# ansonb/RECON

Measured on NVIDIA B200. Metric: SpKBGAT fwd+bwd edges/sec, higher is better.
Workload: dtype f32

## Files before the change

include/spkbgat.h:

```cpp
#ifndef SPKBGAT_H
#define SPKBGAT_H
#include <stdint.h>

#ifdef __cplusplus
extern "C" {
#endif

typedef void* spk_stream_t;

#define SPK_ABI_VERSION 6
int spk_abi_version(void);
const char* spk_last_error(void);
int64_t spk_launch_count(void);

typedef struct {
    int32_t n_heads;
    int32_t d_head;
    int32_t d_pad;
    int32_t width;
} spk_geom;

typedef struct {
    const int32_t* task_seg;
    const int32_t* task_beg;
    const int32_t* task_end;
    const int32_t* hub_seg;
    const int32_t* hub_task_ptr;
    float* partial;
    int64_t ldpart;
    int32_t n_tasks;
    int32_t n_hubs;
    int32_t hub_thresh;
    int32_t reserved;
    const int32_t* task_order;
} spk_hub_tasks;

int spk_edges_concat(const int64_t* edge , int64_t e1, const int64_t* edge_type ,
                     const int64_t* nhop , int64_t e2,
                     int32_t* row, int32_t* col, int32_t* t1, int32_t* t2 ,
                     int64_t n_nodes, int64_t n_rel, int32_t* err_flag, spk_stream_t stream);
int spk_pack_index_host(const int64_t* src, int64_t n, int64_t stride, int64_t lo, int64_t hi, int32_t* dst, int32_t n_threads);
int spk_iota_i32(int32_t* v, int64_t n, spk_stream_t stream);
int64_t spk_sort_workspace_bytes(int64_t n);
int spk_sort_pairs(int32_t* keys, int32_t* vals, int32_t* keys_tmp, int32_t* vals_tmp, int64_t n, int32_t key_bits,
                   void* workspace, int32_t* result_in_tmp, spk_stream_t stream);
int spk_segment_ptr(const int32_t* sorted_keys, int64_t n, int32_t n_seg, int32_t* ptr , spk_stream_t stream);
int spk_gather_i32(const int32_t* src, const int32_t* idx, int64_t n, int32_t* out, spk_stream_t stream);
int spk_rel_incidence(const int32_t* t1, const int32_t* t2, int64_t e, int32_t n_rel, int32_t* keys, int32_t* vals,
                      spk_stream_t stream);

int spk_gemm_nn(const float* A, int64_t lda, const float* B, int64_t ldb, float* C, int64_t ldc,
                int64_t M, int32_t N, int32_t K, int32_t accumulate, spk_stream_t stream);
int64_t spk_gemm_tn_workspace_floats(int64_t M, int32_t Ka, int32_t Nb);
int spk_gemm_tn(const float* A, int64_t lda, const float* B, int64_t ldb, float* C, int64_t ldc,
                int64_t M, int32_t Ka, int32_t Nb, int32_t accumulate, float* workspace, spk_stream_t stream);

int32_t spk_gemm_nn_tc_supported(const float* A, int64_t lda, int64_t M, int32_t N, int32_t K);
int64_t spk_gemm_tc_workspace_floats(int32_t N, int32_t K);
int spk_gemm_nn_tc(const float* A, int64_t lda, const float* B, int64_t ldb, float* C, int64_t ldc,
                   int64_t M, int32_t N, int32_t K, int32_t accumulate, float* workspace, spk_stream_t stream);

int spk_gemm_nn_tc_act(const float* A, int64_t lda, const float* B, int64_t ldb, float* C, int64_t ldc,
                       int64_t M, int32_t N, int32_t K, int32_t accumulate, int32_t act, float* workspace,
                       spk_stream_t stream);
int spk_elu_inplace(float* x, int64_t ldx, int64_t n_rows, int32_t width, spk_stream_t stream);

int32_t spk_gemm_tn_tc_supported(const float* A, int64_t lda, const float* B, int64_t ldb, int64_t M, int32_t Ka, int32_t Nb);
int64_t spk_gemm_tn_tc_workspace_floats(int64_t M, int32_t Ka, int32_t Nb);
int spk_gemm_tn_tc(const float* A, int64_t lda, const float* B, int64_t ldb, float* C, int64_t ldc,
                   int64_t M, int32_t Ka, int32_t Nb, int32_t accumulate, float* workspace, spk_stream_t stream);

typedef struct {
    const int32_t* segptr; const int32_t* col; const int32_t* t1; const int32_t* t2;
    const float* P1; int64_t ld1;
    const float* P2; int64_t ld2;
    const float* P3; int64_t ld3;
    const float* mask; int64_t mask_stride;
    float* out; int64_t ldo;
    float* den; float* sw;
    int32_t* nanflag;
    int32_t n_rows; int32_t apply_elu; float alpha;
    int32_t elu_rows;
    spk_geom geom;
    spk_hub_tasks hub;
} spk_edge_fwd_args;
int spk_edge_attn_fwd(const spk_edge_fwd_args* args, spk_stream_t stream);

typedef struct {
    const int32_t* segptr; const int32_t* col; const int32_t* t1; const int32_t* t2;
    const float* P1; int64_t ld1;
    const float* P2; int64_t ld2;
    const float* P3; int64_t ld3;
    const float* mask; int64_t mask_stride;
    const float* out; const float* dout; int64_t ldo;
    const float* den;
    float* G; int64_t ldg;
    float* dP1; int64_t ldd1;
    float* rec;
    int32_t n_rows; int32_t apply_elu; float alpha; int32_t reserved;
    spk_geom geom;
    spk_hub_tasks hub;
} spk_edge_bwd_rows_args;
int spk_edge_attn_bwd_rows(const spk_edge_bwd_rows_args* args, spk_stream_t stream);

typedef struct {
    const int32_t* segptr; const int32_t* src; const int32_t* pos;
    const float* G; int64_t ldg;
    const float* rec;
    float* out; int64_t ldout;
    int32_t n_seg;
    int32_t flags;
    spk_geom geom;
    spk_hub_tasks hub;
} spk_seg_gather_args;
int spk_edge_attn_bwd_segments(const spk_seg_gather_args* args, spk_stream_t stream);

typedef struct {
    const int32_t* rowptr;
    const int32_t* colptr; const int32_t* csc_row; const int32_t* csc_pos; const int32_t* csc_t1; const int32_t* csc_t2;
    const float* P1; int64_t ld1;
    const float* P2; int64_t ld2;
    const float* P3; int64_t ld3;
    const float* mask; int64_t mask_stride;
    const float* out; const float* dout; int64_t ldo;
    const float* den; const float* sw;
    float* G; int64_t ldg;
    float* rowsc;
    float* dP1; int64_t ldd1;
    float* dP2; int64_t ldd2;
    float* rec;
    int32_t n_rows; int32_t n_cols; int32_t apply_elu; float alpha;
    spk_geom geom;
    spk_hub_tasks row_hub;
    spk_hub_tasks col_hub;
} spk_edge_bwd_fused_args;
int spk_edge_attn_bwd_fused(const spk_edge_bwd_fused_args* args, spk_stream_t stream);

typedef struct {
    spk_edge_bwd_fused_args base;
    const int32_t* relptr; const int32_t* rel_row; const int32_t* rel_pos;
    float* rec4; float* dsv;
    float* dP3; int64_t ldd3;
    int32_t n_rel; int32_t phases;
    spk_hub_tasks rel_hub;
    float* colsum; int64_t ld_colsum;
    float* rowsum; int64_t ld_rowsum;
    const float* G_rel; int64_t ldg_rel;
    int32_t dup; int32_t reserved;
} spk_edge_bwd_split_args;
int spk_edge_attn_bwd_split(const spk_edge_bwd_split_args* args, spk_stream_t stream);

typedef struct {
    int32_t n_heads;
    int32_t f_chunks;
    int32_t r_chunks;
    int32_t lz;
} spk_agg_geom;
int spk_agg_table(const float* X, int64_t ldx, const float* V, float* T, int64_t ldt, int64_t n_rows,
                  int32_t F, int32_t f_chunks, spk_stream_t stream);
typedef struct {
    const int32_t* segptr; const int32_t* col; const int32_t* t1; const int32_t* t2;
    const float* xrow; int64_t ldxr;
    const float* xcol; int64_t ldxc;
    const float* rel; int64_t ldr;
    const float* mask; int64_t mask_stride;
    float* z; int64_t ldz;
    float* den; float* sw;
    int32_t* nanflag;
    int32_t n_rows; float alpha;
    spk_agg_geom geom;
    spk_hub_tasks hub;
} spk_agg_fwd_args;
int spk_agg_fwd(const spk_agg_fwd_args* args, spk_stream_t stream);
int spk_agg_bwd_pre(const float* out, const float* dout, int64_t ldo, const float* den, int32_t n_heads, int32_t d_head,
                    int32_t apply_elu, float* dhn, int64_t ldd, float* dden, int64_t n_rows, spk_stream_t stream);
typedef struct {
    const int32_t* segptr; const int32_t* col; const int32_t* t1; const int32_t* t2;
    const float* xrow; int64_t ldxr; const float* xcol; int64_t ldxc; const float* rel; int64_t ldr;
    const float* mask; int64_t mask_stride;
    const float* dz; int64_t ldz;
    const float* den; const float* sw; const float* dden;
    float* gx; int64_t ldgx;
    float* gr; int64_t ldgr;
    float* rowout; int64_t ldro;
    float* rowsc;
    float* rec;
    int32_t n_rows; float alpha;
    spk_agg_geom geom;
    spk_hub_tasks hub;
} spk_agg_bwd_args;
int spk_agg_bwd_rows(const spk_agg_bwd_args* args, spk_stream_t stream);
int spk_agg_bwd_ctx(const spk_agg_bwd_args* args, spk_stream_t stream);
int spk_agg_dx(const float* rowout, int64_t ldro, const float* dxc, int64_t ldc, const float* V, int64_t n_rows,
               int32_t F, int32_t f_chunks, int32_t n_heads, float* dX, int64_t lddx, float* dq, spk_stream_t stream);

int spk_spmm_rowsum_fwd(const int32_t* segptr, const int32_t* perm, const float* w, int64_t ldw, int32_t width,
                        float* out, int64_t ldo, int32_t n_rows, spk_stream_t stream);
int spk_spmm_rowsum_bwd(const int64_t* edge_row , const float* gout, int64_t ldg, int32_t width,
                        float* gw, int64_t ldw, int64_t n_edges, spk_stream_t stream);

int spk_rownorm(const float* x, int64_t ldx, float* y, int64_t ldy, int64_t n_rows, int32_t width, spk_stream_t stream);
int spk_residual_norm_fwd(const float* ew, int64_t lde, const float* x2, int64_t ldx, const float* mask,
                          float* out, int64_t ldo, float* inv_norm, int64_t n_rows, int32_t width, spk_stream_t stream);
int spk_residual_norm_bwd(const float* g, int64_t ldg, const float* out, int64_t ldo, const float* mask,
                          const float* inv_norm, float* dew, int64_t lde, float* dx2, int64_t ldx,
                          int64_t n_rows, int32_t width, spk_stream_t stream);
int spk_mask_from_index(const int64_t* idx, int64_t n_idx, float* mask, int64_t n_rows, int32_t* flag, spk_stream_t stream);
typedef struct {
    const float* a[4]; const float* a2[4];
    float* da[4]; float* da2[4];
    int32_t n_heads, F, Rd, D;
    int32_t mode; int32_t d_pad, width;
    int32_t f_pad, lz;
    int32_t reserved;
    float* W0; int64_t ld0;
    float* W1; int64_t ld1;
    float* W2;
} spk_attn_weights_args;
int spk_attn_weights_fwd(const spk_attn_weights_args* args, spk_stream_t stream);
int spk_attn_weights_bwd(const spk_attn_weights_args* args, spk_stream_t stream);

int64_t spk_inner_product_workspace_bytes(void);
int spk_inner_product(const float* a, const float* b, int64_t n, void* workspace, float* out, int32_t accumulate,
                      spk_stream_t stream);

int64_t spk_margin_loss_partials(int64_t n_pos);
int spk_margin_loss_fwd(const int64_t* triples, int64_t n_triples, int64_t n_pos,
                        const float* ent, int64_t lde, int64_t n_ent, const float* rel, int64_t ldr, int64_t n_rel,
                        int32_t width, float margin, int32_t mean,
                        float* norm, uint32_t* sgn, float* coef, double* partial, float* loss,
                        int32_t* err_flag, spk_stream_t stream);
int spk_triple_incidence(const int64_t* triples, int64_t n_triples, int64_t n_ent, int64_t n_rel,
                         int32_t* ent_keys , int32_t* ent_vals, int32_t* rel_keys , int32_t* rel_vals,
// ... 66 lines not shown
```

recon_b200/_lib.py:

```python
import ctypes as C
import os

import torch

_HERE = os.path.dirname(os.path.abspath(__file__))
LIB_PATH = os.environ.get("SPK_LIB") or os.path.join(_HERE, "libspkbgat.so")

c_i32p = C.POINTER(C.c_int32)
c_i64p = C.POINTER(C.c_int64)
c_f32p = C.POINTER(C.c_float)
ABI_VERSION = 6


class Geom(C.Structure):
    _fields_ = [("n_heads", C.c_int32), ("d_head", C.c_int32), ("d_pad", C.c_int32), ("width", C.c_int32)]


class HubTasks(C.Structure):
    _fields_ = [("task_seg", C.c_void_p), ("task_beg", C.c_void_p), ("task_end", C.c_void_p),
                ("hub_seg", C.c_void_p), ("hub_task_ptr", C.c_void_p),
                ("partial", C.c_void_p), ("ldpart", C.c_int64),
                ("n_tasks", C.c_int32), ("n_hubs", C.c_int32), ("hub_thresh", C.c_int32), ("reserved", C.c_int32),
                ("task_order", C.c_void_p)]


class EdgeFwdArgs(C.Structure):
    _fields_ = [("segptr", C.c_void_p), ("col", C.c_void_p), ("t1", C.c_void_p), ("t2", C.c_void_p),
                ("P1", C.c_void_p), ("ld1", C.c_int64), ("P2", C.c_void_p), ("ld2", C.c_int64),
                ("P3", C.c_void_p), ("ld3", C.c_int64),
                ("mask", C.c_void_p), ("mask_stride", C.c_int64),
                ("out", C.c_void_p), ("ldo", C.c_int64), ("den", C.c_void_p), ("sw", C.c_void_p),
                ("nanflag", C.c_void_p),
                ("n_rows", C.c_int32), ("apply_elu", C.c_int32), ("alpha", C.c_float), ("elu_rows", C.c_int32),
                ("geom", Geom), ("hub", HubTasks)]


class EdgeBwdRowsArgs(C.Structure):
    _fields_ = [("segptr", C.c_void_p), ("col", C.c_void_p), ("t1", C.c_void_p), ("t2", C.c_void_p),
                ("P1", C.c_void_p), ("ld1", C.c_int64), ("P2", C.c_void_p), ("ld2", C.c_int64),
                ("P3", C.c_void_p), ("ld3", C.c_int64),
                ("mask", C.c_void_p), ("mask_stride", C.c_int64),
                ("out", C.c_void_p), ("dout", C.c_void_p), ("ldo", C.c_int64),
                ("den", C.c_void_p),
                ("G", C.c_void_p), ("ldg", C.c_int64), ("dP1", C.c_void_p), ("ldd1", C.c_int64),
                ("rec", C.c_void_p),
                ("n_rows", C.c_int32), ("apply_elu", C.c_int32), ("alpha", C.c_float), ("reserved", C.c_int32),
                ("geom", Geom), ("hub", HubTasks)]


class SegGatherArgs(C.Structure):
    _fields_ = [("segptr", C.c_void_p), ("src", C.c_void_p), ("pos", C.c_void_p),
                ("G", C.c_void_p), ("ldg", C.c_int64), ("rec", C.c_void_p),
                ("out", C.c_void_p), ("ldout", C.c_int64),
                ("n_seg", C.c_int32), ("flags", C.c_int32),
                ("geom", Geom), ("hub", HubTasks)]


class EdgeBwdFusedArgs(C.Structure):
    _fields_ = [("rowptr", C.c_void_p),
                ("colptr", C.c_void_p), ("csc_row", C.c_void_p), ("csc_pos", C.c_void_p), ("csc_t1", C.c_void_p),
                ("csc_t2", C.c_void_p),
                ("P1", C.c_void_p), ("ld1", C.c_int64), ("P2", C.c_void_p), ("ld2", C.c_int64),
                ("P3", C.c_void_p), ("ld3", C.c_int64),
                ("mask", C.c_void_p), ("mask_stride", C.c_int64),
                ("out", C.c_void_p), ("dout", C.c_void_p), ("ldo", C.c_int64),
                ("den", C.c_void_p), ("sw", C.c_void_p),
                ("G", C.c_void_p), ("ldg", C.c_int64), ("rowsc", C.c_void_p),
                ("dP1", C.c_void_p), ("ldd1", C.c_int64), ("dP2", C.c_void_p), ("ldd2", C.c_int64),
                ("rec", C.c_void_p),
                ("n_rows", C.c_int32), ("n_cols", C.c_int32), ("apply_elu", C.c_int32), ("alpha", C.c_float),
                ("geom", Geom), ("row_hub", HubTasks), ("col_hub", HubTasks)]


class EdgeBwdSplitArgs(C.Structure):
    _fields_ = [("base", EdgeBwdFusedArgs),
                ("relptr", C.c_void_p), ("rel_row", C.c_void_p), ("rel_pos", C.c_void_p),
                ("rec4", C.c_void_p), ("dsv", C.c_void_p),
                ("dP3", C.c_void_p), ("ldd3", C.c_int64),
                ("n_rel", C.c_int32), ("phases", C.c_int32),
                ("rel_hub", HubTasks),
                ("colsum", C.c_void_p), ("ld_colsum", C.c_int64),
                ("rowsum", C.c_void_p), ("ld_rowsum", C.c_int64),
                ("G_rel", C.c_void_p), ("ldg_rel", C.c_int64),
                ("dup", C.c_int32), ("reserved", C.c_int32)]


class AggGeom(C.Structure):
    _fields_ = [("n_heads", C.c_int32), ("f_chunks", C.c_int32), ("r_chunks", C.c_int32), ("lz", C.c_int32)]


class AggFwdArgs(C.Structure):
    _fields_ = [("segptr", C.c_void_p), ("col", C.c_void_p), ("t1", C.c_void_p), ("t2", C.c_void_p),
                ("xrow", C.c_void_p), ("ldxr", C.c_int64), ("xcol", C.c_void_p), ("ldxc", C.c_int64),
                ("rel", C.c_void_p), ("ldr", C.c_int64),
                ("mask", C.c_void_p), ("mask_stride", C.c_int64),
                ("z", C.c_void_p), ("ldz", C.c_int64), ("den", C.c_void_p), ("sw", C.c_void_p),
                ("nanflag", C.c_void_p),
                ("n_rows", C.c_int32), ("alpha", C.c_float),
                ("geom", AggGeom), ("hub", HubTasks)]


class AggBwdArgs(C.Structure):
    _fields_ = [("segptr", C.c_void_p), ("col", C.c_void_p), ("t1", C.c_void_p), ("t2", C.c_void_p),
                ("xrow", C.c_void_p), ("ldxr", C.c_int64), ("xcol", C.c_void_p), ("ldxc", C.c_int64),
                ("rel", C.c_void_p), ("ldr", C.c_int64),
                ("mask", C.c_void_p), ("mask_stride", C.c_int64),
                ("dz", C.c_void_p), ("ldz", C.c_int64),
                ("den", C.c_void_p), ("sw", C.c_void_p), ("dden", C.c_void_p),
                ("gx", C.c_void_p), ("ldgx", C.c_int64), ("gr", C.c_void_p), ("ldgr", C.c_int64),
                ("rowout", C.c_void_p), ("ldro", C.c_int64), ("rowsc", C.c_void_p), ("rec", C.c_void_p),
                ("n_rows", C.c_int32), ("alpha", C.c_float),
                ("geom", AggGeom), ("hub", HubTasks)]


_VP, _I64, _I32 = C.c_void_p, C.c_int64, C.c_int32

ALLOC_FN = C.CFUNCTYPE(C.c_void_p, C.c_void_p, C.c_int64)


class TripleGraphArgs(C.Structure):
    _fields_ = [("uptr", C.c_void_p), ("ut", C.c_void_p), ("ur0", C.c_void_p), ("ugs", C.c_void_p), ("uge", C.c_void_p),
                ("rs", C.c_void_p), ("n_nodes", C.c_int32), ("n_pairs", C.c_int32), ("n_triples", C.c_int32),
                ("reserved", C.c_int32)]


class NhopResult(C.Structure):
    _fields_ = [("adj_idx", C.c_void_p), ("adj_val", C.c_void_p), ("nhop", C.c_void_p), ("e1", C.c_int64), ("e2", C.c_int64)]


class LossBwdArgs(C.Structure):
    _fields_ = [("segptr", C.c_void_p), ("inc", C.c_void_p), ("coef", C.c_void_p), ("sgn", C.c_void_p),
                ("gscale", C.c_void_p), ("out", C.c_void_p), ("ldo", C.c_int64),
                ("n_seg", C.c_int32), ("width", C.c_int32), ("mode", C.c_int32), ("reserved", C.c_int32),
                ("hub", HubTasks)]


class SgdArgs(C.Structure):
    _fields_ = [("param", C.c_void_p * 16), ("grad", C.c_void_p * 16), ("numel", C.c_int64 * 16),
                ("count", C.c_int32), ("lr", C.c_float)]


class AttnWeightsArgs(C.Structure):
    _fields_ = [("a", C.c_void_p * 4), ("a2", C.c_void_p * 4), ("da", C.c_void_p * 4), ("da2", C.c_void_p * 4),
                ("n_heads", C.c_int32), ("F", C.c_int32), ("Rd", C.c_int32), ("D", C.c_int32),
                ("mode", C.c_int32), ("d_pad", C.c_int32), ("width", C.c_int32),
                ("f_pad", C.c_int32), ("lz", C.c_int32), ("reserved", C.c_int32),
                ("W0", C.c_void_p), ("ld0", C.c_int64), ("W1", C.c_void_p), ("ld1", C.c_int64), ("W2", C.c_void_p)]


SIGNATURES = {
    "spk_abi_version": (_I32, []),
    "spk_last_error": (C.c_char_p, []),
    "spk_launch_count": (_I64, []),
    "spk_edges_concat": (_I32, [_VP, _I64, _VP, _VP, _I64, _VP, _VP, _VP, _VP, _I64, _I64, _VP, _VP]),
    "spk_pack_index_host": (_I32, [_VP, _I64, _I64, _I64, _I64, _VP, _I32]),
    "spk_iota_i32": (_I32, [_VP, _I64, _VP]),
    "spk_sort_workspace_bytes": (_I64, [_I64]),
    "spk_sort_pairs": (_I32, [_VP, _VP, _VP, _VP, _I64, _I32, _VP, C.POINTER(_I32), _VP]),
    "spk_segment_ptr": (_I32, [_VP, _I64, _I32, _VP, _VP]),
    "spk_gather_i32": (_I32, [_VP, _VP, _I64, _VP, _VP]),
    "spk_rel_incidence": (_I32, [_VP, _VP, _I64, _I32, _VP, _VP, _VP]),
    "spk_gemm_nn": (_I32, [_VP, _I64, _VP, _I64, _VP, _I64, _I64, _I32, _I32, _I32, _VP]),
    "spk_gemm_nn_tc_supported": (_I32, [_VP, _I64, _I64, _I32, _I32]),
    "spk_gemm_tc_workspace_floats": (_I64, [_I32, _I32]),
    "spk_gemm_nn_tc": (_I32, [_VP, _I64, _VP, _I64, _VP, _I64, _I64, _I32, _I32, _I32, _VP, _VP]),
    "spk_gemm_nn_tc_act": (_I32, [_VP, _I64, _VP, _I64, _VP, _I64, _I64, _I32, _I32, _I32, _I32, _VP, _VP]),
    "spk_elu_inplace": (_I32, [_VP, _I64, _I64, _I32, _VP]),
    "spk_agg_table": (_I32, [_VP, _I64, _VP, _VP, _I64, _I64, _I32, _I32, _VP]),
    "spk_agg_fwd": (_I32, [C.POINTER(AggFwdArgs), _VP]),
    "spk_agg_bwd_pre": (_I32, [_VP, _VP, _I64, _VP, _I32, _I32, _I32, _VP, _I64, _VP, _I64, _VP]),
    "spk_agg_bwd_rows": (_I32, [C.POINTER(AggBwdArgs), _VP]),
    "spk_agg_bwd_ctx": (_I32, [C.POINTER(AggBwdArgs), _VP]),
    "spk_agg_dx": (_I32, [_VP, _I64, _VP, _I64, _VP, _I64, _I32, _I32, _I32, _VP, _I64, _VP, _VP]),
    "spk_gemm_tn_tc_supported": (_I32, [_VP, _I64, _VP, _I64, _I64, _I32, _I32]),
    "spk_gemm_tn_tc_workspace_floats": (_I64, [_I64, _I32, _I32]),
    "spk_gemm_tn_tc": (_I32, [_VP, _I64, _VP, _I64, _VP, _I64, _I64, _I32, _I32, _I32, _VP, _VP]),
    "spk_gemm_tn_workspace_floats": (_I64, [_I64, _I32, _I32]),
    "spk_gemm_tn": (_I32, [_VP, _I64, _VP, _I64, _VP, _I64, _I64, _I32, _I32, _I32, _VP, _VP]),
    "spk_edge_attn_fwd": (_I32, [C.POINTER(EdgeFwdArgs), _VP]),
    "spk_edge_attn_bwd_rows": (_I32, [C.POINTER(EdgeBwdRowsArgs), _VP]),
    "spk_edge_attn_bwd_segments": (_I32, [C.POINTER(SegGatherArgs), _VP]),
    "spk_edge_attn_bwd_fused": (_I32, [C.POINTER(EdgeBwdFusedArgs), _VP]),
    "spk_edge_attn_bwd_split": (_I32, [C.POINTER(EdgeBwdSplitArgs), _VP]),
    "spk_spmm_rowsum_fwd": (_I32, [_VP, _VP, _VP, _I64, _I32, _VP, _I64, _I32, _VP]),
    "spk_spmm_rowsum_bwd": (_I32, [_VP, _VP, _I64, _I32, _VP, _I64, _I64, _VP]),
    "spk_rownorm": (_I32, [_VP, _I64, _VP, _I64, _I64, _I32, _VP]),
    "spk_residual_norm_fwd": (_I32, [_VP, _I64, _VP, _I64, _VP, _VP, _I64, _VP, _I64, _I32, _VP]),
    "spk_residual_norm_bwd": (_I32, [_VP, _I64, _VP, _I64, _VP, _VP, _VP, _I64, _VP, _I64, _I64, _I32, _VP]),
    "spk_mask_from_index": (_I32, [_VP, _I64, _VP, _I64, _VP, _VP]),
    "spk_attn_weights_fwd": (_I32, [_VP, _VP]),
    "spk_attn_weights_bwd": (_I32, [_VP, _VP]),
    "spk_inner_product_workspace_bytes": (_I64, []),
    "spk_inner_product": (_I32, [_VP, _VP, _I64, _VP, _VP, _I32, _VP]),
    "spk_margin_loss_partials": (_I64, [_I64]),
    "spk_margin_loss_fwd": (_I32, [_VP, _I64, _I64, _VP, _I64, _I64, _VP, _I64, _I64, _I32, C.c_float, _I32,
                                   _VP, _VP, _VP, _VP, _VP, _VP, _VP]),
    "spk_triple_incidence": (_I32, [_VP, _I64, _I64, _I64, _VP, _VP, _VP, _VP, _VP, _VP]),
    "spk_margin_loss_bwd": (_I32, [C.POINTER(LossBwdArgs), _VP]),
    "spk_sgd_step": (_I32, [C.POINTER(SgdArgs), _VP]),
    "spk_triple_keys": (_I32, [_VP, _I64, _I64, _I64, _VP, _VP, _VP]),
    "spk_corrupt_triples": (_I32, [_VP, _I64, _I32, _VP, _I64, _I64, _I64, _VP, _VP, C.c_uint64, _VP, _VP, _VP]),
    "spk_nhop_build": (_I32, [C.POINTER(TripleGraphArgs), _VP, _I64, _I32, ALLOC_FN, _VP, C.POINTER(NhopResult), _VP]),
    "spk_gather_concat": (_I32, [_VP, _VP, _VP, _VP, _VP, _I32, _I64, _I32, _VP, _I64, _VP, _VP]),
    "spk_mlp_head_fwd": (_I32, [_VP, _I64, _VP, _VP, _VP, C.c_float, _I64, _I32, _VP, _VP]),
    "spk_mlp_head_bwd": (_I32, [_VP, _I64, _VP, _VP, C.c_float, _VP, _I64, _I32, _VP, _I64, _VP, _I64, _VP]),
    "spk_tanh_fwd": (_I32, [_VP, _I64, _I64, _I32, _VP]),
    "spk_tanh_bwd": (_I32, [_VP, _I64, _VP, _I64, _I64, _I32, _VP, _I64, _VP]),
    "spk_rank_scores": (_I32, [_VP, _I64, _VP, _I64, _VP, _VP, C.c_float, _I64, _I32, _I32, _VP, _I64, _VP]),
    "spk_linkpred_count": (_I32, [_VP, _I64, _I64, _VP, _I64, _I64, _VP, _VP, C.c_float, _I32, _VP, _VP, _I64, _I32,
                                  _VP, _I64, _VP, _VP, _VP, _VP, _VP]),
    "spk_linkpred_filter": (_I32, [_VP, _I64, _I64, _I64, _VP, C.c_float, _I32, _VP, _I64, _I32, _VP, _I64, _VP, _VP,
                                   _VP, _I64, _VP, _VP, _VP, _VP]),
    "spk_export_json": (_I32, [_VP, _I64, _I64, _I64, C.c_char_p, _I32]),
    "spk_export_bin": (_I32, [_VP, _I64, _I64, _I64, C.c_char_p]),
    "spk_import_json_shape": (_I32, [C.c_char_p, C.POINTER(_I64), C.POINTER(_I64)]),
    "spk_import_json": (_I32, [C.c_char_p, _VP, _I64, _I64, _I64, _I32]),
}

_lib = None
current_tag = ""


class _Lib:

    def __init__(self, cdll):
        self._cdll = cdll
        self.timing = None

    def __getattr__(self, name):
        fn = getattr(self._cdll, name)
        if self.timing is None or SIGNATURES[name][1][-1:] != [_VP] or "workspace" in name or "supported" in name:
            return fn

        def timed(*args):
            e0 = torch.cuda.Event(enable_timing=True)
            e1 = torch.cuda.Event(enable_timing=True)
            e0.record()
            rc = fn(*args)
            e1.record()
            global current_tag
            self.timing.append((name[4:] + (":" + current_tag if current_tag else ""), e0, e1))
            if "gemm" in name:
                current_tag = ""
            return rc
        return timed


def load():
    global _lib
    if _lib is not None:
        return _lib
    if not os.path.exists(LIB_PATH):
        raise RuntimeError(
            f"{LIB_PATH} is missing: build it with `python -c 'import __graft_entry__ as g; g.build()'` "
            "(or make -C recon_b200/csrc). recon_b200 has no CPU / PyTorch fallback.")
    lib = C.CDLL(LIB_PATH)
    for name, (res, args) in SIGNATURES.items():
        fn = getattr(lib, name)
        fn.restype = res
        fn.argtypes = args
    if lib.spk_abi_version() != ABI_VERSION:
        raise RuntimeError(f"libspkbgat ABI {lib.spk_abi_version()} != binding {ABI_VERSION}")
    _lib = _Lib(lib)
    return _lib


def stream_ptr():
    return C.c_void_p(torch.cuda.current_stream().cuda_stream)


def ptr(t):
    if t is None:
        return None
    if not t.is_cuda:
        raise RuntimeError("recon_b200 ops need CUDA tensors (no CPU fallback)")
    return t.data_ptr()


def launch_count():
    return int(load().spk_launch_count())


def check(rc, what):
    if rc != 0:
        msg = load().spk_last_error().decode("utf-8", "replace")
        raise RuntimeError(f"libspkbgat {what} failed (code {rc}): {msg}")
```

recon_b200/csrc/spk_api.cu:

```cuda
#include "../../include/spkbgat.h"
#include "spk_common.cuh"
#include "spk_edge.cuh"
#include "spk_edge_bwd_fused.cuh"
#include "spk_agg.cuh"
#include "spk_gemm.cuh"
#include "spk_graph.cuh"
#include "spk_rowops.cuh"

namespace spk {

static thread_local char g_err[512] = "";
static unsigned long long g_launches = 0;

void set_error(const char* fmt, ...) {
    va_list ap;
    va_start(ap, fmt);
    vsnprintf(g_err, sizeof(g_err), fmt, ap);
    va_end(ap);
}

int check_launch(const char* what) {
    const cudaError_t e = cudaGetLastError();
    __atomic_fetch_add(&g_launches, 1ULL, __ATOMIC_RELAXED);
    if (e == cudaSuccess) return 0;
// ... 61 lines not shown
extern "C" {

int spk_abi_version(void) { return SPK_ABI_VERSION; }
const char* spk_last_error(void) { return g_err; }
int64_t spk_launch_count(void) { return (int64_t)__atomic_load_n(&g_launches, __ATOMIC_RELAXED); }

int spk_edges_concat(const int64_t* edge, int64_t e1, const int64_t* edge_type, const int64_t* nhop, int64_t e2,
                     int32_t* row, int32_t* col, int32_t* t1, int32_t* t2, int64_t n_nodes, int64_t n_rel,
                     int32_t* err_flag, spk_stream_t stream) {
    if (e1 + e2 >= (1LL << 31) || n_nodes >= (1LL << 31)) { set_error("edges_concat: sizes exceed int32"); return 1; }
    if (e2 > 0 && !t2) { set_error("edges_concat: t2 required when 2-hop rows are given"); return 1; }
    return edges_concat(reinterpret_cast<const long long*>(edge), e1, reinterpret_cast<const long long*>(edge_type),
                        reinterpret_cast<const long long*>(nhop), e2, row, col, t1, t2, n_nodes, n_rel, err_flag,
                        (cudaStream_t)stream);
}
int spk_iota_i32(int32_t* v, int64_t n, spk_stream_t stream) { return iota_i32(v, n, (cudaStream_t)stream); }
int64_t spk_sort_workspace_bytes(int64_t n) { return radix_sort_workspace_bytes(n); }
int spk_sort_pairs(int32_t* keys, int32_t* vals, int32_t* keys_tmp, int32_t* vals_tmp, int64_t n, int32_t key_bits,
                   void* workspace, int32_t* result_in_tmp, spk_stream_t stream) {
    if (key_bits < 1 || key_bits > 31) { set_error("sort_pairs: key_bits %d out of range", key_bits); return 1; }
    return radix_sort_pairs(keys, vals, keys_tmp, vals_tmp, n, key_bits, workspace, result_in_tmp, (cudaStream_t)stream);
}
int spk_segment_ptr(const int32_t* sorted_keys, int64_t n, int32_t n_seg, int32_t* ptr, spk_stream_t stream) {
    return segment_ptr(sorted_keys, n, n_seg, ptr, (cudaStream_t)stream);
}
int spk_gather_i32(const int32_t* src, const int32_t* idx, int64_t n, int32_t* out, spk_stream_t stream) {
    return gather_i32(src, idx, n, out, (cudaStream_t)stream);
}
int spk_rel_incidence(const int32_t* t1, const int32_t* t2, int64_t e, int32_t n_rel, int32_t* keys, int32_t* vals,
                      spk_stream_t stream) {
    return rel_incidence(t1, t2, e, n_rel, keys, vals, (cudaStream_t)stream);
}

int spk_gemm_nn(const float* A, int64_t lda, const float* B, int64_t ldb, float* C, int64_t ldc,
                int64_t M, int32_t N, int32_t K, int32_t accumulate, spk_stream_t stream) {
    if (lda < K || ldb < N || ldc < N) { set_error("gemm_nn: leading dimension too small"); return 1; }
    return gemm_nn_simt(A, lda, B, ldb, C, ldc, M, N, K, accumulate, (cudaStream_t)stream);
}
int64_t spk_gemm_tn_workspace_floats(int64_t M, int32_t Ka, int32_t Nb) { return gemm_tn_workspace_floats(M, Ka, Nb); }
int spk_gemm_tn(const float* A, int64_t lda, const float* B, int64_t ldb, float* C, int64_t ldc,
                int64_t M, int32_t Ka, int32_t Nb, int32_t accumulate, float* workspace, spk_stream_t stream) {
    if (lda < Ka || ldb < Nb || ldc < Nb) { set_error("gemm_tn: leading dimension too small"); return 1; }
    if (!workspace) { set_error("gemm_tn: workspace required"); return 1; }
    return gemm_tn_simt(A, lda, B, ldb, C, ldc, M, Ka, Nb, accumulate, workspace, (cudaStream_t)stream);
}

int32_t spk_gemm_nn_tc_supported(const float* A, int64_t lda, int64_t M, int32_t N, int32_t K) {
    return gemm_nn_tc_supported(A, lda, M, N, K);
}
int64_t spk_gemm_tc_workspace_floats(int32_t N, int32_t K) { return 2LL * N * gemm_tc_ldt(K); }
int spk_gemm_nn_tc(const float* A, int64_t lda, const float* B, int64_t ldb, float* C, int64_t ldc,
                   int64_t M, int32_t N, int32_t K, int32_t accumulate, float* workspace, spk_stream_t stream) {
    if (lda < K || ldb < N || ldc < N) { set_error("gemm_nn_tc: leading dimension too small"); return 1; }
    if (!gemm_nn_tc_supported(A, lda, M, N, K)) { set_error("gemm_nn_tc: A must be 16-byte aligned with lda %% 4 == 0"); return 1; }
    if (!workspace || (reinterpret_cast<uintptr_t>(workspace) & 15)) { set_error("gemm_nn_tc: aligned workspace required"); return 1; }
    return gemm_nn_tc(A, lda, B, ldb, C, ldc, M, N, K, accumulate, workspace, (cudaStream_t)stream);
}

int spk_gemm_nn_tc_act(const float* A, int64_t lda, const float* B, int64_t ldb, float* C, int64_t ldc,
                       int64_t M, int32_t N, int32_t K, int32_t accumulate, int32_t act, float* workspace, spk_stream_t stream) {
    if (lda < K || ldb < N || ldc < N) { set_error("gemm_nn_tc_act: leading dimension too small"); return 1; }
    if (!gemm_nn_tc_supported(A, lda, M, N, K)) { set_error("gemm_nn_tc_act: A must be 16-byte aligned with lda %% 4 == 0"); return 1; }
    if (!workspace || (reinterpret_cast<uintptr_t>(workspace) & 15)) { set_error("gemm_nn_tc_act: aligned workspace required"); return 1; }
    if (act < 0 || act > 2) { set_error("gemm_nn_tc_act: unknown activation %d", act); return 1; }
    return gemm_nn_tc(A, lda, B, ldb, C, ldc, M, N, K, accumulate, workspace, (cudaStream_t)stream, act);
}
int spk_elu_inplace(float* x, int64_t ldx, int64_t n_rows, int32_t width, spk_stream_t stream) {
    if (ldx < width) { set_error("elu_inplace: leading dimension too small"); return 1; }
    return launch_elu_inplace(x, ldx, n_rows, width, (cudaStream_t)stream);
}

int32_t spk_gemm_tn_tc_supported(const float* A, int64_t lda, const float* B, int64_t ldb, int64_t M, int32_t Ka, int32_t Nb) {
    return gemm_tn_tc_supported(A, lda, B, ldb, M, Ka, Nb);
}
int64_t spk_gemm_tn_tc_workspace_floats(int64_t M, int32_t Ka, int32_t Nb) { return gemm_tn_tc_workspace_floats(M, Ka, Nb); }
int spk_gemm_tn_tc(const float* A, int64_t lda, const float* B, int64_t ldb, float* C, int64_t ldc,
                   int64_t M, int32_t Ka, int32_t Nb, int32_t accumulate, float* workspace, spk_stream_t stream) {
    if (ldc < Nb) { set_error("gemm_tn_tc: leading dimension too small"); return 1; }
    if (!gemm_tn_tc_supported(A, lda, B, ldb, M, Ka, Nb)) { set_error("gemm_tn_tc: operands must be 16-byte aligned with ld %% 4 == 0"); return 1; }
    if (!workspace) { set_error("gemm_tn_tc: workspace required"); return 1; }
    return gemm_tn_tc(A, lda, B, ldb, C, ldc, M, Ka, Nb, accumulate, workspace, (cudaStream_t)stream);
}

int spk_edge_attn_fwd(const spk_edge_fwd_args* p, spk_stream_t stream) {
    EdgeFwdArgs a;
    if (!geom_ok(p->geom, &a.g, "edge_attn_fwd")) return 1;
    if ((p->ld1 & 3) || (p->ld2 & 3) || (p->ld3 & 3) || p->ld1 < p->geom.width || p->ld2 < p->geom.width ||
        p->ld3 < p->geom.width || !aligned16(p->P1) || !aligned16(p->P2) || !aligned16(p->P3)) {
        set_error("edge_attn_fwd: projected tables must be 16-byte aligned with ld >= width, ld %% 4 == 0");
        return 1;
    }
    a.segptr = p->segptr; a.col = p->col; a.t1 = p->t1; a.t2 = p->t2;
    a.P1 = p->P1; a.ld1 = p->ld1; a.P2 = p->P2; a.ld2 = p->ld2; a.P3 = p->P3; a.ld3 = p->ld3;
    a.mask = p->mask; a.mask_stride = p->mask_stride;
    a.out = p->out; a.ldo = p->ldo; a.den = p->den; a.sw = p->sw; a.nanflag = p->nanflag;
    a.n_rows = p->n_rows; a.alpha = p->alpha; a.apply_elu = p->apply_elu;
    a.elu_rows = p->elu_rows > 0 ? p->elu_rows : 0x7fffffff;
    a.out_vec = (p->geom.d_head % 4 == 0) && (p->ldo % 4 == 0) && aligned16(p->out);
    a.hub = hub_of(p->hub);
    if (a.hub.n_tasks > 0 && (a.hub.ldpart < p->geom.width + 2 * SPK_MAX_HEADS || (a.hub.ldpart & 3) || !aligned16(a.hub.partial))) {
        set_error("edge_attn_fwd: hub partial buffer needs ldpart >= width+8, ldpart %% 4 == 0");
        return 1;
    }
    return launch_edge_fwd(a, (cudaStream_t)stream);
}

int spk_edge_attn_bwd_rows(const spk_edge_bwd_rows_args* p, spk_stream_t stream) {
    EdgeBwdRowsArgs a;
    if (!geom_ok(p->geom, &a.g, "edge_attn_bwd_rows")) return 1;
    if ((p->ld1 & 3) || (p->ld2 & 3) || (p->ld3 & 3) || (p->ldg & 3) || (p->ldd1 & 3) || p->ldg < p->geom.n_heads * p->geom.d_pad ||
        p->ldd1 < p->geom.width || !aligned16(p->P1) || !aligned16(p->P2) || !aligned16(p->P3) || !aligned16(p->G) ||
        !aligned16(p->dP1) || (reinterpret_cast<uintptr_t>(p->rec) & 7)) {
        set_error("edge_attn_bwd_rows: bad leading dimension or alignment");
        return 1;
    }
    a.segptr = p->segptr; a.col = p->col; a.t1 = p->t1; a.t2 = p->t2;
    a.P1 = p->P1; a.ld1 = p->ld1; a.P2 = p->P2; a.ld2 = p->ld2; a.P3 = p->P3; a.ld3 = p->ld3;
    a.mask = p->mask; a.mask_stride = p->mask_stride;
    a.out = p->out; a.dout = p->dout; a.ldo = p->ldo; a.den = p->den;
    a.G = p->G; a.ldg = p->ldg; a.dP1 = p->dP1; a.ldd1 = p->ldd1; a.rec = p->rec;
    a.n_rows = p->n_rows; a.alpha = p->alpha; a.apply_elu = p->apply_elu;
    a.out_vec = (p->geom.d_head % 4 == 0) && (p->ldo % 4 == 0) && aligned16(p->out) && aligned16(p->dout);
    a.hub = hub_of(p->hub);
    if (a.hub.n_tasks > 0 && a.hub.ldpart < 2 * SPK_MAX_HEADS) { set_error("edge_attn_bwd_rows: hub ldpart must be >= 8"); return 1; }
    return launch_edge_bwd_rows(a, (cudaStream_t)stream);
}

int spk_edge_attn_bwd_segments(const spk_seg_gather_args* p, spk_stream_t stream) {
    SegGatherArgs a;
    if (!geom_ok(p->geom, &a.g, "edge_attn_bwd_segments")) return 1;
    if ((p->ldg & 3) || (p->ldout & 3) || p->ldout < p->geom.width || p->ldg < p->geom.n_heads * p->geom.d_pad ||
        !aligned16(p->G) || !aligned16(p->out) || (reinterpret_cast<uintptr_t>(p->rec) & 7)) {
        set_error("edge_attn_bwd_segments: bad leading dimension or alignment");
        return 1;
    }
    a.segptr = p->segptr; a.src = p->src; a.pos = p->pos; a.G = p->G; a.ldg = p->ldg; a.rec = p->rec;
    a.outp = p->out; a.ldout = p->ldout; a.n_seg = p->n_seg; a.prefer_stream = p->flags & 1;
    a.hub = hub_of(p->hub);
    if (a.hub.n_tasks > 0 && (a.hub.ldpart < p->geom.width || (a.hub.ldpart & 3) || !aligned16(a.hub.partial))) {
        set_error("edge_attn_bwd_segments: hub partial buffer needs ldpart >= width");
        return 1;
    }
    return launch_seg_gather(a, (cudaStream_t)stream);
}

static int fused_args_of(const spk_edge_bwd_fused_args* p, BwdFusedArgs& a, const char* who, int dup = 0);

int spk_edge_attn_bwd_fused(const spk_edge_bwd_fused_args* p, spk_stream_t stream) {
    BwdFusedArgs a;
    if (int rc = fused_args_of(p, a, "edge_attn_bwd_fused")) return rc;
    if (reinterpret_cast<uintptr_t>(p->rec) & 7) { set_error("edge_attn_bwd_fused: rec must be 8-byte aligned"); return 1; }
    return launch_edge_bwd_fused(a, (cudaStream_t)stream);
}

int spk_edge_attn_bwd_split(const spk_edge_bwd_split_args* q, spk_stream_t stream) {
    BwdSplitArgs a;
    if (int rc = fused_args_of(&q->base, a.f, "edge_attn_bwd_split", q->dup)) return rc;
    if (q->base.csc_t2 != nullptr) { set_error("edge_attn_bwd_split: graphs with 2-hop edges are not supported"); return 1; }
    if ((q->ldd3 & 3) || q->ldd3 < q->base.geom.width || !aligned16(q->dP3) || !aligned16(q->rec4) ||
        (reinterpret_cast<uintptr_t>(q->dsv) & 3)) {
        set_error("edge_attn_bwd_split: bad leading dimension or alignment");
        return 1;
    }
    a.colptr = a.f.colptr; a.csc_row = a.f.csc_row; a.csc_pos = a.f.csc_pos; a.csc_t1 = a.f.csc_t1;
    a.relptr = q->relptr; a.rel_row = q->rel_row; a.rel_pos = q->rel_pos;
    a.P2 = a.f.P2; a.ld2 = a.f.ld2; a.P3 = a.f.P3; a.ld3 = a.f.ld3; a.mask = a.f.mask; a.mask_stride = a.f.mask_stride;
    a.G = a.f.G; a.ldg = a.f.ldg; a.rowsc = a.f.rowsc; a.rec4 = q->rec4; a.dsv = q->dsv;
    a.dP2 = a.f.dP2; a.ldd2 = a.f.ldd2; a.dP3 = q->dP3; a.ldd3 = q->ldd3;
    a.n_cols = a.f.n_cols; a.n_rel = q->n_rel; a.g = a.f.g; a.alpha = a.f.alpha;
    a.col_hub = a.f.col_hub;
    if (a.f.row_hub.n_tasks > 0 && (a.f.row_hub.partial == nullptr || a.f.row_hub.ldpart < 4)) {
        set_error("edge_attn_bwd_split: row hub partial buffer [n_tasks, >= 4] required");
        return 1;
    }
    a.phases = q->phases == 0 ? 15 : q->phases;
    a.colsum = q->colsum; a.ld_colsum = q->ld_colsum;
    a.rowsum = q->rowsum; a.ld_rowsum = q->ld_rowsum;
    a.G_rel = q->G_rel ? q->G_rel : a.f.G; a.ldg_rel = q->G_rel ? q->ldg_rel : a.f.ldg;
    a.dup = q->dup;
    if ((a.rowsum && a.ld_rowsum < q->base.geom.n_heads) || (q->G_rel && ((q->ldg_rel & 3) || !aligned16(q->G_rel) ||
        q->ldg_rel < q->base.geom.n_heads * q->base.geom.d_pad)) || (a.dup && (a.phases & 1))) {
        set_error("edge_attn_bwd_split: bad rowsum / G_rel / dup arguments");
        return 1;
    }
    if (a.phases < 0 || a.phases > 15 || (a.colsum && a.ld_colsum < q->base.geom.n_heads)) {
        set_error("edge_attn_bwd_split: bad phases / colsum");
        return 1;
    }
    a.rel_hub = hub_of(q->rel_hub);
    if (a.rel_hub.n_tasks > 0 && (a.rel_hub.ldpart < q->base.geom.width || (a.rel_hub.ldpart & 3) || !aligned16(a.rel_hub.partial))) {
        set_error("edge_attn_bwd_split: relation hub partial buffer needs ldpart >= width");
        return 1;
    }
    return launch_edge_bwd_split(a, (cudaStream_t)stream);
}

static int fused_args_of(const spk_edge_bwd_fused_args* p, BwdFusedArgs& a, const char* who, int dup) {
    if (!geom_ok(p->geom, &a.g, who)) return 1;
    const int64_t tab_w = dup ? p->geom.d_pad + 4 : p->geom.width;
    if ((p->ld1 & 3) || (p->ld2 & 3) || (p->ld3 & 3) || (p->ldg & 3) || (p->ldd1 & 3) || (p->ldd2 & 3) ||
        p->ldg < p->geom.n_heads * p->geom.d_pad || p->ldd1 < p->geom.width || p->ldd2 < p->geom.width ||
        (!dup && p->ld1 < p->geom.width) || p->ld2 < tab_w || p->ld3 < tab_w ||
        !aligned16(p->P1) || !aligned16(p->P2) || !aligned16(p->P3) || !aligned16(p->G) || !aligned16(p->dP1) ||
        !aligned16(p->dP2) || !aligned16(p->rowsc)) {
        set_error("%s: bad leading dimension or alignment", who);
        return 1;
    }
    a.rowptr = p->rowptr; a.colptr = p->colptr; a.csc_row = p->csc_row; a.csc_pos = p->csc_pos;
    a.csc_t1 = p->csc_t1; a.csc_t2 = p->csc_t2;
    a.P1 = p->P1; a.ld1 = p->ld1; a.P2 = p->P2; a.ld2 = p->ld2; a.P3 = p->P3; a.ld3 = p->ld3;
    a.mask = p->mask; a.mask_stride = p->mask_stride;
    a.out = p->out; a.dout = p->dout; a.ldo = p->ldo; a.den = p->den; a.sw = p->sw;
    a.G = p->G; a.ldg = p->ldg; a.rowsc = p->rowsc; a.dP1 = p->dP1; a.ldd1 = p->ldd1; a.dP2 = p->dP2; a.ldd2 = p->ldd2;
    a.rec = p->rec; a.n_rows = p->n_rows; a.n_cols = p->n_cols; a.alpha = p->alpha; a.apply_elu = p->apply_elu;
    a.out_vec = (p->geom.d_head % 4 == 0) && (p->ldo % 4 == 0) && aligned16(p->out) && aligned16(p->dout);
    a.row_hub = hub_of(p->row_hub);
    a.col_hub = hub_of(p->col_hub);
    if (a.col_hub.n_tasks > 0 && (a.col_hub.ldpart < p->geom.width || (a.col_hub.ldpart & 3) || !aligned16(a.col_hub.partial))) {
        set_error("%s: hub partial buffer needs ldpart >= width", who);
        return 1;
    }
    return 0;
}

static bool agg_geom_ok(const spk_agg_geom& g, AggGeom* out, const char* who) {
    if (g.n_heads < 1 || g.n_heads > 2 || g.f_chunks < 1 || g.f_chunks > 15 || g.r_chunks < 1 || g.r_chunks > 15 ||
        g.lz != 4 * (2 * g.f_chunks + g.r_chunks)) {
        set_error("%s: bad geometry H=%d f_chunks=%d r_chunks=%d lz=%d", who, g.n_heads, g.f_chunks, g.r_chunks, g.lz);
        return false;
    }
    out->H = g.n_heads; out->Fx4 = g.f_chunks; out->Fr4 = g.r_chunks; out->LZ = g.lz;
    return true;
}

int spk_agg_table(const float* X, int64_t ldx, const float* V, float* T, int64_t ldt, int64_t n_rows, int32_t F,
                  int32_t f_chunks, spk_stream_t stream) {
    if (F < 1 || F > 60 || f_chunks != (F + 3) / 4 || ldt < 4 * f_chunks + 4 || ldx < F || !aligned16(V)) {
        set_error("agg_table: needs 1 <= F <= 60, f_chunks = ceil(F/4), ldt >= 4*f_chunks+4, 16-byte aligned V");
        return 1;
    }
    return launch_agg_table(X, ldx, V, T, ldt, n_rows, F, f_chunks, (cudaStream_t)stream);
}

int spk_agg_fwd(const spk_agg_fwd_args* p, spk_stream_t stream) {
    AggFwdArgs a;
    if (!agg_geom_ok(p->geom, &a.g, "agg_fwd")) return 1;
    const int wx = 4 * a.g.Fx4 + 4, wr = 4 * a.g.Fr4 + 4;
    if ((p->ldxr & 3) || (p->ldxc & 3) || (p->ldr & 3) || (p->ldz & 3) || p->ldxr < wx || p->ldxc < wx || p->ldr < wr ||
        p->ldz < (int64_t)a.g.H * a.g.LZ || !aligned16(p->xrow) || !aligned16(p->xcol) || !aligned16(p->rel) || !aligned16(p->z)) {
        set_error("agg_fwd: tables must be 16-byte aligned with ld %% 4 == 0 and wide enough");
        return 1;
    }
    a.segptr = p->segptr; a.col = p->col; a.t1 = p->t1; a.t2 = p->t2;
    a.Xrow = p->xrow; a.ldxr = p->ldxr; a.Xcol = p->xcol; a.ldxc = p->ldxc; a.Rt = p->rel; a.ldr = p->ldr;
    a.mask = p->mask; a.mask_stride = p->mask_stride;
    a.Z = p->z; a.ldz = p->ldz; a.den = p->den; a.sw = p->sw; a.nanflag = p->nanflag;
    a.n_rows = p->n_rows; a.alpha = p->alpha;
    a.hub = hub_of(p->hub);
    if (a.hub.n_tasks > 0 && (a.hub.ldpart < AGG_LDPART || (a.hub.ldpart & 3) || !aligned16(a.hub.partial))) {
        set_error("agg_fwd: hub partial buffer needs ldpart >= %d, ldpart %% 4 == 0", AGG_LDPART);
        return 1;
    }
    return launch_agg_fwd(a, (cudaStream_t)stream);
}

int spk_agg_bwd_pre(const float* out, const float* dout, int64_t ldo, const float* den, int32_t n_heads, int32_t d_head,
                    int32_t apply_elu, float* dhn, int64_t ldd, float* dden, int64_t n_rows, spk_stream_t stream) {
    if (n_heads < 1 || d_head < 1 || ldo < (int64_t)n_heads * d_head || ldd < (int64_t)n_heads * d_head) {
        set_error("agg_bwd_pre: bad shape");
        return 1;
    }
    return launch_agg_bwd_pre(out, dout, ldo, den, n_heads, d_head, apply_elu, dhn, ldd, dden, n_rows, (cudaStream_t)stream);
}

int spk_agg_bwd_rows(const spk_agg_bwd_args* p, spk_stream_t stream) {
    AggBwdArgs a;
    if (!agg_geom_ok(p->geom, &a.g, "agg_bwd_rows")) return 1;
// ... 118 lines not shown
```

recon_b200/csrc/spk_edge.cuh:

```cuda
#pragma once
#include "spk_common.cuh"

namespace spk {

struct HubTasks {
    const int* task_seg;
    const int* task_beg;
    const int* task_end;
    const int* hub_seg;
    const int* hub_task_ptr;
    float* partial;
    long ldpart;
    int n_tasks;
    int n_hubs;
    int hub_thresh;
    const int* task_order;
};

__device__ __forceinline__ int hub_task_of_slot(const HubTasks& h, int slot) {
    return h.task_order ? __ldg(h.task_order + slot) : slot;
}

struct EdgeFwdArgs {
    const int* segptr;
    const int* col;
    const int* t1;
    const int* t2;
    const float* P1; long ld1;
    const float* P2; long ld2;
    const float* P3; long ld3;
    const float* mask; long mask_stride;
    float* out; long ldo;
    float* den;
    float* sw;
    int* nanflag;
    int n_rows;
    LayerGeom g;
    float alpha;
    int apply_elu;
    int elu_rows;
    int out_vec;
    HubTasks hub;
};

struct EdgeBwdRowsArgs {
    const int* segptr; const int* col; const int* t1; const int* t2;
    const float* P1; long ld1;
    const float* P2; long ld2;
    const float* P3; long ld3;
    const float* mask; long mask_stride;
    const float* out; const float* dout; long ldo;
    const float* den;
    float* G; long ldg;
    float* dP1; long ldd1;
    float* rec;
    int n_rows;
    LayerGeom g;
    float alpha;
    int apply_elu;
    int out_vec;
    HubTasks hub;
};

struct SegGatherArgs {
    const int* segptr;
    const int* src;
    const int* pos;
    const float* G; long ldg;
    const float* rec;
    float* outp; long ldout;
    int n_seg;
    int prefer_stream;
    LayerGeom g;
    HubTasks hub;
};

int launch_edge_fwd(const EdgeFwdArgs& a, cudaStream_t s);
int launch_edge_bwd_rows(const EdgeBwdRowsArgs& a, cudaStream_t s);
int launch_seg_gather(const SegGatherArgs& a, cudaStream_t s);

}
```

recon_b200/csrc/spk_edge_bwd.cuh:

```cuda
#pragma once
#include "spk_edge.cuh"

namespace spk {

__device__ __forceinline__ float4 load_act_chunk(const float* base, int h, int off, int D, int vec) {
    const float* p = base + (long)h * D + off;
    if (vec) return ldg4(p);
    float4 r;
    r.x = off + 0 < D ? __ldg(p + 0) : 0.f;
    r.y = off + 1 < D ? __ldg(p + 1) : 0.f;
    r.z = off + 2 < D ? __ldg(p + 2) : 0.f;
    r.w = off + 3 < D ? __ldg(p + 3) : 0.f;
    return r;
}

template <int NCH, int HT>
struct RowCtx {
    float4 dnum[NCH];
    int hc[NCH];
    float q1[HT];
    float dden[HT];
    float c1[HT];
};

template <int NCH, int HT>
__device__ __forceinline__ void bwd_row_prologue(const EdgeBwdRowsArgs& a, int row, int lane, RowCtx<NCH, HT>& rc) {
    const LayerGeom g = a.g;
    float pdh[HT], pc1[HT], den[HT];
#pragma unroll
    for (int h = 0; h < HT; ++h) {
        pdh[h] = 0.f; pc1[h] = 0.f;
        den[h] = h < g.H ? __ldg(a.den + (long)row * g.H + h) : 1.f;
    }
    const float4 q1v = ldg4(a.P1 + (long)row * a.ld1 + (long)g.Dt4 * 4);
#pragma unroll
    for (int h = 0; h < HT; ++h) rc.q1[h] = f4get(q1v, h);
#pragma unroll
    for (int ci = 0; ci < NCH; ++ci) {
        const int c4 = lane + 32 * ci;
        rc.hc[ci] = 0;
        rc.dnum[ci] = make_float4(0.f, 0.f, 0.f, 0.f);
        if (c4 >= g.Dt4) continue;
        const int h = HT > 1 ? c4 / g.Dp4 : 0;
        rc.hc[ci] = h;
        const int off = (c4 - h * g.Dp4) * 4;
        const float4 o4 = load_act_chunk(a.out + (long)row * a.ldo, h, off, g.D, a.out_vec);
        const float4 g4 = load_act_chunk(a.dout + (long)row * a.ldo, h, off, g.D, a.out_vec);
        const float o[4] = {o4.x, o4.y, o4.z, o4.w};
        const float gg[4] = {g4.x, g4.y, g4.z, g4.w};
        float dh[4], hv[4];
#pragma unroll
        for (int k = 0; k < 4; ++k) {
            if (a.apply_elu) {
                const bool pos = o[k] > 0.f;
                dh[k] = pos ? gg[k] : gg[k] * (o[k] + 1.f);
                hv[k] = pos ? o[k] : (o[k] > -1.f ? fast_log1p(o[k]) : 0.f);
            } else {
                dh[k] = gg[k];
                hv[k] = o[k];
            }
        }
        const float d = selh<HT>(h, den);
        const float dot_h = fmaf(dh[0], hv[0], fmaf(dh[1], hv[1], fmaf(dh[2], hv[2], dh[3] * hv[3])));
        rc.dnum[ci] = make_float4(dh[0] / d, dh[1] / d, dh[2] / d, dh[3] / d);
        const float4 p1 = ldg4(a.P1 + (long)row * a.ld1 + c4 * 4);
        const float dot_c = f4dot(rc.dnum[ci], p1);
#pragma unroll
        for (int hh = 0; hh < HT; ++hh) {
            pdh[hh] += (h == hh) ? dot_h : 0.f;
            pc1[hh] += (h == hh) ? dot_c : 0.f;
        }
    }
#pragma unroll
    for (int h = 0; h < HT; ++h) {
        rc.dden[h] = 0.f; rc.c1[h] = 0.f;
        if (h < g.H) {
            rc.dden[h] = -warp_sum(pdh[h]) / den[h];
            rc.c1[h] = warp_sum(pc1[h]);
        }
    }
}

template <int NCH, int HT>
__device__ __forceinline__ void bwd_row_store(const EdgeBwdRowsArgs& a, int row, int lane, const RowCtx<NCH, HT>& rc,
                                              const float (&usum)[HT], const float (&swsum)[HT],
                                              bool store_g, bool store_dp1) {
    const LayerGeom g = a.g;
#pragma unroll
    for (int ci = 0; ci < NCH; ++ci) {
        const int c4 = lane + 32 * ci;
        if (store_g && c4 * 4 < a.ldg)
            *reinterpret_cast<float4*>(a.G + (long)row * a.ldg + c4 * 4) = rc.dnum[ci];
        if (store_dp1 && c4 < g.Wd4) {
            float4 o;
            if (c4 < g.Dt4) {
                const float s = selh<HT>(rc.hc[ci], swsum);
                o = make_float4(s * rc.dnum[ci].x, s * rc.dnum[ci].y, s * rc.dnum[ci].z, s * rc.dnum[ci].w);
            } else if (c4 == g.Dt4) {
                o = make_float4(usum[0], HT > 1 ? usum[HT > 1 ? 1 : 0] : 0.f, HT > 2 ? usum[HT > 2 ? 2 : 0] : 0.f,
                                HT > 3 ? usum[HT > 3 ? 3 : 0] : 0.f);
            } else {
                o = make_float4(0.f, 0.f, 0.f, 0.f);
            }
            *reinterpret_cast<float4*>(a.dP1 + (long)row * a.ldd1 + c4 * 4) = o;
        }
    }
}


int launch_edge_bwd_rows_stream(const EdgeBwdRowsArgs& a, cudaStream_t s);

}
```

recon_b200/csrc/spk_edge_bwd_fused.cu:

```cuda
#include <stdlib.h>
#include "spk_edge.cuh"
#include "spk_edge_bwd.cuh"
#include "spk_edge_bwd_fused.cuh"

namespace spk {
namespace {

constexpr unsigned FULLM = 0xffffffffu;
__device__ __forceinline__ float fexp(float x) { return exp2f(x * 1.4426950408889634f); }

template <int NCH, int HT>
__global__ void __launch_bounds__(SPK_CTA_THREADS)
bwd_node_kernel(const EdgeBwdRowsArgs a, const float* __restrict__ sw, float* __restrict__ rowsc) {
    const int lane = threadIdx.x & 31;
    const int row = blockIdx.x * SPK_WARPS_PER_CTA + (threadIdx.x >> 5);
    if (row >= a.n_rows) return;
    if (__ldg(a.segptr + row) == __ldg(a.segptr + row + 1)) {
        for (int c4 = lane; c4 < a.g.Wd4; c4 += 32)
            *reinterpret_cast<float4*>(a.dP1 + (long)row * a.ldd1 + c4 * 4) = make_float4(0.f, 0.f, 0.f, 0.f);
        return;
    }
    RowCtx<NCH, HT> rc;
    bwd_row_prologue<NCH, HT>(a, row, lane, rc);
    float usum[HT], swsum[HT];
#pragma unroll
    for (int h = 0; h < HT; ++h) {
        usum[h] = 0.f;
        swsum[h] = h < a.g.H ? __ldg(sw + (long)row * a.g.H + h) : 0.f;
    }
    bwd_row_store<NCH, HT>(a, row, lane, rc, usum, swsum, true, true);
    if (lane < a.g.H) {
        const float4 o = make_float4(selh<HT>(lane, rc.q1), selh<HT>(lane, rc.c1), selh<HT>(lane, rc.dden), 0.f);
        *reinterpret_cast<float4*>(rowsc + ((long)row * a.g.H + lane) * 4) = o;
    }
}

template <int NCH, int HT>
struct ColCtx {
    float4 p2[NCH];
    int hc[NCH];
    float q2[HT];
};

template <int NCH, int HT>
__device__ __forceinline__ void col_ctx_load(const BwdFusedArgs& a, int colj, int lane, ColCtx<NCH, HT>& cc) {
    const LayerGeom g = a.g;
    const float* p = a.P2 + (long)colj * a.ld2;
#pragma unroll
    for (int ci = 0; ci < NCH; ++ci) {
        const int c4 = lane + 32 * ci;
        cc.hc[ci] = (HT > 1 && c4 < g.Dt4) ? c4 / g.Dp4 : 0;
        cc.p2[ci] = c4 < g.Dt4 ? ldg4(p + c4 * 4) : make_float4(0.f, 0.f, 0.f, 0.f);
    }
    const float4 qv = ldg4(p + (long)g.Dt4 * 4);
#pragma unroll
    for (int h = 0; h < HT; ++h) cc.q2[h] = f4get(qv, h);
}

template <int NCH, int HT>
struct ColAcc {
    float4 acc[NCH];
    float vs[HT];
};

template <int NCH, int HT, bool HAS2, int U>
__device__ __forceinline__ void col_accumulate(const BwdFusedArgs& a, int beg, int end, int lane,
                                               const ColCtx<NCH, HT>& cc, ColAcc<NCH, HT>& st) {
    const LayerGeom g = a.g;
    const int H = g.H;
    const bool has_mask = a.mask != nullptr;
    for (int base = beg; base < end; base += 32) {
        const int n = min(32, end - base);
        int my_row = 0, my_pos = 0, my_k1 = 0, my_k2 = -1;
        float my_w[HT], my_ca[HT], my_cb[HT], my_t[HT];
#pragma unroll
        for (int h = 0; h < HT; ++h) { my_w[h] = 0.f; my_ca[h] = 0.f; my_cb[h] = 0.f; my_t[h] = 0.f; }
        if (lane < n) {
            my_row = __ldg(a.csc_row + base + lane);
            my_pos = __ldg(a.csc_pos + base + lane);
            my_k1 = __ldg(a.csc_t1 + base + lane);
            if (HAS2) my_k2 = __ldg(a.csc_t2 + base + lane);
            float4 q3 = ldg4(a.P3 + (long)my_k1 * a.ld3 + (long)g.Dt4 * 4);
            if (HAS2 && my_k2 >= 0) q3 = f4add(q3, ldg4(a.P3 + (long)my_k2 * a.ld3 + (long)g.Dt4 * 4));
#pragma unroll
            for (int h = 0; h < HT; ++h) {
                if (h < H) {
                    const float4 rs = ldg4(a.rowsc + ((long)my_row * H + h) * 4);
                    const float m = has_mask ? __ldg(a.mask + (long)h * a.mask_stride + my_pos) : 1.f;
                    const float s = rs.x + cc.q2[h] + f4get(q3, h);
                    const float slope = s > 0.f ? 1.f : a.alpha;
                    const float ee = fexp(-(s * slope));
                    my_w[h] = ee * m;
                    my_ca[h] = my_w[h] * slope;
                    my_cb[h] = fmaf(m, rs.y, rs.z) * ee * slope;
                }
            }
        }
        for (int u0 = 0; u0 < n; u0 += U) {
            float4 v[U][NCH], r[U][NCH];
#pragma unroll
            for (int u = 0; u < U; ++u) {
                const int idx = u0 + u;
                const int i = __shfl_sync(FULLM, my_row, idx & 31);
                const int k1 = __shfl_sync(FULLM, my_k1, idx & 31);
                int k2 = -1;
                if (HAS2) k2 = __shfl_sync(FULLM, my_k2, idx & 31);
// ... 134 lines not shown
    __shared__ float red[HT][512];
    const int row = __ldg(hub_seg + blockIdx.x);
    const int beg = __ldg(rowptr + row), end = __ldg(rowptr + row + 1);
    float u[HT];
#pragma unroll
    for (int h = 0; h < HT; ++h) u[h] = 0.f;
    for (int e = beg + threadIdx.x; e < end; e += 512) {
#pragma unroll
        for (int h = 0; h < HT; ++h)
            if (h < H) u[h] += __ldg(rec + (long)e * (2 * H) + 2 * h + 1);
    }
#pragma unroll
    for (int h = 0; h < HT; ++h) red[h][threadIdx.x] = u[h];
    __syncthreads();
    for (int s = 256; s > 0; s >>= 1) {
        if ((int)threadIdx.x < s) {
#pragma unroll
            for (int h = 0; h < HT; ++h) red[h][threadIdx.x] += red[h][threadIdx.x + s];
        }
        __syncthreads();
    }
    if ((int)threadIdx.x < H) dP1[(long)row * ldd1 + qoff + threadIdx.x] = red[threadIdx.x < HT ? threadIdx.x : 0][0];
}

static int fused_variant() {
    static int v = -1;
    if (v < 0) { const char* e = getenv("SPK_FUSED_VARIANT"); v = e ? atoi(e) : 0; if (v < 0 || v > 1) v = 0; }
    return v;
}

template <int NCH, int HT, bool HAS2, int U, int MINB>
int launch_cols_v(const BwdFusedArgs& a, cudaStream_t s) {
    if (a.n_cols > 0) {
        const unsigned grid = (a.n_cols + SPK_WARPS_PER_CTA - 1) / SPK_WARPS_PER_CTA;
        bwd_cols_fused_kernel<NCH, HT, HAS2, U, MINB><<<grid, SPK_CTA_THREADS, 0, s>>>(a);
        if (int rc = check_launch("bwd_cols_fused")) return rc;
    }
    if (a.col_hub.n_tasks > 0) {
        const unsigned grid = (a.col_hub.n_tasks + SPK_WARPS_PER_CTA - 1) / SPK_WARPS_PER_CTA;
        bwd_cols_fused_tasks_kernel<NCH, HT, HAS2, U, MINB><<<grid, SPK_CTA_THREADS, 0, s>>>(a);
        if (int rc = check_launch("bwd_cols_fused_tasks")) return rc;
    }
    return 0;
}

template <int NCH, int HT, bool HAS2>
int launch_fused_t(const BwdFusedArgs& a, cudaStream_t s) {
    constexpr int U = (NCH <= 2) ? 4 : 2;
    constexpr int MINB = (NCH <= 2) ? 2 : 1;
    bool done = false;
    if constexpr (NCH <= 2) {
        if (fused_variant() == 1) { if (int rc = launch_cols_v<NCH, HT, HAS2, 2, 3>(a, s)) return rc; done = true; }
    }
    if (!done) { if (int rc = launch_cols_v<NCH, HT, HAS2, U, MINB>(a, s)) return rc; }
    if (a.col_hub.n_tasks > 0) {
        SegGatherArgs fa;
        fa.segptr = a.colptr; fa.src = nullptr; fa.pos = nullptr; fa.G = a.G; fa.ldg = a.ldg; fa.rec = a.rec;
        fa.outp = a.dP2; fa.ldout = a.ldd2; fa.n_seg = a.n_cols; fa.prefer_stream = 0; fa.g = a.g; fa.hub = a.col_hub;
        if (int rc = launch_seg_gather_hub_finalize(fa, s)) return rc;
    }
    if (a.n_rows > 0) {
        const unsigned grid = (a.n_rows + SPK_WARPS_PER_CTA - 1) / SPK_WARPS_PER_CTA;
        bwd_rowsum_kernel<HT><<<grid, SPK_CTA_THREADS, 0, s>>>(a.rowptr, a.rec, a.g.H, a.n_rows, a.row_hub.hub_thresh,
                                                               a.dP1, a.ldd1, a.g.Dt4 * 4);
        if (int rc = check_launch("bwd_rowsum")) return rc;
        if (a.row_hub.n_hubs > 0) {
            bwd_rowsum_hub_kernel<HT><<<a.row_hub.n_hubs, 512, 0, s>>>(a.rowptr, a.row_hub.hub_seg, a.rec, a.g.H, a.dP1,
                                                                       a.ldd1, a.g.Dt4 * 4);
            if (int rc = check_launch("bwd_rowsum_hub")) return rc;
        }
    }
    return 0;
}

template <int NCH>
int launch_fused_n(const BwdFusedArgs& a, cudaStream_t s) {
    const bool has2 = a.csc_t2 != nullptr;
    if (a.g.H == 1) return has2 ? launch_fused_t<NCH, 1, true>(a, s) : launch_fused_t<NCH, 1, false>(a, s);
    if (a.g.H == 2) return has2 ? launch_fused_t<NCH, 2, true>(a, s) : launch_fused_t<NCH, 2, false>(a, s);
    return has2 ? launch_fused_t<NCH, 4, true>(a, s) : launch_fused_t<NCH, 4, false>(a, s);
}


template <int NCH>
int launch_node_n(const EdgeBwdRowsArgs& ra, const BwdFusedArgs& a, cudaStream_t s) {
    const unsigned grid = (a.n_rows + SPK_WARPS_PER_CTA - 1) / SPK_WARPS_PER_CTA;
    if (a.g.H == 1) bwd_node_kernel<NCH, 1><<<grid, SPK_CTA_THREADS, 0, s>>>(ra, a.sw, a.rowsc);
    else if (a.g.H == 2) bwd_node_kernel<NCH, 2><<<grid, SPK_CTA_THREADS, 0, s>>>(ra, a.sw, a.rowsc);
    else bwd_node_kernel<NCH, 4><<<grid, SPK_CTA_THREADS, 0, s>>>(ra, a.sw, a.rowsc);
    return check_launch("bwd_node");
}

}

int launch_edge_bwd_node(const BwdFusedArgs& a, cudaStream_t s) {
    if (a.n_rows <= 0) return 0;
    EdgeBwdRowsArgs ra;
    ra.segptr = a.rowptr; ra.col = nullptr; ra.t1 = nullptr; ra.t2 = nullptr;
    ra.P1 = a.P1; ra.ld1 = a.ld1; ra.P2 = a.P2; ra.ld2 = a.ld2; ra.P3 = a.P3; ra.ld3 = a.ld3;
    ra.mask = nullptr; ra.mask_stride = 0;
    ra.out = a.out; ra.dout = a.dout; ra.ldo = a.ldo; ra.den = a.den;
    ra.G = a.G; ra.ldg = a.ldg; ra.dP1 = a.dP1; ra.ldd1 = a.ldd1; ra.rec = a.rec;
    ra.n_rows = a.n_rows; ra.g = a.g; ra.alpha = a.alpha; ra.apply_elu = a.apply_elu; ra.out_vec = a.out_vec;
    ra.hub = a.row_hub;
    switch ((a.g.Wd4 + 31) / 32) {
        case 1: return launch_node_n<1>(ra, a, s);
        case 2: return launch_node_n<2>(ra, a, s);
        case 3: return launch_node_n<3>(ra, a, s);
        case 4: return launch_node_n<4>(ra, a, s);
        default: set_error("edge_bwd_node: row width %d floats exceeds the supported 512", a.g.Wd4 * 4); return 2;
    }
}

int launch_edge_bwd_fused(const BwdFusedArgs& a, cudaStream_t s) {
    if (int rc = launch_edge_bwd_node(a, s)) return rc;
    switch ((a.g.Wd4 + 31) / 32) {
        case 1: return launch_fused_n<1>(a, s);
        case 2: return launch_fused_n<2>(a, s);
        case 3: return launch_fused_n<3>(a, s);
        case 4: return launch_fused_n<4>(a, s);
        default: set_error("edge_bwd_fused: row width %d floats exceeds the supported 512", a.g.Wd4 * 4); return 2;
    }
}

}
```

recon_b200/csrc/spk_edge_bwd_fused.cuh:

```cuda
#pragma once
#include "spk_edge.cuh"

namespace spk {

struct BwdFusedArgs {
    const int* rowptr;
    const int* colptr;
    const int* csc_row;
    const int* csc_pos;
    const int* csc_t1;
    const int* csc_t2;
    const float* P1; long ld1;
    const float* P2; long ld2;
    const float* P3; long ld3;
    const float* mask; long mask_stride;
    const float* out; const float* dout; long ldo;
    const float* den; const float* sw;
    float* G; long ldg;
    float* rowsc;
    float* dP1; long ldd1;
    float* dP2; long ldd2;
    float* rec;
    int n_rows, n_cols;
    LayerGeom g;
    float alpha;
    int apply_elu;
    int out_vec;
    HubTasks row_hub;
    HubTasks col_hub;
};

struct BwdSplitArgs {
    BwdFusedArgs f;
    const int* colptr; const int* csc_row; const int* csc_pos; const int* csc_t1;
    const int* relptr; const int* rel_row; const int* rel_pos;
    const float* P2; long ld2;
    const float* P3; long ld3;
    const float* mask; long mask_stride;
    const float* G; long ldg;
    const float* rowsc;
    float* rec4;
    float* dsv;
    float* dP2; long ldd2;
    float* dP3; long ldd3;
    int n_cols, n_rel;
    LayerGeom g;
    float alpha;
    HubTasks col_hub;
    HubTasks rel_hub;
    int phases;
    float* colsum; long ld_colsum;
    float* rowsum; long ld_rowsum;
    const float* G_rel; long ldg_rel;
    int dup;
};

int launch_edge_bwd_fused(const BwdFusedArgs& a, cudaStream_t s);
int launch_edge_bwd_node(const BwdFusedArgs& a, cudaStream_t s);
int launch_edge_bwd_split(const BwdSplitArgs& a, cudaStream_t s);
int launch_seg_gather_hub_finalize(const SegGatherArgs& a, cudaStream_t s);

}
```

recon_b200/csrc/spk_edge_bwd_split.cu:

```cuda
#include <stdlib.h>
#include "spk_edge.cuh"
#include "spk_edge_bwd.cuh"
#include "spk_edge_bwd_fused.cuh"

namespace spk {
namespace {

constexpr unsigned FULLM = 0xffffffffu;
__device__ __forceinline__ float sexp(float x) { return exp2f(x * 1.4426950408889634f); }

template <int NCH, int HT>
struct SegCtx {
    float4 p[NCH];
    int hc[NCH];
    float q[HT];
};

template <int NCH, int HT>
__device__ __forceinline__ void seg_ctx_load(const float* __restrict__ row, const LayerGeom& g, int lane, SegCtx<NCH, HT>& cc,
                                             int dup = 0) {
#pragma unroll
    for (int ci = 0; ci < NCH; ++ci) {
        const int c4 = lane + 32 * ci;
        cc.hc[ci] = (HT > 1 && c4 < g.Dt4) ? c4 / g.Dp4 : 0;
// ... 345 lines not shown
        if (int rc = check_launch("split_sum_hub")) return rc;
    }
    return 0;
}

static int split_variant() {
    static int v = -1;
    if (v < 0) { const char* e = getenv("SPK_SPLIT_VARIANT"); v = e ? atoi(e) : 0; if (v < 0 || v > 3) v = 0; }
    return v;
}

static int sm_count() {
    static int n[64] = {};
    int dev = 0;
    if (cudaGetDevice(&dev) != cudaSuccess || dev < 0 || dev >= 64) return 148;
    if (n[dev] == 0) { int v = 148; cudaDeviceGetAttribute(&v, cudaDevAttrMultiProcessorCount, dev); n[dev] = v > 0 ? v : 148; }
    return n[dev];
}
static int split_persist() {
    static int v = -1;
    if (v < 0) { const char* e = getenv("SPK_SPLIT_PERSIST"); v = e ? atoi(e) : 8; if (v < 0 || v > 64) v = 8; }
    return v;
}

template <int NCH, int HT, int U, int MINB>
int launch_split_passes(const BwdSplitArgs& a, cudaStream_t s, int which) {
    if (which == 0) {
        if (a.n_cols > 0) {
            const unsigned full = (a.n_cols + SPK_WARPS_PER_CTA - 1) / SPK_WARPS_PER_CTA;
            const unsigned resident = (unsigned)(sm_count() * MINB) * (unsigned)split_persist();
            const unsigned grid = (split_persist() > 0 && full > resident) ? resident : full;
            split_cols_kernel<NCH, HT, U, MINB><<<grid, SPK_CTA_THREADS, 0, s>>>(a);
            if (int rc = check_launch("split_cols")) return rc;
        }
        if (a.col_hub.n_tasks > 0) {
            const unsigned grid = (a.col_hub.n_tasks + SPK_WARPS_PER_CTA - 1) / SPK_WARPS_PER_CTA;
            split_cols_tasks_kernel<NCH, HT, U, MINB><<<grid, SPK_CTA_THREADS, 0, s>>>(a);
            if (int rc = check_launch("split_cols_tasks")) return rc;
        }
    } else {
        if (a.n_rel > 0) {
            const unsigned grid = (a.n_rel + SPK_WARPS_PER_CTA - 1) / SPK_WARPS_PER_CTA;
            split_rels_kernel<NCH, HT, U, MINB><<<grid, SPK_CTA_THREADS, 0, s>>>(a);
            if (int rc = check_launch("split_rels")) return rc;
        }
        if (a.rel_hub.n_tasks > 0) {
            const unsigned grid = (a.rel_hub.n_tasks + SPK_WARPS_PER_CTA - 1) / SPK_WARPS_PER_CTA;
            split_rels_tasks_kernel<NCH, HT, U, MINB><<<grid, SPK_CTA_THREADS, 0, s>>>(a);
            if (int rc = check_launch("split_rels_tasks")) return rc;
        }
    }
    return 0;
}

static int split_variant_narrow() {
    static int v = -1;
    if (v < 0) { const char* e = getenv("SPK_SPLIT_VARIANT1"); v = e ? atoi(e) : 0; if (v < 0 || v > 4) v = 0; }
    return v;
}

template <int NCH, int HT>
int launch_split_pass(const BwdSplitArgs& a, cudaStream_t s, int which) {
    if constexpr (NCH == 1) {
        switch (split_variant_narrow()) {
            case 1: return launch_split_passes<NCH, HT, 2, 6>(a, s, which);
            case 2: return launch_split_passes<NCH, HT, 2, 8>(a, s, which);
            case 3: return launch_split_passes<NCH, HT, 4, 5>(a, s, which);
            case 4: return launch_split_passes<NCH, HT, 4, 6>(a, s, which);
            default: return launch_split_passes<NCH, HT, 4, 4>(a, s, which);
        }
    } else if constexpr (NCH <= 2) {
        switch (split_variant()) {
            case 1: return launch_split_passes<NCH, HT, 4, 3>(a, s, which);
            case 2: return launch_split_passes<NCH, HT, 2, 4>(a, s, which);
            case 3: return launch_split_passes<NCH, HT, 8, 2>(a, s, which);
            default: return launch_split_passes<NCH, HT, 4, 4>(a, s, which);
        }
    } else {
        return launch_split_passes<NCH, HT, 2, 2>(a, s, which);
    }
}

template <int NCH, int HT>
int launch_split_t(const BwdSplitArgs& a, cudaStream_t s) {
    if (a.phases & 1) {
        if (int rc = launch_edge_bwd_node(a.f, s)) return rc;
    }
    if (a.phases & 2) {
        if (int rc = launch_split_pass<NCH, HT>(a, s, 0)) return rc;
        if (a.col_hub.n_tasks > 0) {
            SegGatherArgs fa;
            fa.segptr = a.colptr; fa.src = nullptr; fa.pos = nullptr; fa.G = a.G; fa.ldg = a.ldg; fa.rec = nullptr;
            fa.outp = a.dP2; fa.ldout = a.ldd2; fa.n_seg = a.n_cols; fa.prefer_stream = 0; fa.g = a.g; fa.hub = a.col_hub;
            if (int rc = launch_seg_gather_hub_finalize(fa, s)) return rc;
        }
    }
    if (a.phases & 4) {
        if (int rc = launch_split_pass<NCH, HT>(a, s, 1)) return rc;
        if (a.rel_hub.n_tasks > 0) {
            SegGatherArgs fa;
            fa.segptr = a.relptr; fa.src = nullptr; fa.pos = nullptr; fa.G = a.G; fa.ldg = a.ldg; fa.rec = nullptr;
            fa.outp = a.dP3; fa.ldout = a.ldd3; fa.n_seg = a.n_rel; fa.prefer_stream = 0; fa.g = a.g; fa.hub = a.rel_hub;
            if (int rc = launch_seg_gather_hub_finalize(fa, s)) return rc;
        }
        if (a.rowsum) {
            if (int rc = launch_sums<HT>(a.f.rowptr, nullptr, a.dsv, a.g.H, a.f.n_rows, a.f.row_hub, a.rowsum, a.ld_rowsum, 0, s)) return rc;
        } else {
            if (int rc = launch_sums<HT>(a.f.rowptr, nullptr, a.dsv, a.g.H, a.f.n_rows, a.f.row_hub, a.f.dP1, a.f.ldd1, a.g.Dt4 * 4, s)) return rc;
        }
    }
    if (a.phases & 8) {
        if (a.colsum) return launch_sums<HT>(a.colptr, a.csc_pos, a.dsv, a.g.H, a.n_cols, a.col_hub, a.colsum, a.ld_colsum, 0, s);
        return launch_sums<HT>(a.colptr, a.csc_pos, a.dsv, a.g.H, a.n_cols, a.col_hub, a.dP2, a.ldd2, a.g.Dt4 * 4, s);
    }
    return 0;
}

template <int NCH>
int launch_split_n(const BwdSplitArgs& a, cudaStream_t s) {
    if (a.g.H == 1) return launch_split_t<NCH, 1>(a, s);
    if (a.g.H == 2) return launch_split_t<NCH, 2>(a, s);
    return launch_split_t<NCH, 4>(a, s);
}

}

int launch_edge_bwd_split(const BwdSplitArgs& a, cudaStream_t s) {
    switch ((a.g.Wd4 + 31) / 32) {
        case 1: return launch_split_n<1>(a, s);
        case 2: return launch_split_n<2>(a, s);
        case 3: return launch_split_n<3>(a, s);
        case 4: return launch_split_n<4>(a, s);
        default: set_error("edge_bwd_split: row width %d floats exceeds the supported 512", a.g.Wd4 * 4); return 2;
    }
}

}
```

recon_b200/csrc/spk_edge_fwd.cu:

```cuda
#include "spk_edge.cuh"
#include "spk_stream.cuh"
#include <stdlib.h>

namespace spk {

__device__ __forceinline__ float elu1(float x) {
    const float big = exp2f(x * 1.4426950408889634f) - 1.0f;
    const float small = x * (1.0f + x * (0.5f + x * (0.16666667f + x * (0.041666668f + x * 0.0083333338f))));
    const float neg = x > -0.125f ? small : big;
    return x > 0.f ? x : neg;
}

template <int NCH, int HT>
struct FwdAcc {
    float4 acc[NCH];
    float den[HT];
    float sw[HT];
};

template <int NCH, int HT, bool HAS2>
__device__ __forceinline__ void fwd_accumulate(const EdgeFwdArgs& a, int row, int beg, int end, int lane,
                                               const int (&hc)[NCH], FwdAcc<NCH, HT>& st, bool& bad) {
    constexpr int U = (NCH <= 2) ? 4 : 2;
    const int H = a.g.H, Wd4 = a.g.Wd4;
// ... 6 lines not shown

    for (int base = beg; base < end; base += 32) {
        const int n = min(32, end - base);
        int my_col = 0, my_t1 = 0, my_t2 = -1;
        float my_m[HT];
#pragma unroll
        for (int h = 0; h < HT; ++h) my_m[h] = 1.f;
        if (lane < n) {
            my_col = __ldg(a.col + base + lane);
            my_t1 = __ldg(a.t1 + base + lane);
            if (HAS2) my_t2 = __ldg(a.t2 + base + lane);
            if (has_mask) {
#pragma unroll
                for (int h = 0; h < HT; ++h)
                    if (h < H) my_m[h] = __ldg(a.mask + (long)h * a.mask_stride + base + lane);
            }
        }
        for (int u0 = 0; u0 < n; u0 += U) {
            float4 v[U][NCH];
#pragma unroll
            for (int u = 0; u < U; ++u) {
                const int idx = u0 + u;
                const int j = __shfl_sync(0xffffffffu, my_col, idx & 31);
                const int k1 = __shfl_sync(0xffffffffu, my_t1, idx & 31);
                int k2 = -1;
                if (HAS2) k2 = __shfl_sync(0xffffffffu, my_t2, idx & 31);
                const float* p2 = a.P2 + (long)j * a.ld2;
                const float* p3 = a.P3 + (long)k1 * a.ld3;
                const float* p3b = a.P3 + (long)(k2 < 0 ? 0 : k2) * a.ld3;
#pragma unroll
                for (int ci = 0; ci < NCH; ++ci) {
                    const int c4 = lane + 32 * ci;
                    float4 x = make_float4(0.f, 0.f, 0.f, 0.f);
                    if (idx < n && c4 < Wd4) {
                        x = f4add(ldg4(p2 + c4 * 4), ldg4(p3 + c4 * 4));
                        if (HAS2 && k2 >= 0) x = f4add(x, ldg4(p3b + c4 * 4));
                    }
                    v[u][ci] = x;
                }
            }
#pragma unroll
            for (int u = 0; u < U; ++u) {
                const int idx = u0 + u;
                if (idx >= n) break;
                float4 qv = v[u][0];
#pragma unroll
                for (int ci = 1; ci < NCH; ++ci)
                    if (qci == ci) qv = v[u][ci];
                float w[HT];
#pragma unroll
                for (int h = 0; h < HT; ++h) {
                    w[h] = 0.f;
                    if (h < H) {
                        const float s = q1[h] + __shfl_sync(0xffffffffu, f4get(qv, h), qlane);
                        const float ee = expf(-(s > 0.f ? s : a.alpha * s));
                        bad |= (ee != ee);
                        st.den[h] += ee;
                        float m = 1.f;
                        if (has_mask) m = __shfl_sync(0xffffffffu, my_m[h], idx & 31);
                        w[h] = ee * m;
                        st.sw[h] += w[h];
                    }
                }
#pragma unroll
                for (int ci = 0; ci < NCH; ++ci) f4fma(st.acc[ci], selh<HT>(hc[ci], w), v[u][ci]);
            }
        }
    }
}

template <int NCH, int HT>
__device__ __forceinline__ void fwd_init(const LayerGeom& g, int lane, int (&hc)[NCH], FwdAcc<NCH, HT>& st) {
#pragma unroll
    for (int ci = 0; ci < NCH; ++ci) {
        const int c4 = lane + 32 * ci;
        hc[ci] = (HT > 1 && c4 < g.Dt4) ? c4 / g.Dp4 : 0;
        st.acc[ci] = make_float4(0.f, 0.f, 0.f, 0.f);
    }
#pragma unroll
    for (int h = 0; h < HT; ++h) st.den[h] = st.sw[h] = 0.f;
}

template <int NCH, int HT>
__device__ __forceinline__ void fwd_finalize(const EdgeFwdArgs& a, int row, int lane, const int (&hc)[NCH],
                                             FwdAcc<NCH, HT>& st, bool& bad, uint32_t p1_smem = 0) {
    const LayerGeom g = a.g;
    float rden[HT];
#pragma unroll
    for (int h = 0; h < HT; ++h) {
        if (st.den[h] == 0.f) st.den[h] = 1e-12f;
        rden[h] = 1.0f / st.den[h];
    }
#pragma unroll
    for (int ci = 0; ci < NCH; ++ci) {
        const int c4 = lane + 32 * ci;
        if (c4 >= g.Dt4) continue;
        const int h = hc[ci];
        const float d = selh<HT>(h, rden);
        const float s = selh<HT>(h, st.sw);
        const float4 p1 = p1_smem ? lds4(p1_smem + c4 * 16) : ldg4(a.P1 + (long)row * a.ld1 + c4 * 4);
        float o[4] = {fmaf(s, p1.x, st.acc[ci].x), fmaf(s, p1.y, st.acc[ci].y),
                      fmaf(s, p1.z, st.acc[ci].z), fmaf(s, p1.w, st.acc[ci].w)};
#pragma unroll
        for (int k = 0; k < 4; ++k) {
            o[k] = o[k] * d;
            bad |= (o[k] != o[k]);
            if (a.apply_elu && row < a.elu_rows) o[k] = elu1(o[k]);
        }
        const int off = (c4 - h * g.Dp4) * 4;
        float* dst = a.out + (long)row * a.ldo + (long)h * g.D + off;
        if (a.out_vec) {
            *reinterpret_cast<float4*>(dst) = make_float4(o[0], o[1], o[2], o[3]);
        } else {
#pragma unroll
            for (int k = 0; k < 4; ++k)
                if (off + k < g.D) dst[k] = o[k];
        }
    }
    if (lane < g.H) {
        a.den[(long)row * g.H + lane] = selh<HT>(lane, st.den);
        a.sw[(long)row * g.H + lane] = selh<HT>(lane, st.sw);
    }
}


template <int NCH, int HT>
__device__ __forceinline__ void fwd_zero_row(const EdgeFwdArgs& a, int row, int lane) {
    const LayerGeom g = a.g;
    const int hd = g.H * g.D;
    float* dst = a.out + (long)row * a.ldo;
    for (int c = lane; c < hd; c += 32) dst[c] = 0.f;
    if (lane < g.H) { a.den[(long)row * g.H + lane] = 1e-12f; a.sw[(long)row * g.H + lane] = 0.f; }
}

template <int NCH, int HT, bool HAS2>
__global__ void __launch_bounds__(SPK_CTA_THREADS, (NCH <= 2) ? 3 : 2)
edge_fwd_rows_kernel(const EdgeFwdArgs a) {
    const int lane = threadIdx.x & 31;
    const int row = blockIdx.x * SPK_WARPS_PER_CTA + (threadIdx.x >> 5);
    if (row >= a.n_rows) return;
    const int beg = __ldg(a.segptr + row), end = __ldg(a.segptr + row + 1);
    if (end - beg > a.hub.hub_thresh) return;
    int hc[NCH];
    FwdAcc<NCH, HT> st;
    bool bad = false;
    fwd_init<NCH, HT>(a.g, lane, hc, st);
    fwd_accumulate<NCH, HT, HAS2>(a, row, beg, end, lane, hc, st, bad);
    fwd_finalize<NCH, HT>(a, row, lane, hc, st, bad);
    if (__any_sync(0xffffffffu, bad) && lane == 0) atomicOr(a.nanflag, 1);
}

template <int NCH, int HT, bool HAS2>
__global__ void __launch_bounds__(SPK_CTA_THREADS, (NCH <= 2) ? 3 : 2)
edge_fwd_tasks_kernel(const EdgeFwdArgs a) {
    const int lane = threadIdx.x & 31;
    const int task = blockIdx.x * SPK_WARPS_PER_CTA + (threadIdx.x >> 5);
    if (task >= a.hub.n_tasks) return;
    const int row = __ldg(a.hub.task_seg + task);
    int hc[NCH];
    FwdAcc<NCH, HT> st;
    bool bad = false;
    fwd_init<NCH, HT>(a.g, lane, hc, st);
    fwd_accumulate<NCH, HT, HAS2>(a, row, __ldg(a.hub.task_beg + task), __ldg(a.hub.task_end + task), lane, hc, st, bad);
    float* part = a.hub.partial + (long)task * a.hub.ldpart;
#pragma unroll
    for (int ci = 0; ci < NCH; ++ci) {
        const int c4 = lane + 32 * ci;
        if (c4 < a.g.Wd4) *reinterpret_cast<float4*>(part + c4 * 4) = st.acc[ci];
    }
    if (lane < SPK_MAX_HEADS) {
        part[a.g.Wd4 * 4 + lane] = lane < HT ? selh<HT>(lane, st.den) : 0.f;
        part[a.g.Wd4 * 4 + SPK_MAX_HEADS + lane] = lane < HT ? selh<HT>(lane, st.sw) : 0.f;
    }
    if (__any_sync(0xffffffffu, bad) && lane == 0) atomicOr(a.nanflag, 1);
}

template <int NCH> struct FinCfg { static constexpr int NW = (NCH <= 2) ? 32 : 16; };

template <int NCH, int HT>
__global__ void __launch_bounds__(FinCfg<NCH>::NW * 32)
edge_fwd_hub_finalize_kernel(const EdgeFwdArgs a) {
    __shared__ __align__(16) float red[FinCfg<NCH>::NW][NCH * 128 + 2 * SPK_MAX_HEADS];
    const int lane = threadIdx.x & 31, wid = threadIdx.x >> 5;
    const int hub = blockIdx.x;
    const int row = __ldg(a.hub.hub_seg + hub);
    const int t0 = __ldg(a.hub.hub_task_ptr + hub), t1 = __ldg(a.hub.hub_task_ptr + hub + 1);
    const int len = a.g.Wd4 * 4 + 2 * SPK_MAX_HEADS;
    cta_sum_partials<NCH * 4 + 1, FinCfg<NCH>::NW>(a.hub.partial, a.hub.ldpart, t0, t1, len, &red[0][0], NCH * 128 + 2 * SPK_MAX_HEADS);
    if (wid != 0) return;
    int hc[NCH];
    FwdAcc<NCH, HT> st;
    bool bad = false;
    fwd_init<NCH, HT>(a.g, lane, hc, st);
#pragma unroll
    for (int ci = 0; ci < NCH; ++ci) {
        const int c4 = lane + 32 * ci;
        if (c4 < a.g.Wd4) st.acc[ci] = *reinterpret_cast<const float4*>(&red[0][c4 * 4]);
    }
#pragma unroll
    for (int h = 0; h < HT; ++h) {
        st.den[h] = red[0][a.g.Wd4 * 4 + h];
        st.sw[h] = red[0][a.g.Wd4 * 4 + SPK_MAX_HEADS + h];
    }
    fwd_finalize<NCH, HT>(a, row, lane, hc, st, bad);
    if (__any_sync(0xffffffffu, bad) && lane == 0) atomicOr(a.nanflag, 1);
}


constexpr int STREAM_WARPS = 8;
constexpr int STREAM_G = 2;
template <int NCH, bool HAS2> struct StreamCfg { static constexpr int NG = (NCH <= 2) ? (HAS2 ? 2 : 3) : 2; };

template <int HT>
struct IdxBatch { int col, t1, t2; float m[HT]; };

// ... 25 lines not shown
    long row0 = 0;
    int task_row = 0;
    if (!TASKS) {
        row0 = ((long)blockIdx.x * STREAM_WARPS + wid) * 32;
        const long r = row0 + lane;
        if (r < a.n_rows) {
            const int b = __ldg(a.segptr + r), e = __ldg(a.segptr + r + 1);
            st.beg = b;
            if (e - b > a.hub.hub_thresh) is_hub = true; else st.deg = e - b;
        }
    } else {
        const int task = blockIdx.x * STREAM_WARPS + wid;
        if (task >= a.hub.n_tasks) return;
        task_row = __ldg(a.hub.task_seg + task);
        if (lane == 0) { st.beg = __ldg(a.hub.task_beg + task); st.deg = __ldg(a.hub.task_end + task) - st.beg; }
    }
    st.pre = warp_excl_scan(st.deg, lane, st.total);
    const int T = st.total;
    const bool has_mask = a.mask != nullptr;
    const long qoff = (long)g.Dt4 * 4;

    bool bad = false;
    float4 q1v = make_float4(0.f, 0.f, 0.f, 0.f);
    if (!TASKS) { if (st.deg > 0) q1v = ldg4(a.P1 + (row0 + lane) * a.ld1 + qoff); }
    else q1v = ldg4(a.P1 + (long)task_row * a.ld1 + qoff);
    IdxBatch<HT> cur, nxt;
    auto load_batch = [&](int nb0, IdxBatch<HT>& b) {
        b.col = 0; b.t1 = 0; b.t2 = -1;
#pragma unroll
        for (int h = 0; h < HT; ++h) b.m[h] = 1.f;
        if (nb0 >= T) return;
        const int m = nb0 + lane;
        int seg;
        const int e = st.entry_of(m < T ? m : T - 1, seg);
        if (m < T) {
            b.col = __ldg(a.col + e);
            b.t1 = __ldg(a.t1 + e);
            if (HAS2) b.t2 = __ldg(a.t2 + e);
            if (has_mask) {
#pragma unroll
                for (int h = 0; h < HT; ++h)
                    if (h < H) b.m[h] = __ldg(a.mask + (long)h * a.mask_stride + e);
            }
        }
    };
    load_batch(0, cur);
    load_batch(32, nxt);
    int nb = 0;
    auto issue_group = [&](int n0) {
        const int n = n0 + lane;
        const int d = n - nb, src = d & 31;
        const int jc = __shfl_sync(0xffffffffu, cur.col, src), jn = __shfl_sync(0xffffffffu, nxt.col, src);
        const int kc = __shfl_sync(0xffffffffu, cur.t1, src), kn = __shfl_sync(0xffffffffu, nxt.t1, src);
        int k2 = -1;
        if (HAS2) {
            const int k2c = __shfl_sync(0xffffffffu, cur.t2, src), k2n = __shfl_sync(0xffffffffu, nxt.t2, src);
            k2 = d < 32 ? k2c : k2n;
        }
        const bool mine = lane < G && n < T;
        const uint32_t bar = bars + 8u * ((n0 / G) % NG);
        unsigned n3 = 0;
        if (HAS2) n3 = __popc(__ballot_sync(0xffffffffu, mine && k2 >= 0));
        if (lane == 0) {
            const int cnt = T - n0 < G ? T - n0 : G;
            sbar_expect(bar, (uint32_t)cnt * 2u * row_bytes + n3 * row_bytes);
        }
        if (mine) {
            const int j = d < 32 ? jc : jn, k1 = d < 32 ? kc : kn;
            const uint32_t slot = wbase + (uint32_t)(n % S) * slot_bytes;
            bulk_g2s(slot, a.P2 + (long)j * a.ld2, row_bytes, bar);
            bulk_g2s(slot + row_bytes, a.P3 + (long)k1 * a.ld3, row_bytes, bar);
            if (HAS2 && k2 >= 0) bulk_g2s(slot + 2u * row_bytes, a.P3 + (long)k2 * a.ld3, row_bytes, bar);
        }
    };
    for (int gi = 0; gi < NG && gi * G < T; ++gi) issue_group(gi * G);

    unsigned act = TASKS ? 1u : __ballot_sync(0xffffffffu, st.deg > 0);
    if (!TASKS) {
        unsigned empt = __ballot_sync(0xffffffffu, st.deg == 0 && !is_hub && row0 + lane < a.n_rows);
        while (empt) { const int r = __ffs(empt) - 1; empt &= empt - 1; fwd_zero_row<NCH, HT>(a, (int)(row0 + r), lane); }
    }
    unsigned rem = TASKS ? 0u : act;
    int pk = 0;
    auto issue_p1 = [&]() {
        if (!rem) return;
        const int r = __ffs(rem) - 1;
        rem &= rem - 1;
        if (lane == 0) {
            const uint32_t bar = bars + 8u * (NG + (pk & 1));
            sbar_expect(bar, row_bytes);
            bulk_g2s(p1buf + (uint32_t)(pk & 1) * row_bytes, a.P1 + (row0 + r) * a.ld1, row_bytes, bar);
        }
        ++pk;
    };
    issue_p1();
    issue_p1();

    int hc[NCH];
    bool cvalid[NCH];
    uint32_t coff[NCH];
#pragma unroll
    for (int ci = 0; ci < NCH; ++ci) { cvalid[ci] = lane + 32 * ci < g.Wd4; coff[ci] = (uint32_t)(lane + 32 * ci) * 16u; }
    FwdAcc<NCH, HT> acc;
    fwd_init<NCH, HT>(g, lane, hc, acc);
    int ak = 0;
    int r = TASKS ? 0 : __ffs(act) - 1;
    act &= act - 1;
    int row_end = T ? __shfl_sync(0xffffffffu, st.pre + st.deg, r < 0 ? 0 : r) : 0;
    float q1[HT];
#pragma unroll
    for (int h = 0; h < HT; ++h) q1[h] = TASKS ? f4get(q1v, h) : __shfl_sync(0xffffffffu, f4get(q1v, h), r < 0 ? 0 : r);
    const uint32_t qo = (uint32_t)g.Dt4 * 16u;

    for (int n0 = 0; n0 < T; n0 += G) {
        if (n0 - nb == 32) { cur = nxt; nb += 32; load_batch(nb + 32, nxt); }
        const int grp = (n0 / G) % NG;
        sbar_wait(bars + 8u * grp, (uint32_t)(n0 / S) & 1u);
#pragma unroll
        for (int u = 0; u < G; ++u) {
            const int n = n0 + u;
            if (n >= T) break;
            const uint32_t slot = wbase + (uint32_t)(grp * G + u) * slot_bytes;
            const int src = n - nb;
            int k2 = -1;
            if (HAS2) k2 = __shfl_sync(0xffffffffu, cur.t2, src);
            float4 v[NCH];
#pragma unroll
            for (int ci = 0; ci < NCH; ++ci) {
                float4 x = make_float4(0.f, 0.f, 0.f, 0.f);
                if (cvalid[ci]) {
                    x = f4add(lds4(slot + coff[ci]), lds4(slot + row_bytes + coff[ci]));
                    if (HAS2 && k2 >= 0) x = f4add(x, lds4(slot + 2u * row_bytes + coff[ci]));
                }
                v[ci] = x;
            }
            float4 qq = f4add(lds4(slot + qo), lds4(slot + row_bytes + qo));
            if (HAS2 && k2 >= 0) qq = f4add(qq, lds4(slot + 2u * row_bytes + qo));
            float w[HT];
#pragma unroll
            for (int h = 0; h < HT; ++h) {
                w[h] = 0.f;
                if (h < H) {
                    const float sc = q1[h] + f4get(qq, h);
                    const float ee = fast_exp(-(sc > 0.f ? sc : a.alpha * sc));
                    bad |= (ee != ee);
                    acc.den[h] += ee;
                    w[h] = has_mask ? ee * __shfl_sync(0xffffffffu, cur.m[h], src) : ee;
                    acc.sw[h] += w[h];
                }
            }
#pragma unroll
            for (int ci = 0; ci < NCH; ++ci) f4fma(acc.acc[ci], selh<HT>(hc[ci], w), v[ci]);
            if (!TASKS && n + 1 == row_end) {
                const uint32_t pb = p1buf + (uint32_t)(ak & 1) * row_bytes;
                sbar_wait(bars + 8u * (NG + (ak & 1)), (uint32_t)(ak >> 1) & 1u);
                fwd_finalize<NCH, HT>(a, (int)(row0 + r), lane, hc, acc, bad, pb);
                __syncwarp();
                issue_p1();
                ++ak;
                fwd_init<NCH, HT>(g, lane, hc, acc);
                if (act) {
                    r = __ffs(act) - 1;
                    act &= act - 1;
                    row_end = __shfl_sync(0xffffffffu, st.pre + st.deg, r);
#pragma unroll
                    for (int h = 0; h < HT; ++h) q1[h] = __shfl_sync(0xffffffffu, f4get(q1v, h), r);
                }
            }
        }
        __syncwarp();
        if (n0 + S < T) issue_group(n0 + S);
    }
    if (TASKS) {
        const int task = blockIdx.x * STREAM_WARPS + wid;
// ... 112 lines not shown
```

recon_b200/csrc/spk_stream.cuh:

```cuda
#pragma once
#include "spk_common.cuh"

namespace spk {

__device__ __forceinline__ uint32_t smem_addr(const void* p) { return (uint32_t)__cvta_generic_to_shared(p); }

__device__ __forceinline__ void sbar_init(uint32_t bar, uint32_t count) {
    asm volatile("mbarrier.init.shared::cta.b64 [%0], %1;" ::"r"(bar), "r"(count) : "memory");
}
__device__ __forceinline__ void sbar_expect(uint32_t bar, uint32_t bytes) {
    asm volatile("mbarrier.arrive.expect_tx.shared::cta.b64 _, [%0], %1;" ::"r"(bar), "r"(bytes) : "memory");
}
__device__ __forceinline__ void sbar_wait(uint32_t bar, uint32_t parity) {
    asm volatile(
        "{\n\t"
        ".reg .pred P1;\n\t"
        "SW_WAIT:\n\t"
        "mbarrier.try_wait.parity.shared::cta.b64 P1, [%0], %1;\n\t"
        "@P1 bra SW_DONE;\n\t"
        "bra SW_WAIT;\n\t"
        "SW_DONE:\n\t"
        "}" ::"r"(bar), "r"(parity) : "memory");
}
__device__ __forceinline__ void bulk_g2s(uint32_t dst, const void* src, uint32_t bytes, uint32_t bar) {
    asm volatile("cp.async.bulk.shared::cluster.global.mbarrier::complete_tx::bytes [%0], [%1], %2, [%3];"
                 ::"r"(dst), "l"(src), "r"(bytes), "r"(bar) : "memory");
}
__device__ __forceinline__ float4 lds4(uint32_t addr) {
    float4 v;
    asm volatile("ld.shared.v4.f32 {%0,%1,%2,%3}, [%4];" : "=f"(v.x), "=f"(v.y), "=f"(v.z), "=f"(v.w) : "r"(addr));
    return v;
}

__device__ __forceinline__ int warp_excl_scan(int v, int lane, int& total) {
    int inc = v;
#pragma unroll
    for (int o = 1; o < 32; o <<= 1) {
        const int t = __shfl_up_sync(0xffffffffu, inc, o);
        if (lane >= o) inc += t;
    }
    total = __shfl_sync(0xffffffffu, inc, 31);
    return inc - v;
}

struct SegTable {
    int beg, deg, pre, total;
    __device__ __forceinline__ int entry_of(int m, int& seg) const {
        int lo = 0, hi = 31;
#pragma unroll
        for (int it = 0; it < 5; ++it) {
            const int mid = (lo + hi + 1) >> 1;
            const int pm = __shfl_sync(0xffffffffu, pre, mid);
            if (pm <= m) lo = mid; else hi = mid - 1;
        }
        seg = lo;
        return __shfl_sync(0xffffffffu, beg, lo) + (m - __shfl_sync(0xffffffffu, pre, lo));
    }
};

}
```

recon_b200/functional.py:

```python
import ctypes as C
import os
import weakref

import torch

from . import _lib
from .graph import KGraph

MAX_HEADS = 4
USE_TC = True
TC_MIN_ROWS = 1


WD_ALIGN = int(os.environ.get("SPK_WD_ALIGN", "8"))


class Geometry:

    def __init__(self, n_heads, d_head):
        assert 1 <= n_heads <= MAX_HEADS
        self.H, self.D = n_heads, d_head
        self.Dp = (d_head + 3) // 4 * 4
        self.Dt = self.H * self.Dp
        self.Wd = (self.Dt + self.H + WD_ALIGN - 1) // WD_ALIGN * WD_ALIGN
# ... 126 lines not shown


def gemm_tn(A, B, out=None, accumulate=False):
    assert A.dim() == 2 and B.dim() == 2 and A.shape[0] == B.shape[0]
    assert A.stride(1) == 1 and B.stride(1) == 1
    M, Ka = A.shape
    Nb = B.shape[1]
    lib = _lib.load()
    if out is None:
        assert not accumulate
        out = torch.empty(Ka, Nb, dtype=torch.float32, device=A.device)
    if Ka and Nb:
        if lib.timing is not None:
            _lib.current_tag = f"{M}x{Ka}x{Nb}"
        if USE_TC and M >= TC_MIN_ROWS and lib.spk_gemm_tn_tc_supported(_lib.ptr(A), A.stride(0), _lib.ptr(B), B.stride(0),
                                                                        M, Ka, Nb):
            ws = torch.empty(max(1, lib.spk_gemm_tn_tc_workspace_floats(M, Ka, Nb)), dtype=torch.float32, device=A.device)
            _lib.check(lib.spk_gemm_tn_tc(_lib.ptr(A), A.stride(0), _lib.ptr(B), B.stride(0), _lib.ptr(out),
                                          out.stride(0), M, Ka, Nb, int(accumulate), _lib.ptr(ws), _lib.stream_ptr()),
                       "gemm_tn_tc")
        else:
            ws = torch.empty(max(1, lib.spk_gemm_tn_workspace_floats(M, Ka, Nb)), dtype=torch.float32, device=A.device)
            _lib.check(lib.spk_gemm_tn(_lib.ptr(A), A.stride(0), _lib.ptr(B), B.stride(0), _lib.ptr(out), out.stride(0),
                                       M, Ka, Nb, int(accumulate), _lib.ptr(ws), _lib.stream_ptr()), "gemm_tn")
    return out


def tc_friendly(X):
    if X.dim() != 2 or X.stride(1) != 1 or X.stride(0) % 4 == 0 or not USE_TC:
        return X
    f = X.shape[1]
    Xp = X.new_zeros(X.shape[0], (f + 3) // 4 * 4)
    Xp[:, :f] = X
    return Xp[:, :f]


_X_TABLE = {"key": None, "table": None}


def _x_key(X):
    return (X.data_ptr(), X._version, tuple(X.shape), tuple(X.stride()), str(X.device))


def _tma_operand(X):
    if _X_TABLE["key"] is not None and _X_TABLE["key"] == _x_key(X) and USE_TC:
        t = _X_TABLE["table"]()
        _X_TABLE["key"] = _X_TABLE["table"] = None
        if t is not None:
            return t[:, :X.shape[1]]
    return tc_friendly(X.contiguous())


class MatMulFn(torch.autograd.Function):

    @staticmethod
    def forward(ctx, X, W, dist=None):
        X = _tma_operand(X); W = W.contiguous()
        ctx.save_for_backward(X, W)
        ctx.dist = dist
        return gemm_nn(X, W)

    @staticmethod
    def backward(ctx, g):
        X, W = ctx.saved_tensors
        g = g.contiguous()
        dX = gemm_nn(g, W.t().contiguous()) if ctx.needs_input_grad[0] else None
        dW = gemm_tn(X, g) if ctx.needs_input_grad[1] else None
        if dW is not None and ctx.dist is not None:
            ctx.dist.all_reduce(dW)
        return dX, dW, None


def matmul(X, W, dist=None):
    return MatMulFn.apply(X, W, dist)



def _hub_partial(hubs, ldpart, device):
    if hubs is None or hubs.n_tasks == 0:
        return None
    return torch.empty(hubs.n_tasks, ldpart, dtype=torch.float32, device=device)


def edge_attn_forward(graph, P1, P2, P3, geom, alpha, apply_elu, mask_csr, nanflag, elu_rows=0):
    lib = _lib.load()
    n = graph.n_nodes
    dev = P1.device
    out = torch.empty(n, geom.H * geom.D, dtype=torch.float32, device=dev)
    den = torch.empty(n, geom.H, dtype=torch.float32, device=dev)
    sw = torch.empty(n, geom.H, dtype=torch.float32, device=dev)
    a = _lib.EdgeFwdArgs()
    a.segptr = graph.rowptr.data_ptr(); a.col = graph.col.data_ptr(); a.t1 = graph.t1.data_ptr()
    a.t2 = graph.t2.data_ptr() if graph.t2 is not None else None
    a.P1 = P1.data_ptr(); a.ld1 = P1.stride(0)
    a.P2 = P2.data_ptr(); a.ld2 = P2.stride(0)
    a.P3 = P3.data_ptr(); a.ld3 = P3.stride(0)
    if mask_csr is not None:
        a.mask = mask_csr.data_ptr(); a.mask_stride = mask_csr.stride(0)
    a.out = out.data_ptr(); a.ldo = out.stride(0); a.den = den.data_ptr(); a.sw = sw.data_ptr()
    a.nanflag = nanflag.data_ptr()
    a.n_rows = n; a.apply_elu = int(apply_elu); a.alpha = float(alpha); a.elu_rows = int(elu_rows)
    a.geom = geom.struct()
    ldpart = geom.Wd + 2 * MAX_HEADS
    partial = _hub_partial(graph.row_hubs, ldpart, dev)
    graph.row_hubs.fill(a.hub, partial, ldpart)
    _lib.check(lib.spk_edge_attn_fwd(C.byref(a), _lib.stream_ptr()), "edge_attn_fwd")
    return out, den, sw


BWD_MODE = os.environ.get("SPK_BWD_MODE", "split")


def _fill_fused_args(f, graph, P1, P2, P3, geom, alpha, apply_elu, mask_csr, out, dout, den, sw, G, ldg, rowsc, dP1, dP2, rec):
    f.rowptr = graph.rowptr.data_ptr()
    f.colptr = graph.colptr.data_ptr(); f.csc_row = graph.csc_row.data_ptr(); f.csc_pos = graph.csc_pos.data_ptr()
    f.csc_t1 = graph.csc_t1.data_ptr(); f.csc_t2 = graph.csc_t2.data_ptr() if graph.csc_t2 is not None else None
    f.P1 = P1.data_ptr(); f.ld1 = P1.stride(0); f.P2 = P2.data_ptr(); f.ld2 = P2.stride(0)
    f.P3 = P3.data_ptr(); f.ld3 = P3.stride(0)
    if mask_csr is not None:
        f.mask = mask_csr.data_ptr(); f.mask_stride = mask_csr.stride(0)
    f.out = out.data_ptr(); f.dout = dout.data_ptr(); f.ldo = out.stride(0)
    assert dout.stride(0) == out.stride(0)
    f.den = den.data_ptr(); f.sw = sw.data_ptr()
    f.G = G.data_ptr(); f.ldg = ldg; f.rowsc = rowsc.data_ptr()
    f.dP1 = dP1.data_ptr(); f.ldd1 = dP1.stride(0); f.dP2 = dP2.data_ptr(); f.ldd2 = dP2.stride(0)
    f.rec = rec.data_ptr() if rec is not None else None
    f.n_rows = graph.n_nodes; f.n_cols = graph.n_cols; f.apply_elu = int(apply_elu); f.alpha = float(alpha)
    f.geom = geom.struct()
    graph.row_hubs.fill(f.row_hub, None, 0)
    part = _hub_partial(graph.col_hubs, geom.Wd, P1.device)
    graph.col_hubs.fill(f.col_hub, part, geom.Wd)
    return part


def edge_attn_backward(graph, P1, P2, P3, geom, alpha, apply_elu, mask_csr, out, dout, den, sw, dP1, dP2, dP3,
                       after_columns=None, colsum=None):
    lib = _lib.load()
    graph.build_backward()
    n, dev = graph.n_nodes, P1.device
    ldg = _row_stride(geom.Dt, G_ALIGN)
    G = torch.empty(n, ldg, dtype=torch.float32, device=dev)
    mode = BWD_MODE if sw is not None else "rows"
    if mode == "split" and graph.t2 is not None:
        mode = "rows"
    ne = max(1, graph.n_edges)
    if mode == "split":
        q = _lib.EdgeBwdSplitArgs()
        rowsc = torch.empty(max(1, n), geom.H, 4, dtype=torch.float32, device=dev)
        rec4 = torch.empty(ne, geom.H, 4, dtype=torch.float32, device=dev)
        dsv = torch.empty(ne, geom.H, dtype=torch.float32, device=dev)
        keep = _fill_fused_args(q.base, graph, P1, P2, P3, geom, alpha, apply_elu, mask_csr, out, dout, den, sw, G, ldg,
                                rowsc, dP1, dP2, None)
        q.relptr = graph.relptr.data_ptr(); q.rel_row = graph.rel_row.data_ptr(); q.rel_pos = graph.rel_pos.data_ptr()
        q.rec4 = rec4.data_ptr(); q.dsv = dsv.data_ptr()
        q.dP3 = dP3.data_ptr(); q.ldd3 = dP3.stride(0); q.n_rel = graph.n_rel
        part3 = _hub_partial(graph.rel_hubs, geom.Wd, dev)
        graph.rel_hubs.fill(q.rel_hub, part3, geom.Wd)
        part1 = _hub_partial(graph.row_hubs, 4, dev)
        graph.row_hubs.fill(q.base.row_hub, part1, 4)
        if after_columns is None:
            if lib.timing is None:
                _lib.check(lib.spk_edge_attn_bwd_split(C.byref(q), _lib.stream_ptr()), "edge_attn_bwd_split")
            else:
                for ph, tag in ((1, "node"), (2, "cols"), (4, "rels"), (8, "colsums")):
                    q.phases = ph
                    _lib.current_tag = tag
                    _lib.check(lib.spk_edge_attn_bwd_split(C.byref(q), _lib.stream_ptr()), "edge_attn_bwd_split")
                _lib.current_tag = ""
            del keep, part3, part1
            return False
        q.phases = 3
        _lib.current_tag = "node+cols"
        _lib.check(lib.spk_edge_attn_bwd_split(C.byref(q), _lib.stream_ptr()), "edge_attn_bwd_split")
        after_columns()
        q.phases = 12
        q.colsum = colsum.data_ptr(); q.ld_colsum = colsum.stride(0)
        _lib.current_tag = "rels+sums"
        _lib.check(lib.spk_edge_attn_bwd_split(C.byref(q), _lib.stream_ptr()), "edge_attn_bwd_split")
        _lib.current_tag = ""
        del keep, part3, part1
        return True
    rec = torch.empty(ne, 2 * geom.H, dtype=torch.float32, device=dev)
    if mode == "fused":
        f = _lib.EdgeBwdFusedArgs()
        rowsc = torch.empty(max(1, n), geom.H, 4, dtype=torch.float32, device=dev)
        keep = _fill_fused_args(f, graph, P1, P2, P3, geom, alpha, apply_elu, mask_csr, out, dout, den, sw, G, ldg, rowsc,
                                dP1, dP2, rec)
        _lib.check(lib.spk_edge_attn_bwd_fused(C.byref(f), _lib.stream_ptr()), "edge_attn_bwd_fused")
        del keep
        seg_gather(graph.relptr, graph.rel_row, graph.rel_pos, graph.rel_hubs, G, ldg, rec, geom, dP3, graph.n_rel, "rels")
        return False
    a = _lib.EdgeBwdRowsArgs()
    a.segptr = graph.rowptr.data_ptr(); a.col = graph.col.data_ptr(); a.t1 = graph.t1.data_ptr()
    a.t2 = graph.t2.data_ptr() if graph.t2 is not None else None
    a.P1 = P1.data_ptr(); a.ld1 = P1.stride(0)
    a.P2 = P2.data_ptr(); a.ld2 = P2.stride(0)
    a.P3 = P3.data_ptr(); a.ld3 = P3.stride(0)
    if mask_csr is not None:
        a.mask = mask_csr.data_ptr(); a.mask_stride = mask_csr.stride(0)
    a.out = out.data_ptr(); a.dout = dout.data_ptr(); a.ldo = out.stride(0)
    assert dout.stride(0) == out.stride(0)
    a.den = den.data_ptr()
    a.G = G.data_ptr(); a.ldg = ldg; a.dP1 = dP1.data_ptr(); a.ldd1 = dP1.stride(0); a.rec = rec.data_ptr()
    a.n_rows = n; a.apply_elu = int(apply_elu); a.alpha = float(alpha)
    a.geom = geom.struct()
    part_a = _hub_partial(graph.row_hubs, 2 * MAX_HEADS, dev)
    graph.row_hubs.fill(a.hub, part_a, 2 * MAX_HEADS)
    _lib.check(lib.spk_edge_attn_bwd_rows(C.byref(a), _lib.stream_ptr()), "edge_attn_bwd_rows")

    seg_gather(graph.colptr, graph.csc_row, graph.csc_pos, graph.col_hubs, G, ldg, rec, geom, dP2, graph.n_cols, "cols")
    seg_gather(graph.relptr, graph.rel_row, graph.rel_pos, graph.rel_hubs, G, ldg, rec, geom, dP3, graph.n_rel, "rels")
    return False


def seg_gather(ptr, src, pos, hubs, G, ldg, rec, geom, dst, n_seg, tag):
    s = _lib.SegGatherArgs()
    s.segptr = ptr.data_ptr(); s.src = src.data_ptr(); s.pos = pos.data_ptr()
    s.G = G.data_ptr(); s.ldg = ldg; s.rec = rec.data_ptr()
    s.out = dst.data_ptr(); s.ldout = dst.stride(0); s.n_seg = n_seg
    s.flags = 1 if (n_seg > 0 and src.numel() < 5 * n_seg) else 0
    s.geom = geom.struct()
    part = _hub_partial(hubs, geom.Wd, G.device)
    hubs.fill(s.hub, part, geom.Wd)
    _lib.current_tag = f"{tag}:w{geom.Wd}"
    try:
        _lib.check(_lib.load().spk_edge_attn_bwd_segments(C.byref(s), _lib.stream_ptr()), "edge_attn_bwd_segments")
    finally:
        _lib.current_tag = ""


def _ghost_combine(ghost, vals, den, sw, n, H):
    ng = ghost.n
    W = vals.shape[1] // H
    v = vals[n:].view(ng, H, W)
    d = den[n:]
    d0 = torch.where(sw[n:] == 0, torch.zeros_like(d), d)
    buf = torch.cat(((v * d0.unsqueeze(-1)).reshape(ng, H * W), d0), dim=1)
    ghost.sum_partials(buf)
    dg = buf[:, H * W:]
    dg = torch.where(dg == 0, torch.full_like(dg, 1e-12), dg)
    vals[n:] = (buf[:, :H * W].view(ng, H, W) / dg.unsqueeze(-1)).reshape(ng, H * W)
    den[n:] = dg


def _ghost_dout(ghost, dout, n, n_ext):
    ext = torch.empty(n_ext, dout.shape[1], dtype=dout.dtype, device=dout.device)
    ext[:n] = dout
    ext[n:] = ghost.gather_rows(dout)
    ext[ghost.mine_local] = 0
    return ext


class AttentionGroupFn(torch.autograd.Function):

    @staticmethod
    def forward(ctx, X, Wn, Rel, Wr, graph, geom, alpha, apply_elu, mask_csr, nanflag):
        X = tc_friendly(X.contiguous()); Wn = Wn.contiguous(); Rel = Rel.contiguous(); Wr = Wr.contiguous()
        dist = getattr(graph, "dist", None)
        ghost = dist.ghost if dist is not None else None
        Wd = geom.Wd
        mode = "local"
        X_all = None
        if dist is None:
            P3 = gemm_nn(Rel, Wr)
            P = gemm_nn(X, Wn)
            P1, P2 = P[:, :Wd], P[:, Wd:]
        elif 2 * X.shape[1] <= Wd:
            mode = "input"
            Fp = (X.shape[1] + 3) // 4 * 4
            X_all, mine = dist.gather_buffer(Fp, X.device)
            mine[:, :X.shape[1]].copy_(X)
            if Fp != X.shape[1]:
                mine[:, X.shape[1]:].zero_()
            h = dist.all_gather_start(X_all)
            P3 = gemm_nn(Rel, Wr)
            P1 = gemm_nn(X, Wn[:, :Wd])
            h.wait()
            X_all = X_all[:, :X.shape[1]]
            P2 = gemm_nn(X_all, Wn[:, Wd:])
        else:
            mode = "proj"
            P2, mine = dist.gather_buffer(Wd, X.device)
            gemm_nn(X, Wn[:, Wd:], out=mine)
            h = dist.all_gather_start(P2)
            n = X.shape[0]
            if ghost is None:
                P1 = gemm_nn(X, Wn[:, :Wd])
            else:
                P1 = torch.empty(n + ghost.n, Wd, dtype=torch.float32, device=X.device)
                gemm_nn(X, Wn[:, :Wd], out=P1[:n])
                gemm_nn(tc_friendly(ghost.gather_rows(X)), Wn[:, :Wd], out=P1[n:])
            P3 = gemm_nn(Rel, Wr)
            h.wait()
        if ghost is not None and mode != "proj":
            raise NotImplementedError("hub rows split across ranks need the projected exchange (or the aggregate-then-project path)")
        if ghost is None:
            out, den, sw = edge_attn_forward(graph, P1, P2, P3, geom, alpha, apply_elu, mask_csr, nanflag)
            out_ret = out
        else:
            n = X.shape[0]
            k_elu = bool(apply_elu) and n > 0
            out, den, sw = edge_attn_forward(graph, P1, P2, P3, geom, alpha, k_elu, mask_csr, nanflag, elu_rows=n if k_elu else 0)
            _ghost_combine(ghost, out, den, sw, n, geom.H)
            nanflag.bitwise_or_(torch.isnan(out[n:]).any().to(torch.int32))
            if apply_elu and out.shape[0] > n:
                tail = out[n:]
                _lib.check(_lib.load().spk_elu_inplace(_lib.ptr(tail), tail.stride(0), tail.shape[0], tail.shape[1],
                                                       _lib.stream_ptr()), "elu_inplace")
            out[ghost.mine_local] = out[n:][ghost.mine]
            out_ret = out[:n]
        ctx.save_for_backward(X, Wn, Rel, Wr, P1, P2, P3, out, den, sw, X_all if X_all is not None else X.new_empty(0))
        ctx.graph, ctx.geom, ctx.alpha, ctx.apply_elu, ctx.mask_csr, ctx.mode = graph, geom, alpha, apply_elu, mask_csr, mode
        ctx.mark_non_differentiable(den, sw)
        return out_ret, den, sw

    @staticmethod
    def backward(ctx, dout, _dden, _dsw):
        geom, graph, mode = ctx.geom, ctx.graph, ctx.mode
        dist = getattr(graph, "dist", None)
        X, Wn, Rel, Wr, P1, P2, P3, out, den, sw, X_all = ctx.saved_tensors
        Wd = geom.Wd
        dout = dout.contiguous()
        n = X.shape[0]
        dev = X.device
        dP3 = torch.empty_like(P3)
        WnT = Wn.t().contiguous()
        need_x, need_w = ctx.needs_input_grad[0], ctx.needs_input_grad[1]
        dX = dWn = None
        if mode == "local":
            dP = torch.empty(n, 2 * Wd, dtype=torch.float32, device=dev)
            edge_attn_backward(graph, P1, P2, P3, geom, ctx.alpha, ctx.apply_elu, ctx.mask_csr, out, dout, den, sw,
                               dP[:, :Wd], dP[:, Wd:], dP3)
            if need_x:
                dX = gemm_nn(dP, WnT)
            if need_w:
                dWn = gemm_tn(X, dP)
        else:
            mr = dist.part.max_rows
            ghost = dist.ghost
            n_ext = n + (ghost.n if ghost is not None else 0)
            if ghost is not None:
                dout = _ghost_dout(ghost, dout, n, n_ext)
            dP1 = torch.empty(n_ext, Wd, dtype=torch.float32, device=dev)
            dP2_all = torch.empty_like(P2)
            colsum = torch.empty(P2.shape[0], geom.H, dtype=torch.float32, device=dev)
            pend = {}

            def start_main():
                if mode == "proj":
                    pend["pad"] = torch.empty(mr, Wd, dtype=torch.float32, device=dev)
                    pend["h"] = dist.reduce_scatter_start(dP2_all, pend["pad"])

            split = edge_attn_backward(graph, P1, P2, P3, geom, ctx.alpha, ctx.apply_elu, ctx.mask_csr, out, dout, den, sw,
                                       dP1, dP2_all, dP3, after_columns=start_main if mode == "proj" else None, colsum=colsum)
            if mode == "proj":
                if split:
                    qs_pad = torch.empty(mr, geom.H, dtype=torch.float32, device=dev)
                    hq = dist.reduce_scatter_start(colsum, qs_pad)
                else:
                    start_main()
                h3 = dist.all_reduce_start(dP3)
                if ghost is not None:
                    gsum = ghost.sum_partials(dP1[n:].contiguous())
                    dP1[ghost.mine_local] = gsum[ghost.mine]
                    dP1 = dP1[:n]
                if need_x:
                    dX = gemm_nn(dP1, WnT[:Wd])
                if need_w:
                    dWn = torch.empty_like(Wn)
                    gemm_tn(X, dP1, out=dWn[:, :Wd])
                pend["h"].wait()
                dP2 = pend["pad"][:n]
                if split:
                    hq.wait()
                    dP2[:, geom.Dt:geom.Dt + geom.H].copy_(qs_pad[:n])
                del dP2_all
                if need_x:
                    gemm_nn(dP2, WnT[Wd:], out=dX, accumulate=True)
                if need_w:
                    gemm_tn(X, dP2, out=dWn[:, Wd:])
                    dist.all_reduce(dWn)
                h3.wait()
            else:
                h3 = dist.all_reduce_start(dP3)
                F = X.shape[1]
                Fp = (F + 3) // 4 * 4
                if need_x:
                    dX2_all = torch.empty(P2.shape[0], Fp, dtype=torch.float32, device=dev)
                    gemm_nn(dP2_all, WnT[Wd:], out=dX2_all[:, :F])
                    if Fp != F:
                        dX2_all[:, F:].zero_()
                    pad = torch.empty(mr, Fp, dtype=torch.float32, device=dev)
                    h = dist.reduce_scatter_start(dX2_all, pad)
                    dX1 = gemm_nn(dP1, WnT[:Wd])
                    h.wait()
                    dX = dX1.add_(pad[:n, :F])
                    del dX2_all
                if need_w:
                    dWn = torch.empty_like(Wn)
                    gemm_tn(X, dP1, out=dWn[:, :Wd])
                    gemm_tn(X_all, dP2_all, out=dWn[:, Wd:])
                    dist.all_reduce(dWn)
                h3.wait()
        dRel = gemm_nn(dP3, Wr.t().contiguous()) if ctx.needs_input_grad[2] else None
        dWr = gemm_tn(Rel, dP3) if ctx.needs_input_grad[3] else None
        return dX, dWn, dRel, dWr, None, None, None, None, None, None



AGG_MODE = "auto"
AGG_BWD_MODE = os.environ.get("SPK_AGG_BWD_MODE", "split")
AGG_MAX_HEADS = 2


G_ALIGN = int(os.environ.get("SPK_G_ALIGN", "8"))
GX_ALIGN = int(os.environ.get("SPK_GX_ALIGN", "8"))
LX_ALIGN = int(os.environ.get("SPK_LX_ALIGN", "8"))


def _row_stride(width, align):
    return (width + align - 1) // align * align


class AggGeometry:

    def __init__(self, n_heads, in_features, nrela_dim, d_head):
        self.H, self.F, self.Rd, self.D = n_heads, in_features, nrela_dim, d_head
        self.Fx4, self.Fr4 = (in_features + 3) // 4, (nrela_dim + 3) // 4
        self.Fp, self.Rp = 4 * self.Fx4, 4 * self.Fr4
        self.LX = _row_stride(self.Fp + 4, LX_ALIGN)
        self.LR = _row_stride(self.Rp + 4, LX_ALIGN)
        self.LZ = 2 * self.Fp + self.Rp

    @staticmethod
    def supported(n_heads, in_features, nrela_dim):
        return 1 <= n_heads <= AGG_MAX_HEADS and 1 <= in_features <= 60 and 1 <= nrela_dim <= 60

    def struct(self):
        return _lib.AggGeom(self.H, self.Fx4, self.Fr4, self.LZ)


def use_agg_path(n_heads, in_features, nrela_dim, d_head, graph):
    if AGG_MODE == "off" or (getattr(graph, "dist", None) is None and graph.n_cols != graph.n_nodes):
        return False
    if not AggGeometry.supported(n_heads, in_features, nrela_dim):
        return False
    if AGG_MODE == "force":
        return True
    g = AggGeometry(n_heads, in_features, nrela_dim, d_head)
    return g.LX + g.LR < n_heads * d_head


def agg_weights(a_list, a2_list, geom):
    if _on_library(list(a_list) + list(a2_list)):
        dims = dict(F=geom.F, Rd=geom.Rd, D=geom.D, Fp=geom.Fp, LZ=geom.LZ)
        return AttnWeightsFn.apply(1, dims, *a_list, *a2_list)
    return _agg_weights_torch(a_list, a2_list, geom)


def _agg_weights_torch(a_list, a2_list, geom):
    F, Rd, Fp = geom.F, geom.Rd, geom.Fp
    a0 = a_list[0]
    Wa = a0.new_zeros(geom.H, geom.LZ, geom.D)
    V = a0.new_zeros(F, 4)
    V3 = a0.new_zeros(Rd, 4)
    for h, (a, a2) in enumerate(zip(a_list, a2_list)):
        at = a.t()
        qa = (at * a2).sum(dim=1)
        Wa[h, :F] = at[:F]
        Wa[h, Fp:Fp + F] = at[F:2 * F]
        Wa[h, 2 * Fp:2 * Fp + Rd] = at[2 * F:]
        V[:, 2 + h] = qa[:F]
        V[:, h] = qa[F:2 * F]
        V3[:, h] = qa[2 * F:]
    return Wa, V, V3


def _agg_table(X, V, ld, chunks, out=None):
    T = torch.empty(X.shape[0], ld, dtype=torch.float32, device=X.device) if out is None else out
    assert T.shape[0] == X.shape[0] and T.stride(1) == 1 and T.stride(0) >= ld
    ld = T.stride(0)
    if X.shape[0]:
        _lib.check(_lib.load().spk_agg_table(_lib.ptr(X), X.stride(0), _lib.ptr(V), _lib.ptr(T), ld, X.shape[0],
                                             X.shape[1], chunks, _lib.stream_ptr()), "agg_table")
    return T


class AggGroupFn(torch.autograd.Function):

# ... 127 lines not shown
            rowsum = torch.empty(max(1, n), H, **f32)
            q.rowsum = rowsum.data_ptr(); q.ld_rowsum = H
            q.G_rel = Gr.data_ptr(); q.ldg_rel = Gr.stride(0)
            q.dup = 1

            def run(phases, tag):
                q.phases = phases
                _lib.current_tag = tag + f":w{gx_geom.Wd}"
                try:
                    _lib.check(lib.spk_edge_attn_bwd_split(C.byref(q), _lib.stream_ptr()), "edge_attn_bwd_split")
                finally:
                    _lib.current_tag = ""
        else:
            rec = torch.empty(max(1, graph.n_edges), 2 * H, **f32)
            a.segptr = graph.rowptr.data_ptr(); a.col = graph.col.data_ptr(); a.t1 = graph.t1.data_ptr()
            a.t2 = graph.t2.data_ptr() if graph.t2 is not None else None
            a.xcol = Xc.data_ptr(); a.ldxc = Xc.stride(0)
            a.rel = Rt.data_ptr(); a.ldr = Rt.stride(0)
            if ctx.mask_csr is not None:
                a.mask = ctx.mask_csr.data_ptr(); a.mask_stride = ctx.mask_csr.stride(0)
            rowsc = torch.empty(max(1, n), 8, **f32)
            a.rowsc = rowsc.data_ptr(); a.rec = rec.data_ptr()
            part = _hub_partial(graph.row_hubs, 8, dev)
            graph.row_hubs.fill(a.hub, part, 8)
            _lib.check(lib.spk_agg_bwd_rows(C.byref(a), _lib.stream_ptr()), "agg_bwd_rows")
            del dZ
        if split:
            run(2, "cols")
        else:
            seg_gather(graph.colptr, graph.csc_row, graph.csc_pos, graph.col_hubs, Gx, Gx.stride(0), rec, gx_geom, dXc,
                       graph.n_cols, "cols")
        if dist is not None:
            dXc_all = dXc
            dXc_pad = torch.empty(dist.part.max_rows, gx_geom.Wd, **f32)
            hx = dist.reduce_scatter_start(dXc_all, dXc_pad)
        if split:
            run(4, "rels")
            rowout[:, Fp:Fp + H] = rowsum[:n]
            if dist is not None:
                colsum = torch.empty(graph.n_cols, H, **f32)
                q.colsum = colsum.data_ptr(); q.ld_colsum = H
            run(8, "colsums")
            if dist is not None:
                qs_pad = torch.empty(dist.part.max_rows, H, **f32)
                hq = dist.reduce_scatter_start(colsum, qs_pad)
        else:
            seg_gather(graph.relptr, graph.rel_row, graph.rel_pos, graph.rel_hubs, Gr, Gr.stride(0), rec, gr_geom, dRc,
                       graph.n_rel, "rels")
        if dist is not None:
            dist.all_reduce(dRc)
            dist.all_reduce(dWa)
            if ghost is not None:
                gsum = ghost.sum_partials(rowout[n_loc:].contiguous())
                rowout[ghost.mine_local] = gsum[ghost.mine]
            hx.wait()
            dXc = dXc_pad[:n_loc]
            del dXc_all
            if split:
                hq.wait()
                dXc[:, H * Fp:H * Fp + H].copy_(qs_pad[:n_loc])
        n = n_loc
        dX = torch.empty(n, geom.F, **f32)
        dq = torch.empty(n, 4, **f32)
        _lib.check(lib.spk_agg_dx(_lib.ptr(rowout), rowout.stride(0), _lib.ptr(dXc), dXc.stride(0), _lib.ptr(V), n,
                                  geom.F, geom.Fx4, H, _lib.ptr(dX), dX.stride(0), _lib.ptr(dq), _lib.stream_ptr()),
                   "agg_dx")
        dV = gemm_tn(Xt[:n, :geom.F], dq) if ctx.needs_input_grad[3] else None
        if dV is not None and dist is not None:
            dist.all_reduce(dV)
        dq3 = dRc[:, H * Rp:H * Rp + H].contiguous()
        dRel = None
        if ctx.needs_input_grad[1]:
            dRel = dRc[:, :geom.Rd].clone()
            for h in range(1, H):
                dRel += dRc[:, h * Rp:h * Rp + geom.Rd]
            dRel = gemm_nn(dq3, V3[:, :H].t().contiguous(), out=dRel, accumulate=True)
        dV3 = None
        if ctx.needs_input_grad[4]:
            dV3 = torch.zeros_like(V3)
            dV3[:, :H] = gemm_tn(Rel, dq3)
        return dX, dRel, dWa, dV, dV3, None, None, None, None, None, None


def attention_group(X, Rel, a_list, a2_list, graph, alpha, apply_elu, mask_csr, nanflag):
    outs = []
    if X.shape[0] != graph.n_nodes - getattr(graph, "n_ghost", 0):
        raise IndexError(f"entity table has {X.shape[0]} rows but the graph was built for "
                         f"{graph.n_nodes - getattr(graph, 'n_ghost', 0)} nodes")
    if getattr(graph, "dist", None) is None and graph.n_cols > X.shape[0]:
        raise IndexError(f"graph gathers from {graph.n_cols} nodes but the entity table has {X.shape[0]} rows")
    if Rel.shape[0] < graph.n_rel:
        raise IndexError(f"relation table has {Rel.shape[0]} rows but the graph uses {graph.n_rel} relations")
    if X.device != graph.device or Rel.device != graph.device:
        raise RuntimeError(f"tables on {X.device} / {Rel.device} but the graph layouts live on {graph.device}")
    F = X.shape[1]
    D = a_list[0].shape[0]
    Rd = a_list[0].shape[1] - 2 * F
    if use_agg_path(min(len(a_list), AGG_MAX_HEADS), F, Rd, D, graph):
        for g0 in range(0, len(a_list), AGG_MAX_HEADS):
            al, a2l = a_list[g0:g0 + AGG_MAX_HEADS], a2_list[g0:g0 + AGG_MAX_HEADS]
            geom = AggGeometry(len(al), F, Rd, D)
            Wa, V, V3 = agg_weights(al, a2l, geom)
            m = None if mask_csr is None else mask_csr[g0:g0 + AGG_MAX_HEADS].contiguous()
            outs.append(AggGroupFn.apply(X, Rel, Wa, V, V3, graph, geom, alpha, apply_elu, m, nanflag))
        return outs[0] if len(outs) == 1 else torch.cat(outs, dim=1)
    for g0 in range(0, len(a_list), MAX_HEADS):
        al, a2l = a_list[g0:g0 + MAX_HEADS], a2_list[g0:g0 + MAX_HEADS]
        geom = Geometry(len(al), D)
        Wn, Wr = extended_weights(al, a2l, F, geom)
        m = None if mask_csr is None else mask_csr[g0:g0 + MAX_HEADS].contiguous()
        out, _, _ = AttentionGroupFn.apply(X, Wn, Rel, Wr, graph, geom, alpha, apply_elu, m, nanflag)
        outs.append(out)
    return outs[0] if len(outs) == 1 else torch.cat(outs, dim=1)



def rownorm_(x):
    assert x.dim() == 2 and x.stride(1) == 1
    _lib.check(_lib.load().spk_rownorm(_lib.ptr(x), x.stride(0), _lib.ptr(x), x.stride(0), x.shape[0], x.shape[1],
                                       _lib.stream_ptr()), "rownorm")
    return x


def rownorm(x):
    x = x.contiguous()
    y = torch.empty_like(x)
    _lib.check(_lib.load().spk_rownorm(_lib.ptr(x), x.stride(0), _lib.ptr(y), y.stride(0), x.shape[0], x.shape[1],
                                       _lib.stream_ptr()), "rownorm")
    return y


def mask_from_index(idx, n_rows, device, flag=None):
    mask = torch.zeros(n_rows, dtype=torch.float32, device=device)
    if idx.numel() and not idx.is_cuda:
        if int(idx.min()) < -n_rows or int(idx.max()) >= n_rows:
            raise IndexError("batch_entities index out of range")
    idx = idx.to(device=device, dtype=torch.int64).contiguous()
    if idx.numel():
        own = flag is None
        if own:
            flag = torch.zeros(1, dtype=torch.int32, device=device)
        _lib.check(_lib.load().spk_mask_from_index(_lib.ptr(idx), idx.numel(), _lib.ptr(mask), n_rows, _lib.ptr(flag),
                                                   _lib.stream_ptr()), "mask_from_index")
        if own and int(flag.item()) & 2:
            raise IndexError("batch_entities index out of range")
    return mask


class ResidualNormFn(torch.autograd.Function):

    @staticmethod
    def forward(ctx, EW, x2, mask):
        EW = EW.contiguous(); x2 = x2.contiguous()
        n, w = EW.shape
        out = torch.empty_like(EW)
        inv = torch.empty(n, dtype=torch.float32, device=EW.device)
        _lib.check(_lib.load().spk_residual_norm_fwd(_lib.ptr(EW), EW.stride(0), _lib.ptr(x2), x2.stride(0),
                                                     _lib.ptr(mask), _lib.ptr(out), out.stride(0), _lib.ptr(inv),
                                                     n, w, _lib.stream_ptr()), "residual_norm_fwd")
        ctx.save_for_backward(out, mask, inv)
        return out

    @staticmethod
    def backward(ctx, g):
        out, mask, inv = ctx.saved_tensors
        g = g.contiguous()
        n, w = out.shape
        dew = torch.empty_like(out)
        dx2 = torch.empty_like(out)
        _lib.check(_lib.load().spk_residual_norm_bwd(_lib.ptr(g), g.stride(0), _lib.ptr(out), out.stride(0),
                                                     _lib.ptr(mask), _lib.ptr(inv), _lib.ptr(dew), dew.stride(0),
                                                     _lib.ptr(dx2), dx2.stride(0), n, w, _lib.stream_ptr()),
                   "residual_norm_bwd")
        return dew, dx2, None



class InnerProductFn(torch.autograd.Function):

    @staticmethod
    def forward(ctx, *tensors):
# ... 33 lines not shown
```

recon_b200/models.py:

```python
import torch
import torch.nn as nn

from . import functional as SF
from .graph import KGraph
from .layers import SpGraphAttentionLayer, ConvKB, check_nanflag, edge_dropout_mask


def _fingerprint(t):
    if t.is_cuda or t.numel() == 0:
        return None
    flat = t.reshape(-1)
    n = flat.numel()
    return tuple(int(flat[i]) for i in sorted({0, n // 3, n // 2, (2 * n) // 3, n - 1}))


def _nhop_rows(edge_list_nhop, edge_type_nhop):
    if edge_type_nhop is None or edge_type_nhop.numel() == 0:
        return None
    el = edge_list_nhop.long()
    et = edge_type_nhop.long().to(el.device)
    return torch.stack((el[1], et[:, 0], et[:, 1], el[0]), dim=1)


class SpGAT(nn.Module):
    def __init__(self, num_nodes, nfeat, nhid, relation_dim, dropout, alpha, nheads):
        super().__init__()
        self.dropout = dropout
        self.alpha = alpha
        self.dropout_layer = nn.Dropout(self.dropout)
        self.attentions = [SpGraphAttentionLayer(num_nodes, nfeat, nhid, relation_dim, dropout=dropout,
                                                 alpha=alpha, concat=True) for _ in range(nheads)]
        for i, attention in enumerate(self.attentions):
            self.add_module('attention_{}'.format(i), attention)
        self.W = nn.Parameter(torch.zeros(size=(relation_dim, nheads * nhid)))
        nn.init.xavier_uniform_(self.W.data, gain=1.414)
        self.out_att = SpGraphAttentionLayer(num_nodes, nhid * nheads, nheads * nhid, nheads * nhid,
                                             dropout=dropout, alpha=alpha, concat=False)

    def forward(self, Corpus_, entity_embeddings, relation_embed, edge_list, edge_type, edge_embed,
                edge_list_nhop, edge_type_nhop, graph=None, dropout_masks=None, nanflag=None):
        x = entity_embeddings
        if not x.is_cuda:
            raise RuntimeError("recon_b200.SpGAT needs CUDA tensors (no CPU fallback)")
        dev = x.device
        with torch.cuda.device(dev):
            return self._forward(x, relation_embed, edge_list, edge_type, edge_list_nhop, edge_type_nhop, graph,
                                 dropout_masks, nanflag)

    def _forward(self, x, relation_embed, edge_list, edge_type, edge_list_nhop, edge_type_nhop, graph, dropout_masks, nanflag):
        dev = x.device
        if graph is None:
            graph = KGraph(edge_list, edge_type, _nhop_rows(edge_list_nhop, edge_type_nhop), x.shape[0],
                           relation_embed.shape[0], device=dev)
        own_flag = nanflag is None
        if own_flag:
            nanflag = torch.zeros(1, dtype=torch.int32, device=dev)
        nheads = len(self.attentions)
        e = graph.n_edges
        p = self.dropout
        m_att = m_out = m_x = None
        if dropout_masks is not None:
            if dropout_masks.get("att") is not None:
                m_att = graph.to_csr_order(dropout_masks["att"].to(dev, torch.float32).reshape(nheads, e))
            if dropout_masks.get("out") is not None:
                m_out = graph.to_csr_order(dropout_masks["out"].to(dev, torch.float32).reshape(1, e))
            if dropout_masks.get("x") is not None:
                m_x = dropout_masks["x"].to(dev, torch.float32)
        elif self.training and p > 0:
            m_att = edge_dropout_mask(p, nheads, e, dev)
            m_out = edge_dropout_mask(p, 1, e, dev)
            m_x = (torch.rand(x.shape[0], nheads * self.attentions[0].out_features, device=dev) >= p).float().mul_(1.0 / (1.0 - p))

        x = SF.attention_group(x, relation_embed, [att.a for att in self.attentions],
                               [att.a_2 for att in self.attentions], graph, self.alpha, True, m_att, nanflag)
        if m_x is not None:
            x = x * m_x
        out_relation_1 = SF.matmul(relation_embed, self.W)
        x = SF.attention_group(x, out_relation_1, [self.out_att.a], [self.out_att.a_2], graph, self.alpha,
                               True, m_out, nanflag)
        if own_flag:
            check_nanflag(nanflag)
        return x, out_relation_1


class SpKBGATModified(nn.Module):
    def __init__(self, initial_entity_emb, initial_relation_emb, entity_out_dim, relation_out_dim,
                 drop_GAT, alpha, nheads_GAT, initial_entity_emb_params=None, *, sep_space=False):
        super().__init__()
        self.num_nodes = initial_entity_emb.shape[0]
        self.entity_in_dim = initial_entity_emb.shape[1]
        self.entity_out_dim_1 = entity_out_dim[0]
        self.nheads_GAT_1 = nheads_GAT[0]
        self.entity_out_dim_2 = entity_out_dim[1]
        self.nheads_GAT_2 = nheads_GAT[1]
        self.num_relation = initial_relation_emb.shape[0]
        self.relation_dim = initial_relation_emb.shape[1]
        self.relation_out_dim_1 = relation_out_dim[0]
        self.drop_GAT = drop_GAT
        self.alpha = alpha
        hd = self.entity_out_dim_1 * self.nheads_GAT_1
        self.final_entity_embeddings = nn.Parameter(torch.randn(self.num_nodes, hd))
        self.final_relation_embeddings = nn.Parameter(torch.randn(self.num_relation, hd))
        self.entity_embeddings = nn.Parameter(initial_entity_emb)
        self.relation_embeddings = nn.Parameter(initial_relation_emb)
        self.sparse_gat_1 = SpGAT(self.num_nodes, self.entity_in_dim, self.entity_out_dim_1, self.relation_dim,
                                  self.drop_GAT, self.alpha, self.nheads_GAT_1)
        self.W_entities = nn.Parameter(torch.zeros(size=(self.entity_in_dim, hd)))
        nn.init.xavier_uniform_(self.W_entities.data, gain=1.414)
        self.nonlinearity_ent2rel = torch.tanh
        if sep_space:
            self.W_ent2rel = nn.Parameter(torch.zeros(size=(self.num_relation, hd, hd)))
            nn.init.xavier_uniform_(self.W_ent2rel.data, gain=1.414)
        self._graph_cache = {}
        self.graph_cache = True

    def load_state_dict(self, state_dict, strict=True, **kw):
        has = "W_ent2rel" in self._parameters
        if "W_ent2rel" in state_dict and not has:
            w = state_dict["W_ent2rel"]
            self.W_ent2rel = nn.Parameter(torch.empty_like(w, device=self.W_entities.device))
        elif has and "W_ent2rel" not in state_dict:
            state_dict = dict(state_dict)
            state_dict["W_ent2rel"] = self.W_ent2rel.detach()
        return super().load_state_dict(state_dict, strict=strict, **kw)

    def _graph_key(self, adj, train_indices_nhop):
        edge_list, edge_type = adj[0], adj[1]
        has2 = train_indices_nhop is not None and train_indices_nhop.numel() > 0
        tensors = (edge_list, edge_type, train_indices_nhop) if has2 else (edge_list, edge_type)
        dev = self.entity_embeddings.device
        return (str(dev),) + tuple((t.data_ptr(), tuple(t.shape), t._version, str(t.device), _fingerprint(t)) for t in tensors)

    def _graph_is_cached(self, adj, train_indices_nhop):
        if isinstance(adj, KGraph):
            return True
        return bool(self.graph_cache) and self._graph_key(adj, train_indices_nhop) in self._graph_cache

    def prepare_graph(self, adj, train_indices_nhop=None):
        if isinstance(adj, KGraph):
            return adj
        edge_list, edge_type = adj[0], adj[1]
        has2 = train_indices_nhop is not None and train_indices_nhop.numel() > 0
        dev = self.entity_embeddings.device
        if dev.type != "cuda":
            raise RuntimeError("recon_b200.SpKBGATModified must live on a CUDA device (no CPU fallback)")
        key = self._graph_key(adj, train_indices_nhop)
        g = self._graph_cache.get(key) if self.graph_cache else None
        if g is None:
            nhop = train_indices_nhop if has2 else None
            with torch.cuda.device(dev):
                g = KGraph(edge_list, edge_type, nhop, self.num_nodes, self.num_relation, device=dev)
            self._graph_cache.clear()
            if self.graph_cache:
                self._graph_cache[key] = g
                g._keepalive = (edge_list, edge_type, train_indices_nhop)
        return g

    def _run(self, entity_embeddings, relation_embeddings, batch_entities, graph, dropout_masks, entities_upgraded=None):
        with torch.cuda.device(entity_embeddings.device):
            return self._run_on(entity_embeddings, relation_embeddings, batch_entities, graph, dropout_masks, entities_upgraded)

    def _run_on(self, entity_embeddings, relation_embeddings, batch_entities, graph, dropout_masks, entities_upgraded=None):
        dev = entity_embeddings.device
        nanflag = torch.zeros(1, dtype=torch.int32, device=dev)
        out_entity_1, out_relation_1 = self.sparse_gat_1(
            None, entity_embeddings, relation_embeddings, None, None, None, None, None,
            graph=graph, dropout_masks=dropout_masks, nanflag=nanflag)
        mask = SF.mask_from_index(torch.as_tensor(batch_entities), entity_embeddings.shape[0], dev, flag=nanflag)
        if entities_upgraded is None:
            entities_upgraded = SF.matmul(entity_embeddings, self.W_entities, getattr(graph, "dist", None))
        out_entity_1 = SF.ResidualNormFn.apply(entities_upgraded, out_entity_1, mask)
        check_nanflag(nanflag)
        return out_entity_1, out_relation_1, mask

    def forward(self, Corpus_, batch_entities, adj, train_indices_nhop, dropout_masks=None):
        if self.entity_embeddings.device.type != "cuda":
            raise RuntimeError("recon_b200.SpKBGATModified must live on a CUDA device (no CPU fallback)")
        pre = None
        with torch.cuda.device(self.entity_embeddings.device):
            self.entity_embeddings.data = SF.rownorm(self.entity_embeddings.data)
            if not self._graph_is_cached(adj, train_indices_nhop):
                pre = SF.matmul(self.entity_embeddings, self.W_entities, None)
        graph = self.prepare_graph(adj, train_indices_nhop)
        out_entity_1, out_relation_1, mask = self._run(self.entity_embeddings, self.relation_embeddings,
                                                       batch_entities, graph, dropout_masks, pre)
        self.final_entity_embeddings.data = out_entity_1.data
        self.final_relation_embeddings.data = out_relation_1.data
        return out_entity_1, out_relation_1, mask

    def batch_test(self, Corpus_, batch_entities, adj, train_indices_nhop, entity_embeddings, dropout_masks=None):
        graph = self.prepare_graph(adj, train_indices_nhop)
        relation_embeddings = self.relation_embeddings.detach()
        entity_embeddings = SF.rownorm(entity_embeddings.data.to(self.W_entities.device))
        return self._run(entity_embeddings, relation_embeddings, batch_entities, graph, dropout_masks)
```

Before: 509.9 million.

## Fuse residual add and row normalization into edge attention forward and backward kernels

Adds residual variants of the edge-attention forward kernel and the split backward kernel. They compute the masked residual-plus-normalize step (and its gradient) inside the node kernels instead of running a separate ResidualNormFn pass. The model now routes the residual through attention_group when the conditions hold: not the agg path, split backward mode, no 2-hop edges, not distributed. This removes extra kernel launches and global memory round trips of the output, in exchange for more code paths and extra register pressure in the node kernels.

```diff
diff --git a/include/spkbgat.h b/include/spkbgat.h
--- a/include/spkbgat.h
+++ b/include/spkbgat.h
@@ -8,7 +8,7 @@
 
 typedef void* spk_stream_t;
 
-#define SPK_ABI_VERSION 6
+#define SPK_ABI_VERSION 7
 int spk_abi_version(void);
 const char* spk_last_error(void);
 int64_t spk_launch_count(void);
@@ -87,6 +87,16 @@
 int spk_edge_attn_fwd(const spk_edge_fwd_args* args, spk_stream_t stream);
 
 typedef struct {
+    const float* ew; int64_t lde;
+    const float* mask;
+    float* out; int64_t ldo;
+    float* inv;
+    const float* g; int64_t ldg;
+    float* dew; int64_t ldd;
+} spk_residual_args;
+int spk_edge_attn_fwd_residual(const spk_edge_fwd_args* args, const spk_residual_args* res, spk_stream_t stream);
+
+typedef struct {
     const int32_t* segptr; const int32_t* col; const int32_t* t1; const int32_t* t2;
     const float* P1; int64_t ld1;
     const float* P2; int64_t ld2;
@@ -149,6 +159,7 @@
     int32_t dup; int32_t reserved;
 } spk_edge_bwd_split_args;
 int spk_edge_attn_bwd_split(const spk_edge_bwd_split_args* args, spk_stream_t stream);
+int spk_edge_attn_bwd_split_residual(const spk_edge_bwd_split_args* args, const spk_residual_args* res, spk_stream_t stream);
 
 typedef struct {
     int32_t n_heads;
diff --git a/recon_b200/_lib.py b/recon_b200/_lib.py
--- a/recon_b200/_lib.py
+++ b/recon_b200/_lib.py
@@ -9,7 +9,7 @@
 c_i32p = C.POINTER(C.c_int32)
 c_i64p = C.POINTER(C.c_int64)
 c_f32p = C.POINTER(C.c_float)
-ABI_VERSION = 6
+ABI_VERSION = 7
 
 
 class Geom(C.Structure):
@@ -83,6 +83,11 @@
                 ("rowsum", C.c_void_p), ("ld_rowsum", C.c_int64),
                 ("G_rel", C.c_void_p), ("ldg_rel", C.c_int64),
                 ("dup", C.c_int32), ("reserved", C.c_int32)]
+
+
+class ResidualArgs(C.Structure):
+    _fields_ = [("ew", C.c_void_p), ("lde", C.c_int64), ("mask", C.c_void_p), ("out", C.c_void_p), ("ldo", C.c_int64),
+                ("inv", C.c_void_p), ("g", C.c_void_p), ("ldg", C.c_int64), ("dew", C.c_void_p), ("ldd", C.c_int64)]
 
 
 class AggGeom(C.Structure):
@@ -178,10 +183,12 @@
     "spk_gemm_tn_workspace_floats": (_I64, [_I64, _I32, _I32]),
     "spk_gemm_tn": (_I32, [_VP, _I64, _VP, _I64, _VP, _I64, _I64, _I32, _I32, _I32, _VP, _VP]),
     "spk_edge_attn_fwd": (_I32, [C.POINTER(EdgeFwdArgs), _VP]),
+    "spk_edge_attn_fwd_residual": (_I32, [C.POINTER(EdgeFwdArgs), C.POINTER(ResidualArgs), _VP]),
     "spk_edge_attn_bwd_rows": (_I32, [C.POINTER(EdgeBwdRowsArgs), _VP]),
     "spk_edge_attn_bwd_segments": (_I32, [C.POINTER(SegGatherArgs), _VP]),
     "spk_edge_attn_bwd_fused": (_I32, [C.POINTER(EdgeBwdFusedArgs), _VP]),
     "spk_edge_attn_bwd_split": (_I32, [C.POINTER(EdgeBwdSplitArgs), _VP]),
+    "spk_edge_attn_bwd_split_residual": (_I32, [C.POINTER(EdgeBwdSplitArgs), C.POINTER(ResidualArgs), _VP]),
     "spk_spmm_rowsum_fwd": (_I32, [_VP, _VP, _VP, _I64, _I32, _VP, _I64, _I32, _VP]),
     "spk_spmm_rowsum_bwd": (_I32, [_VP, _VP, _I64, _I32, _VP, _I64, _I64, _VP]),
     "spk_rownorm": (_I32, [_VP, _I64, _VP, _I64, _I64, _I32, _VP]),
@@ -219,6 +226,7 @@
 
 _lib = None
 current_tag = ""
+TIMING_NAMES = {"spk_edge_attn_fwd_residual": "edge_attn_fwd", "spk_edge_attn_bwd_split_residual": "edge_attn_bwd_split"}
 
 
 class _Lib:
@@ -239,7 +247,7 @@
             rc = fn(*args)
             e1.record()
             global current_tag
-            self.timing.append((name[4:] + (":" + current_tag if current_tag else ""), e0, e1))
+            self.timing.append((TIMING_NAMES.get(name, name[4:]) + (":" + current_tag if current_tag else ""), e0, e1))
             if "gemm" in name:
                 current_tag = ""
             return rc
diff --git a/recon_b200/csrc/spk_api.cu b/recon_b200/csrc/spk_api.cu
--- a/recon_b200/csrc/spk_api.cu
+++ b/recon_b200/csrc/spk_api.cu
@@ -167,8 +167,8 @@
     return gemm_tn_tc(A, lda, B, ldb, C, ldc, M, Ka, Nb, accumulate, workspace, (cudaStream_t)stream);
 }
 
-int spk_edge_attn_fwd(const spk_edge_fwd_args* p, spk_stream_t stream) {
-    EdgeFwdArgs a;
+static int edge_fwd_args_of(const spk_edge_fwd_args* p, EdgeFwdArgs& a) {
+    a.res = ResidualArgs{};
     if (!geom_ok(p->geom, &a.g, "edge_attn_fwd")) return 1;
     if ((p->ld1 & 3) || (p->ld2 & 3) || (p->ld3 & 3) || p->ld1 < p->geom.width || p->ld2 < p->geom.width ||
         p->ld3 < p->geom.width || !aligned16(p->P1) || !aligned16(p->P2) || !aligned16(p->P3)) {
@@ -187,6 +187,40 @@
         set_error("edge_attn_fwd: hub partial buffer needs ldpart >= width+8, ldpart %% 4 == 0");
         return 1;
     }
+    return 0;
+}
+
+static bool residual_of(const spk_residual_args* r, const spk_geom& g, bool bwd, ResidualArgs& o, const char* who) {
+    const int64_t w = (int64_t)g.n_heads * g.d_head;
+    if (!r || !r->mask || !r->out || !r->inv || r->ldo < w || (!bwd && (!r->ew || r->lde < w)) ||
+        (bwd && (!r->g || !r->dew || r->ldg < w || r->ldd < w))) {
+        set_error("%s: residual arrays missing or leading dimension below %lld", who, (long long)w);
+        return false;
+    }
+    o = ResidualArgs{};
+    o.mask = r->mask; o.out = r->out; o.ldo = r->ldo; o.inv = r->inv;
+    bool vec = g.d_head % 4 == 0 && r->ldo % 4 == 0 && aligned16(r->out);
+    if (bwd) {
+        o.g = r->g; o.ldg = r->ldg; o.dew = r->dew; o.ldd = r->ldd;
+        vec = vec && r->ldg % 4 == 0 && r->ldd % 4 == 0 && aligned16(r->g) && aligned16(r->dew);
+    } else {
+        o.ew = r->ew; o.lde = r->lde;
+        vec = vec && r->lde % 4 == 0 && aligned16(r->ew);
+    }
+    o.vec = vec;
+    return true;
+}
+
+int spk_edge_attn_fwd(const spk_edge_fwd_args* p, spk_stream_t stream) {
+    EdgeFwdArgs a;
+    if (int rc = edge_fwd_args_of(p, a)) return rc;
+    return launch_edge_fwd(a, (cudaStream_t)stream);
+}
+
+int spk_edge_attn_fwd_residual(const spk_edge_fwd_args* p, const spk_residual_args* r, spk_stream_t stream) {
+    EdgeFwdArgs a;
+    if (int rc = edge_fwd_args_of(p, a)) return rc;
+    if (!residual_of(r, p->geom, false, a.res, "edge_attn_fwd_residual")) return 1;
     return launch_edge_fwd(a, (cudaStream_t)stream);
 }
 
@@ -238,8 +272,7 @@
     return launch_edge_bwd_fused(a, (cudaStream_t)stream);
 }
 
-int spk_edge_attn_bwd_split(const spk_edge_bwd_split_args* q, spk_stream_t stream) {
-    BwdSplitArgs a;
+static int split_args_of(const spk_edge_bwd_split_args* q, BwdSplitArgs& a) {
     if (int rc = fused_args_of(&q->base, a.f, "edge_attn_bwd_split", q->dup)) return rc;
     if (q->base.csc_t2 != nullptr) { set_error("edge_attn_bwd_split: graphs with 2-hop edges are not supported"); return 1; }
     if ((q->ldd3 & 3) || q->ldd3 < q->base.geom.width || !aligned16(q->dP3) || !aligned16(q->rec4) ||
@@ -277,7 +310,22 @@
         set_error("edge_attn_bwd_split: relation hub partial buffer needs ldpart >= width");
         return 1;
     }
-    return launch_edge_bwd_split(a, (cudaStream_t)stream);
+    return 0;
+}
+
+int spk_edge_attn_bwd_split(const spk_edge_bwd_split_args* q, spk_stream_t stream) {
+    BwdSplitArgs a;
+    if (int rc = split_args_of(q, a)) return rc;
+    return launch_edge_bwd_split(a, nullptr, (cudaStream_t)stream);
+}
+
+int spk_edge_attn_bwd_split_residual(const spk_edge_bwd_split_args* q, const spk_residual_args* r, spk_stream_t stream) {
+    BwdSplitArgs a;
+    if (int rc = split_args_of(q, a)) return rc;
+    if (a.dup) { set_error("edge_attn_bwd_split_residual: not with dup tables"); return 1; }
+    ResidualArgs res;
+    if (!residual_of(r, q->base.geom, true, res, "edge_attn_bwd_split_residual")) return 1;
+    return launch_edge_bwd_split(a, &res, (cudaStream_t)stream);
 }
 
 static int fused_args_of(const spk_edge_bwd_fused_args* p, BwdFusedArgs& a, const char* who, int dup) {
diff --git a/recon_b200/csrc/spk_edge.cuh b/recon_b200/csrc/spk_edge.cuh
--- a/recon_b200/csrc/spk_edge.cuh
+++ b/recon_b200/csrc/spk_edge.cuh
@@ -21,6 +21,36 @@
     return h.task_order ? __ldg(h.task_order + slot) : slot;
 }
 
+struct ResidualArgs {
+    const float* ew; long lde;
+    const float* mask;
+    float* out; long ldo;
+    float* inv;
+    const float* g; long ldg;
+    float* dew; long ldd;
+    int vec;
+};
+
+__device__ __forceinline__ float4 load_act_chunk(const float* base, int h, int off, int D, int vec) {
+    const float* p = base + (long)h * D + off;
+    if (vec) return ldg4(p);
+    float4 r;
+    r.x = off + 0 < D ? __ldg(p + 0) : 0.f;
+    r.y = off + 1 < D ? __ldg(p + 1) : 0.f;
+    r.z = off + 2 < D ? __ldg(p + 2) : 0.f;
+    r.w = off + 3 < D ? __ldg(p + 3) : 0.f;
+    return r;
+}
+
+__device__ __forceinline__ void store_act_chunk(float* base, int h, int off, int D, int vec, float4 v) {
+    float* p = base + (long)h * D + off;
+    if (vec) { *reinterpret_cast<float4*>(p) = v; return; }
+    if (off + 0 < D) p[0] = v.x;
+    if (off + 1 < D) p[1] = v.y;
+    if (off + 2 < D) p[2] = v.z;
+    if (off + 3 < D) p[3] = v.w;
+}
+
 struct EdgeFwdArgs {
     const int* segptr;
     const int* col;
@@ -41,6 +71,7 @@
     int elu_rows;
     int out_vec;
     HubTasks hub;
+    ResidualArgs res;
 };
 
 struct EdgeBwdRowsArgs {
diff --git a/recon_b200/csrc/spk_edge_bwd.cuh b/recon_b200/csrc/spk_edge_bwd.cuh
--- a/recon_b200/csrc/spk_edge_bwd.cuh
+++ b/recon_b200/csrc/spk_edge_bwd.cuh
@@ -2,17 +2,6 @@
 #include "spk_edge.cuh"
 
 namespace spk {
-
-__device__ __forceinline__ float4 load_act_chunk(const float* base, int h, int off, int D, int vec) {
-    const float* p = base + (long)h * D + off;
-    if (vec) return ldg4(p);
-    float4 r;
-    r.x = off + 0 < D ? __ldg(p + 0) : 0.f;
-    r.y = off + 1 < D ? __ldg(p + 1) : 0.f;
-    r.z = off + 2 < D ? __ldg(p + 2) : 0.f;
-    r.w = off + 3 < D ? __ldg(p + 3) : 0.f;
-    return r;
-}
 
 template <int NCH, int HT>
 struct RowCtx {
@@ -24,15 +13,41 @@
 };
 
 template <int NCH, int HT>
-__device__ __forceinline__ void bwd_row_prologue(const EdgeBwdRowsArgs& a, int row, int lane, RowCtx<NCH, HT>& rc) {
+struct RowLoads {
+    float4 o[NCH];
+    float4 p1[NCH];
+    float4 q1v;
+    float den[HT];
+};
+
+template <int NCH, int HT>
+__device__ __forceinline__ void bwd_row_load(const EdgeBwdRowsArgs& a, int row, int lane, RowLoads<NCH, HT>& ld) {
+    const LayerGeom g = a.g;
+#pragma unroll
+    for (int h = 0; h < HT; ++h) ld.den[h] = h < g.H ? __ldg(a.den + (long)row * g.H + h) : 1.f;
+    ld.q1v = ldg4(a.P1 + (long)row * a.ld1 + (long)g.Dt4 * 4);
+#pragma unroll
+    for (int ci = 0; ci < NCH; ++ci) {
+        const int c4 = lane + 32 * ci;
+        ld.o[ci] = ld.p1[ci] = make_float4(0.f, 0.f, 0.f, 0.f);
+        if (c4 >= g.Dt4) continue;
+        const int h = HT > 1 ? c4 / g.Dp4 : 0;
+        ld.o[ci] = load_act_chunk(a.out + (long)row * a.ldo, h, (c4 - h * g.Dp4) * 4, g.D, a.out_vec);
+        ld.p1[ci] = ldg4(a.P1 + (long)row * a.ld1 + c4 * 4);
+    }
+}
+
+template <int NCH, int HT, bool REG = false>
+__device__ __forceinline__ void bwd_row_prologue(const EdgeBwdRowsArgs& a, int row, int lane, RowCtx<NCH, HT>& rc,
+                                                 const RowLoads<NCH, HT>& ld, const float4 (&dout_reg)[NCH]) {
     const LayerGeom g = a.g;
     float pdh[HT], pc1[HT], den[HT];
 #pragma unroll
     for (int h = 0; h < HT; ++h) {
         pdh[h] = 0.f; pc1[h] = 0.f;
-        den[h] = h < g.H ? __ldg(a.den + (long)row * g.H + h) : 1.f;
+        den[h] = REG ? ld.den[h] : (h < g.H ? __ldg(a.den + (long)row * g.H + h) : 1.f);
     }
-    const float4 q1v = ldg4(a.P1 + (long)row * a.ld1 + (long)g.Dt4 * 4);
+    const float4 q1v = REG ? ld.q1v : ldg4(a.P1 + (long)row * a.ld1 + (long)g.Dt4 * 4);
 #pragma unroll
     for (int h = 0; h < HT; ++h) rc.q1[h] = f4get(q1v, h);
 #pragma unroll
@@ -44,8 +59,8 @@
         const int h = HT > 1 ? c4 / g.Dp4 : 0;
         rc.hc[ci] = h;
         const int off = (c4 - h * g.Dp4) * 4;
-        const float4 o4 = load_act_chunk(a.out + (long)row * a.ldo, h, off, g.D, a.out_vec);
-        const float4 g4 = load_act_chunk(a.dout + (long)row * a.ldo, h, off, g.D, a.out_vec);
+        const float4 o4 = REG ? ld.o[ci] : load_act_chunk(a.out + (long)row * a.ldo, h, off, g.D, a.out_vec);
+        const float4 g4 = REG ? dout_reg[ci] : load_act_chunk(a.dout + (long)row * a.ldo, h, off, g.D, a.out_vec);
         const float o[4] = {o4.x, o4.y, o4.z, o4.w};
         const float gg[4] = {g4.x, g4.y, g4.z, g4.w};
         float dh[4], hv[4];
@@ -63,7 +78,7 @@
         const float d = selh<HT>(h, den);
         const float dot_h = fmaf(dh[0], hv[0], fmaf(dh[1], hv[1], fmaf(dh[2], hv[2], dh[3] * hv[3])));
         rc.dnum[ci] = make_float4(dh[0] / d, dh[1] / d, dh[2] / d, dh[3] / d);
-        const float4 p1 = ldg4(a.P1 + (long)row * a.ld1 + c4 * 4);
+        const float4 p1 = REG ? ld.p1[ci] : ldg4(a.P1 + (long)row * a.ld1 + c4 * 4);
         const float dot_c = f4dot(rc.dnum[ci], p1);
 #pragma unroll
         for (int hh = 0; hh < HT; ++hh) {
@@ -79,6 +94,13 @@
             rc.c1[h] = warp_sum(pc1[h]);
         }
     }
+}
+
+template <int NCH, int HT>
+__device__ __forceinline__ void bwd_row_prologue(const EdgeBwdRowsArgs& a, int row, int lane, RowCtx<NCH, HT>& rc) {
+    const float4 unused[NCH] = {};
+    const RowLoads<NCH, HT> none = {};
+    bwd_row_prologue<NCH, HT, false>(a, row, lane, rc, none, unused);
 }
 
 template <int NCH, int HT>
diff --git a/recon_b200/csrc/spk_edge_bwd_fused.cu b/recon_b200/csrc/spk_edge_bwd_fused.cu
--- a/recon_b200/csrc/spk_edge_bwd_fused.cu
+++ b/recon_b200/csrc/spk_edge_bwd_fused.cu
@@ -10,18 +10,60 @@
 __device__ __forceinline__ float fexp(float x) { return exp2f(x * 1.4426950408889634f); }
 
 template <int NCH, int HT>
+__device__ __forceinline__ void node_residual_bwd(const ResidualArgs& r, const LayerGeom& g, int row, int lane,
+                                                  float4 (&dout)[NCH]) {
+    float4 gv[NCH], ov[NCH];
+    float dot = 0.f;
+#pragma unroll
+    for (int ci = 0; ci < NCH; ++ci) {
+        const int c4 = lane + 32 * ci;
+        gv[ci] = ov[ci] = make_float4(0.f, 0.f, 0.f, 0.f);
+        if (c4 >= g.Dt4) continue;
+        const int h = HT > 1 ? c4 / g.Dp4 : 0;
+        const int off = (c4 - h * g.Dp4) * 4;
+        gv[ci] = load_act_chunk(r.g + (long)row * r.ldg, h, off, g.D, r.vec);
+        ov[ci] = load_act_chunk(r.out + (long)row * r.ldo, h, off, g.D, r.vec);
+        dot = fmaf(gv[ci].x, ov[ci].x, dot); dot = fmaf(gv[ci].y, ov[ci].y, dot);
+        dot = fmaf(gv[ci].z, ov[ci].z, dot); dot = fmaf(gv[ci].w, ov[ci].w, dot);
+    }
+    dot = warp_sum(dot);
+    const float inv = __ldg(r.inv + row);
+    const float m = __ldg(r.mask + row);
+    const bool clamped = inv >= 1e12f;
+#pragma unroll
+    for (int ci = 0; ci < NCH; ++ci) {
+        const int c4 = lane + 32 * ci;
+        const float4 gg = gv[ci], o = ov[ci];
+        const float4 dv = clamped ? make_float4(gg.x * inv, gg.y * inv, gg.z * inv, gg.w * inv)
+                                  : make_float4((gg.x - o.x * dot) * inv, (gg.y - o.y * dot) * inv,
+                                                (gg.z - o.z * dot) * inv, (gg.w - o.w * dot) * inv);
+        dout[ci] = make_float4(m * dv.x, m * dv.y, m * dv.z, m * dv.w);
+        if (c4 < g.Dt4) {
+            const int h = HT > 1 ? c4 / g.Dp4 : 0;
+            store_act_chunk(r.dew + (long)row * r.ldd, h, (c4 - h * g.Dp4) * 4, g.D, r.vec, dv);
+        }
+    }
+}
+
+template <int NCH, int HT, bool RES>
 __global__ void __launch_bounds__(SPK_CTA_THREADS)
-bwd_node_kernel(const EdgeBwdRowsArgs a, const float* __restrict__ sw, float* __restrict__ rowsc) {
+bwd_node_kernel(const EdgeBwdRowsArgs a, const float* __restrict__ sw, float* __restrict__ rowsc, const ResidualArgs res) {
     const int lane = threadIdx.x & 31;
     const int row = blockIdx.x * SPK_WARPS_PER_CTA + (threadIdx.x >> 5);
     if (row >= a.n_rows) return;
+    float4 dout[NCH] = {};
+    RowLoads<NCH, HT> ld = {};
+    if (RES) {
+        bwd_row_load<NCH, HT>(a, row, lane, ld);
+        node_residual_bwd<NCH, HT>(res, a.g, row, lane, dout);
+    }
     if (__ldg(a.segptr + row) == __ldg(a.segptr + row + 1)) {
         for (int c4 = lane; c4 < a.g.Wd4; c4 += 32)
             *reinterpret_cast<float4*>(a.dP1 + (long)row * a.ldd1 + c4 * 4) = make_float4(0.f, 0.f, 0.f, 0.f);
         return;
     }
     RowCtx<NCH, HT> rc;
-    bwd_row_prologue<NCH, HT>(a, row, lane, rc);
+    bwd_row_prologue<NCH, HT, RES>(a, row, lane, rc, ld, dout);
     float usum[HT], swsum[HT];
 #pragma unroll
     for (int h = 0; h < HT; ++h) {
@@ -322,18 +364,23 @@
 }
 
 
+template <int NCH, bool RES>
+int launch_node_n(const EdgeBwdRowsArgs& ra, const BwdFusedArgs& a, const ResidualArgs& res, cudaStream_t s) {
+    const unsigned grid = (a.n_rows + SPK_WARPS_PER_CTA - 1) / SPK_WARPS_PER_CTA;
+    if (a.g.H == 1) bwd_node_kernel<NCH, 1, RES><<<grid, SPK_CTA_THREADS, 0, s>>>(ra, a.sw, a.rowsc, res);
+    else if (a.g.H == 2) bwd_node_kernel<NCH, 2, RES><<<grid, SPK_CTA_THREADS, 0, s>>>(ra, a.sw, a.rowsc, res);
+    else bwd_node_kernel<NCH, 4, RES><<<grid, SPK_CTA_THREADS, 0, s>>>(ra, a.sw, a.rowsc, res);
+    return check_launch("bwd_node");
+}
+
 template <int NCH>
-int launch_node_n(const EdgeBwdRowsArgs& ra, const BwdFusedArgs& a, cudaStream_t s) {
-    const unsigned grid = (a.n_rows + SPK_WARPS_PER_CTA - 1) / SPK_WARPS_PER_CTA;
-    if (a.g.H == 1) bwd_node_kernel<NCH, 1><<<grid, SPK_CTA_THREADS, 0, s>>>(ra, a.sw, a.rowsc);
-    else if (a.g.H == 2) bwd_node_kernel<NCH, 2><<<grid, SPK_CTA_THREADS, 0, s>>>(ra, a.sw, a.rowsc);
-    else bwd_node_kernel<NCH, 4><<<grid, SPK_CTA_THREADS, 0, s>>>(ra, a.sw, a.rowsc);
-    return check_launch("bwd_node");
-}
-
-}
-
-int launch_edge_bwd_node(const BwdFusedArgs& a, cudaStream_t s) {
+int launch_node_r(const EdgeBwdRowsArgs& ra, const BwdFusedArgs& a, const ResidualArgs* res, cudaStream_t s) {
+    return res ? launch_node_n<NCH, true>(ra, a, *res, s) : launch_node_n<NCH, false>(ra, a, ResidualArgs{}, s);
+}
+
+}
+
+int launch_edge_bwd_node(const BwdFusedArgs& a, const ResidualArgs* res, cudaStream_t s) {
     if (a.n_rows <= 0) return 0;
     EdgeBwdRowsArgs ra;
     ra.segptr = a.rowptr; ra.col = nullptr; ra.t1 = nullptr; ra.t2 = nullptr;
@@ -344,16 +391,16 @@
     ra.n_rows = a.n_rows; ra.g = a.g; ra.alpha = a.alpha; ra.apply_elu = a.apply_elu; ra.out_vec = a.out_vec;
     ra.hub = a.row_hub;
     switch ((a.g.Wd4 + 31) / 32) {
-        case 1: return launch_node_n<1>(ra, a, s);
-        case 2: return launch_node_n<2>(ra, a, s);
-        case 3: return launch_node_n<3>(ra, a, s);
-        case 4: return launch_node_n<4>(ra, a, s);
+        case 1: return launch_node_r<1>(ra, a, res, s);
+        case 2: return launch_node_r<2>(ra, a, res, s);
+        case 3: return launch_node_r<3>(ra, a, res, s);
+        case 4: return launch_node_r<4>(ra, a, res, s);
         default: set_error("edge_bwd_node: row width %d floats exceeds the supported 512", a.g.Wd4 * 4); return 2;
     }
 }
 
 int launch_edge_bwd_fused(const BwdFusedArgs& a, cudaStream_t s) {
-    if (int rc = launch_edge_bwd_node(a, s)) return rc;
+    if (int rc = launch_edge_bwd_node(a, nullptr, s)) return rc;
     switch ((a.g.Wd4 + 31) / 32) {
         case 1: return launch_fused_n<1>(a, s);
         case 2: return launch_fused_n<2>(a, s);
diff --git a/recon_b200/csrc/spk_edge_bwd_fused.cuh b/recon_b200/csrc/spk_edge_bwd_fused.cuh
--- a/recon_b200/csrc/spk_edge_bwd_fused.cuh
+++ b/recon_b200/csrc/spk_edge_bwd_fused.cuh
@@ -56,8 +56,8 @@
 };
 
 int launch_edge_bwd_fused(const BwdFusedArgs& a, cudaStream_t s);
-int launch_edge_bwd_node(const BwdFusedArgs& a, cudaStream_t s);
-int launch_edge_bwd_split(const BwdSplitArgs& a, cudaStream_t s);
+int launch_edge_bwd_node(const BwdFusedArgs& a, const ResidualArgs* res, cudaStream_t s);
+int launch_edge_bwd_split(const BwdSplitArgs& a, const ResidualArgs* res, cudaStream_t s);
 int launch_seg_gather_hub_finalize(const SegGatherArgs& a, cudaStream_t s);
 
 }
diff --git a/recon_b200/csrc/spk_edge_bwd_split.cu b/recon_b200/csrc/spk_edge_bwd_split.cu
--- a/recon_b200/csrc/spk_edge_bwd_split.cu
+++ b/recon_b200/csrc/spk_edge_bwd_split.cu
@@ -451,9 +451,9 @@
 }
 
 template <int NCH, int HT>
-int launch_split_t(const BwdSplitArgs& a, cudaStream_t s) {
+int launch_split_t(const BwdSplitArgs& a, const ResidualArgs* res, cudaStream_t s) {
     if (a.phases & 1) {
-        if (int rc = launch_edge_bwd_node(a.f, s)) return rc;
+        if (int rc = launch_edge_bwd_node(a.f, res, s)) return rc;
     }
     if (a.phases & 2) {
         if (int rc = launch_split_pass<NCH, HT>(a, s, 0)) return rc;
@@ -486,20 +486,20 @@
 }
 
 template <int NCH>
-int launch_split_n(const BwdSplitArgs& a, cudaStream_t s) {
-    if (a.g.H == 1) return launch_split_t<NCH, 1>(a, s);
-    if (a.g.H == 2) return launch_split_t<NCH, 2>(a, s);
-    return launch_split_t<NCH, 4>(a, s);
-}
-
-}
-
-int launch_edge_bwd_split(const BwdSplitArgs& a, cudaStream_t s) {
+int launch_split_n(const BwdSplitArgs& a, const ResidualArgs* res, cudaStream_t s) {
+    if (a.g.H == 1) return launch_split_t<NCH, 1>(a, res, s);
+    if (a.g.H == 2) return launch_split_t<NCH, 2>(a, res, s);
+    return launch_split_t<NCH, 4>(a, res, s);
+}
+
+}
+
+int launch_edge_bwd_split(const BwdSplitArgs& a, const ResidualArgs* res, cudaStream_t s) {
     switch ((a.g.Wd4 + 31) / 32) {
-        case 1: return launch_split_n<1>(a, s);
-        case 2: return launch_split_n<2>(a, s);
-        case 3: return launch_split_n<3>(a, s);
-        case 4: return launch_split_n<4>(a, s);
+        case 1: return launch_split_n<1>(a, res, s);
+        case 2: return launch_split_n<2>(a, res, s);
+        case 3: return launch_split_n<3>(a, res, s);
+        case 4: return launch_split_n<4>(a, res, s);
         default: set_error("edge_bwd_split: row width %d floats exceeds the supported 512", a.g.Wd4 * 4); return 2;
     }
 }
diff --git a/recon_b200/csrc/spk_edge_fwd.cu b/recon_b200/csrc/spk_edge_fwd.cu
--- a/recon_b200/csrc/spk_edge_fwd.cu
+++ b/recon_b200/csrc/spk_edge_fwd.cu
@@ -112,6 +112,36 @@
 }
 
 template <int NCH, int HT>
+__device__ __forceinline__ void fwd_residual(const EdgeFwdArgs& a, int row, int lane, const int (&hc)[NCH],
+                                             const float4 (&x)[NCH]) {
+    const LayerGeom g = a.g;
+    const ResidualArgs& r = a.res;
+    const float m = __ldg(r.mask + row);
+    float4 v[NCH];
+    float ss = 0.f;
+#pragma unroll
+    for (int ci = 0; ci < NCH; ++ci) {
+        const int c4 = lane + 32 * ci;
+        v[ci] = make_float4(0.f, 0.f, 0.f, 0.f);
+        if (c4 >= g.Dt4) continue;
+        const float4 e = load_act_chunk(r.ew + (long)row * r.lde, hc[ci], (c4 - hc[ci] * g.Dp4) * 4, g.D, r.vec);
+        v[ci] = make_float4(e.x + m * x[ci].x, e.y + m * x[ci].y, e.z + m * x[ci].z, e.w + m * x[ci].w);
+        ss = fmaf(v[ci].x, v[ci].x, ss); ss = fmaf(v[ci].y, v[ci].y, ss);
+        ss = fmaf(v[ci].z, v[ci].z, ss); ss = fmaf(v[ci].w, v[ci].w, ss);
+    }
+    ss = warp_sum(ss);
+    const float inv = 1.f / fmaxf(sqrtf(ss), 1e-12f);
+#pragma unroll
+    for (int ci = 0; ci < NCH; ++ci) {
+        const int c4 = lane + 32 * ci;
+        if (c4 >= g.Dt4) continue;
+        store_act_chunk(r.out + (long)row * r.ldo, hc[ci], (c4 - hc[ci] * g.Dp4) * 4, g.D, r.vec,
+                        make_float4(v[ci].x * inv, v[ci].y * inv, v[ci].z * inv, v[ci].w * inv));
+    }
+    if (lane == 0) r.inv[row] = inv;
+}
+
+template <int NCH, int HT>
 __device__ __forceinline__ void fwd_finalize(const EdgeFwdArgs& a, int row, int lane, const int (&hc)[NCH],
                                              FwdAcc<NCH, HT>& st, bool& bad, uint32_t p1_smem = 0) {
     const LayerGeom g = a.g;
@@ -121,9 +151,11 @@
         if (st.den[h] == 0.f) st.den[h] = 1e-12f;
         rden[h] = 1.0f / st.den[h];
     }
+    float4 x[NCH];
 #pragma unroll
     for (int ci = 0; ci < NCH; ++ci) {
         const int c4 = lane + 32 * ci;
+        x[ci] = make_float4(0.f, 0.f, 0.f, 0.f);
         if (c4 >= g.Dt4) continue;
         const int h = hc[ci];
         const float d = selh<HT>(h, rden);
@@ -146,11 +178,14 @@
             for (int k = 0; k < 4; ++k)
                 if (off + k < g.D) dst[k] = o[k];
         }
+        x[ci] = make_float4(off + 0 < g.D ? o[0] : 0.f, off + 1 < g.D ? o[1] : 0.f,
+                            off + 2 < g.D ? o[2] : 0.f, off + 3 < g.D ? o[3] : 0.f);
     }
     if (lane < g.H) {
         a.den[(long)row * g.H + lane] = selh<HT>(lane, st.den);
         a.sw[(long)row * g.H + lane] = selh<HT>(lane, st.sw);
     }
+    if (a.res.out) fwd_residual<NCH, HT>(a, row, lane, hc, x);
 }
 
 
@@ -161,6 +196,17 @@
     float* dst = a.out + (long)row * a.ldo;
     for (int c = lane; c < hd; c += 32) dst[c] = 0.f;
     if (lane < g.H) { a.den[(long)row * g.H + lane] = 1e-12f; a.sw[(long)row * g.H + lane] = 0.f; }
+    if (a.res.out) {
+        int hc[NCH];
+        float4 x[NCH];
+#pragma unroll
+        for (int ci = 0; ci < NCH; ++ci) {
+            const int c4 = lane + 32 * ci;
+            hc[ci] = (HT > 1 && c4 < g.Dt4) ? c4 / g.Dp4 : 0;
+            x[ci] = make_float4(0.f, 0.f, 0.f, 0.f);
+        }
+        fwd_residual<NCH, HT>(a, row, lane, hc, x);
+    }
 }
 
 template <int NCH, int HT, bool HAS2>
@@ -352,6 +398,7 @@
     }
     unsigned rem = TASKS ? 0u : act;
     int pk = 0;
+    const uint32_t ew_bytes = (a.res.out && a.res.vec) ? (uint32_t)(g.H * g.D) * 4u : 0u;
     auto issue_p1 = [&]() {
         if (!rem) return;
         const int r = __ffs(rem) - 1;
@@ -360,6 +407,7 @@
             const uint32_t bar = bars + 8u * (NG + (pk & 1));
             sbar_expect(bar, row_bytes);
             bulk_g2s(p1buf + (uint32_t)(pk & 1) * row_bytes, a.P1 + (row0 + r) * a.ld1, row_bytes, bar);
+            if (ew_bytes) bulk_prefetch_l2(a.res.ew + (row0 + r) * a.res.lde, ew_bytes);
         }
         ++pk;
     };
diff --git a/recon_b200/csrc/spk_stream.cuh b/recon_b200/csrc/spk_stream.cuh
--- a/recon_b200/csrc/spk_stream.cuh
+++ b/recon_b200/csrc/spk_stream.cuh
@@ -25,6 +25,9 @@
 __device__ __forceinline__ void bulk_g2s(uint32_t dst, const void* src, uint32_t bytes, uint32_t bar) {
     asm volatile("cp.async.bulk.shared::cluster.global.mbarrier::complete_tx::bytes [%0], [%1], %2, [%3];"
                  ::"r"(dst), "l"(src), "r"(bytes), "r"(bar) : "memory");
+}
+__device__ __forceinline__ void bulk_prefetch_l2(const void* src, uint32_t bytes) {
+    asm volatile("cp.async.bulk.prefetch.L2.global [%0], %1;" ::"l"(src), "r"(bytes) : "memory");
 }
 __device__ __forceinline__ float4 lds4(uint32_t addr) {
     float4 v;
diff --git a/recon_b200/functional.py b/recon_b200/functional.py
--- a/recon_b200/functional.py
+++ b/recon_b200/functional.py
@@ -232,7 +232,7 @@
     return torch.empty(hubs.n_tasks, ldpart, dtype=torch.float32, device=device)
 
 
-def edge_attn_forward(graph, P1, P2, P3, geom, alpha, apply_elu, mask_csr, nanflag, elu_rows=0):
+def edge_attn_forward(graph, P1, P2, P3, geom, alpha, apply_elu, mask_csr, nanflag, elu_rows=0, res=None):
     lib = _lib.load()
     n = graph.n_nodes
     dev = P1.device
@@ -254,11 +254,16 @@
     ldpart = geom.Wd + 2 * MAX_HEADS
     partial = _hub_partial(graph.row_hubs, ldpart, dev)
     graph.row_hubs.fill(a.hub, partial, ldpart)
-    _lib.check(lib.spk_edge_attn_fwd(C.byref(a), _lib.stream_ptr()), "edge_attn_fwd")
+    if res is None:
+        _lib.check(lib.spk_edge_attn_fwd(C.byref(a), _lib.stream_ptr()), "edge_attn_fwd")
+    else:
+        _lib.check(lib.spk_edge_attn_fwd_residual(C.byref(a), C.byref(res), _lib.stream_ptr()), "edge_attn_fwd_residual")
     return out, den, sw
 
 
 BWD_MODE = os.environ.get("SPK_BWD_MODE", "split")
+
+FUSE_RESIDUAL = True
 
 
 def _fill_fused_args(f, graph, P1, P2, P3, geom, alpha, apply_elu, mask_csr, out, dout, den, sw, G, ldg, rowsc, dP1, dP2, rec):
@@ -269,8 +274,10 @@
     f.P3 = P3.data_ptr(); f.ld3 = P3.stride(0)
     if mask_csr is not None:
         f.mask = mask_csr.data_ptr(); f.mask_stride = mask_csr.stride(0)
-    f.out = out.data_ptr(); f.dout = dout.data_ptr(); f.ldo = out.stride(0)
-    assert dout.stride(0) == out.stride(0)
+    f.out = out.data_ptr(); f.ldo = out.stride(0)
+    if dout is not None:
+        f.dout = dout.data_ptr()
+        assert dout.stride(0) == out.stride(0)
     f.den = den.data_ptr(); f.sw = sw.data_ptr()
     f.G = G.data_ptr(); f.ldg = ldg; f.rowsc = rowsc.data_ptr()
     f.dP1 = dP1.data_ptr(); f.ldd1 = dP1.stride(0); f.dP2 = dP2.data_ptr(); f.ldd2 = dP2.stride(0)
@@ -284,7 +291,7 @@
 
 
 def edge_attn_backward(graph, P1, P2, P3, geom, alpha, apply_elu, mask_csr, out, dout, den, sw, dP1, dP2, dP3,
-                       after_columns=None, colsum=None):
+                       after_columns=None, colsum=None, res=None):
     lib = _lib.load()
     graph.build_backward()
     n, dev = graph.n_nodes, P1.device
@@ -293,6 +300,9 @@
     mode = BWD_MODE if sw is not None else "rows"
     if mode == "split" and graph.t2 is not None:
         mode = "rows"
+    if res is not None:
+        assert graph.t2 is None and after_columns is None
+        mode = "split"
     ne = max(1, graph.n_edges)
     if mode == "split":
         q = _lib.EdgeBwdSplitArgs()
@@ -308,14 +318,21 @@
         graph.rel_hubs.fill(q.rel_hub, part3, geom.Wd)
         part1 = _hub_partial(graph.row_hubs, 4, dev)
         graph.row_hubs.fill(q.base.row_hub, part1, 4)
+
+        def run_split():
+            if res is None:
+                _lib.check(lib.spk_edge_attn_bwd_split(C.byref(q), _lib.stream_ptr()), "edge_attn_bwd_split")
+            else:
+                _lib.check(lib.spk_edge_attn_bwd_split_residual(C.byref(q), C.byref(res), _lib.stream_ptr()),
+                           "edge_attn_bwd_split_residual")
         if after_columns is None:
             if lib.timing is None:
-                _lib.check(lib.spk_edge_attn_bwd_split(C.byref(q), _lib.stream_ptr()), "edge_attn_bwd_split")
+                run_split()
             else:
                 for ph, tag in ((1, "node"), (2, "cols"), (4, "rels"), (8, "colsums")):
                     q.phases = ph
                     _lib.current_tag = tag
-                    _lib.check(lib.spk_edge_attn_bwd_split(C.byref(q), _lib.stream_ptr()), "edge_attn_bwd_split")
+                    run_split()
                 _lib.current_tag = ""
             del keep, part3, part1
             return False
@@ -401,12 +418,24 @@
     return ext
 
 
+def _residual_args(EW, mask, out, inv, g=None, dew=None):
+    r = _lib.ResidualArgs()
+    r.mask = mask.data_ptr(); r.out = out.data_ptr(); r.ldo = out.stride(0); r.inv = inv.data_ptr()
+    if EW is not None:
+        r.ew = EW.data_ptr(); r.lde = EW.stride(0)
+    if g is not None:
+        r.g = g.data_ptr(); r.ldg = g.stride(0); r.dew = dew.data_ptr(); r.ldd = dew.stride(0)
+    return r
+
+
 class AttentionGroupFn(torch.autograd.Function):
 
     @staticmethod
-    def forward(ctx, X, Wn, Rel, Wr, graph, geom, alpha, apply_elu, mask_csr, nanflag):
+    def forward(ctx, X, Wn, Rel, Wr, graph, geom, alpha, apply_elu, mask_csr, nanflag, EW=None, mask=None):
         X = tc_friendly(X.contiguous()); Wn = Wn.contiguous(); Rel = Rel.contiguous(); Wr = Wr.contiguous()
         dist = getattr(graph, "dist", None)
+        ctx.residual = EW is not None
+        assert not ctx.residual or (dist is None and graph.t2 is None)
         ghost = dist.ghost if dist is not None else None
         Wd = geom.Wd
         mode = "local"
@@ -444,7 +473,14 @@
             h.wait()
         if ghost is not None and mode != "proj":
             raise NotImplementedError("hub rows split across ranks need the projected exchange (or the aggregate-then-project path)")
-        if ghost is None:
+        if ctx.residual:
+            EW = EW if EW.stride(1) == 1 else EW.contiguous()
+            res_out = torch.empty(X.shape[0], geom.H * geom.D, dtype=torch.float32, device=X.device)
+            inv = torch.empty(X.shape[0], dtype=torch.float32, device=X.device)
+            out, den, sw = edge_attn_forward(graph, P1, P2, P3, geom, alpha, apply_elu, mask_csr, nanflag,
+                                             res=_residual_args(EW, mask, res_out, inv))
+            out_ret = out
+        elif ghost is None:
             out, den, sw = edge_attn_forward(graph, P1, P2, P3, geom, alpha, apply_elu, mask_csr, nanflag)
             out_ret = out
         else:
@@ -459,20 +495,33 @@
                                                        _lib.stream_ptr()), "elu_inplace")
             out[ghost.mine_local] = out[n:][ghost.mine]
             out_ret = out[:n]
-        ctx.save_for_backward(X, Wn, Rel, Wr, P1, P2, P3, out, den, sw, X_all if X_all is not None else X.new_empty(0))
+        ctx.save_for_backward(X, Wn, Rel, Wr, P1, P2, P3, out, den, sw, X_all if X_all is not None else X.new_empty(0),
+                              *((res_out, inv, mask) if ctx.residual else ()))
         ctx.graph, ctx.geom, ctx.alpha, ctx.apply_elu, ctx.mask_csr, ctx.mode = graph, geom, alpha, apply_elu, mask_csr, mode
+        if ctx.residual:
+            ctx.mark_non_differentiable(out_ret, den, sw)
+            ctx.set_materialize_grads(False)
+            return out_ret, den, sw, res_out
         ctx.mark_non_differentiable(den, sw)
         return out_ret, den, sw
 
     @staticmethod
-    def backward(ctx, dout, _dden, _dsw):
+    def backward(ctx, dout, _dden, _dsw, dres=None):
         geom, graph, mode = ctx.geom, ctx.graph, ctx.mode
         dist = getattr(graph, "dist", None)
-        X, Wn, Rel, Wr, P1, P2, P3, out, den, sw, X_all = ctx.saved_tensors
+        X, Wn, Rel, Wr, P1, P2, P3, out, den, sw, X_all = ctx.saved_tensors[:11]
         Wd = geom.Wd
-        dout = dout.contiguous()
         n = X.shape[0]
         dev = X.device
+        res = dEW = None
+        if ctx.residual:
+            res_out, inv, mask = ctx.saved_tensors[11:]
+            dres = dres.contiguous()
+            dEW = torch.empty_like(res_out)
+            res = _residual_args(None, mask, res_out, inv, dres, dEW)
+            dout = None
+        else:
+            dout = dout.contiguous()
         dP3 = torch.empty_like(P3)
         WnT = Wn.t().contiguous()
         need_x, need_w = ctx.needs_input_grad[0], ctx.needs_input_grad[1]
@@ -480,7 +529,7 @@
         if mode == "local":
             dP = torch.empty(n, 2 * Wd, dtype=torch.float32, device=dev)
             edge_attn_backward(graph, P1, P2, P3, geom, ctx.alpha, ctx.apply_elu, ctx.mask_csr, out, dout, den, sw,
-                               dP[:, :Wd], dP[:, Wd:], dP3)
+                               dP[:, :Wd], dP[:, Wd:], dP3, res=res)
             if need_x:
                 dX = gemm_nn(dP, WnT)
             if need_w:
@@ -554,7 +603,7 @@
                 h3.wait()
         dRel = gemm_nn(dP3, Wr.t().contiguous()) if ctx.needs_input_grad[2] else None
         dWr = gemm_tn(Rel, dP3) if ctx.needs_input_grad[3] else None
-        return dX, dWn, dRel, dWr, None, None, None, None, None, None
+        return dX, dWn, dRel, dWr, None, None, None, None, None, None, dEW, None
 
 
 
@@ -848,7 +897,7 @@
         return dX, dRel, dWa, dV, dV3, None, None, None, None, None, None
 
 
-def attention_group(X, Rel, a_list, a2_list, graph, alpha, apply_elu, mask_csr, nanflag):
+def attention_group(X, Rel, a_list, a2_list, graph, alpha, apply_elu, mask_csr, nanflag, residual=None):
     outs = []
     if X.shape[0] != graph.n_nodes - getattr(graph, "n_ghost", 0):
         raise IndexError(f"entity table has {X.shape[0]} rows but the graph was built for "
@@ -862,7 +911,19 @@
     F = X.shape[1]
     D = a_list[0].shape[0]
     Rd = a_list[0].shape[1] - 2 * F
-    if use_agg_path(min(len(a_list), AGG_MAX_HEADS), F, Rd, D, graph):
+    agg = use_agg_path(min(len(a_list), AGG_MAX_HEADS), F, Rd, D, graph)
+    if residual is not None:
+        EW, mask = residual
+        if (FUSE_RESIDUAL and not agg and len(a_list) <= MAX_HEADS and getattr(graph, "dist", None) is None
+                and BWD_MODE == "split" and graph.t2 is None and EW.shape == (X.shape[0], len(a_list) * D)):
+            geom = Geometry(len(a_list), D)
+            Wn, Wr = extended_weights(a_list, a2_list, F, geom)
+            out, _, _, res = AttentionGroupFn.apply(X, Wn, Rel, Wr, graph, geom, alpha, apply_elu, mask_csr, nanflag,
+                                                    EW, mask)
+            return out, res
+        out = attention_group(X, Rel, a_list, a2_list, graph, alpha, apply_elu, mask_csr, nanflag)
+        return out, ResidualNormFn.apply(EW, out, mask)
+    if agg:
         for g0 in range(0, len(a_list), AGG_MAX_HEADS):
             al, a2l = a_list[g0:g0 + AGG_MAX_HEADS], a2_list[g0:g0 + AGG_MAX_HEADS]
             geom = AggGeometry(len(al), F, Rd, D)
diff --git a/recon_b200/models.py b/recon_b200/models.py
--- a/recon_b200/models.py
+++ b/recon_b200/models.py
@@ -45,9 +45,10 @@
         dev = x.device
         with torch.cuda.device(dev):
             return self._forward(x, relation_embed, edge_list, edge_type, edge_list_nhop, edge_type_nhop, graph,
-                                 dropout_masks, nanflag)
-
-    def _forward(self, x, relation_embed, edge_list, edge_type, edge_list_nhop, edge_type_nhop, graph, dropout_masks, nanflag):
+                                 dropout_masks, nanflag)[:2]
+
+    def _forward(self, x, relation_embed, edge_list, edge_type, edge_list_nhop, edge_type_nhop, graph, dropout_masks, nanflag,
+                 residual=None):
         dev = x.device
         if graph is None:
             graph = KGraph(edge_list, edge_type, _nhop_rows(edge_list_nhop, edge_type_nhop), x.shape[0],
@@ -76,11 +77,16 @@
         if m_x is not None:
             x = x * m_x
         out_relation_1 = SF.matmul(relation_embed, self.W)
-        x = SF.attention_group(x, out_relation_1, [self.out_att.a], [self.out_att.a_2], graph, self.alpha,
-                               True, m_out, nanflag)
+        res = None
+        if residual is None:
+            x = SF.attention_group(x, out_relation_1, [self.out_att.a], [self.out_att.a_2], graph, self.alpha,
+                                   True, m_out, nanflag)
+        else:
+            x, res = SF.attention_group(x, out_relation_1, [self.out_att.a], [self.out_att.a_2], graph, self.alpha,
+                                        True, m_out, nanflag, residual=residual())
         if own_flag:
             check_nanflag(nanflag)
-        return x, out_relation_1
+        return x, out_relation_1, res
 
 
 class SpKBGATModified(nn.Module):
@@ -163,13 +169,15 @@
     def _run_on(self, entity_embeddings, relation_embeddings, batch_entities, graph, dropout_masks, entities_upgraded=None):
         dev = entity_embeddings.device
         nanflag = torch.zeros(1, dtype=torch.int32, device=dev)
-        out_entity_1, out_relation_1 = self.sparse_gat_1(
-            None, entity_embeddings, relation_embeddings, None, None, None, None, None,
-            graph=graph, dropout_masks=dropout_masks, nanflag=nanflag)
         mask = SF.mask_from_index(torch.as_tensor(batch_entities), entity_embeddings.shape[0], dev, flag=nanflag)
-        if entities_upgraded is None:
-            entities_upgraded = SF.matmul(entity_embeddings, self.W_entities, getattr(graph, "dist", None))
-        out_entity_1 = SF.ResidualNormFn.apply(entities_upgraded, out_entity_1, mask)
+
+        def residual():
+            ew = entities_upgraded
+            if ew is None:
+                ew = SF.matmul(entity_embeddings, self.W_entities, getattr(graph, "dist", None))
+            return ew, mask
+        _, out_relation_1, out_entity_1 = self.sparse_gat_1._forward(
+            entity_embeddings, relation_embeddings, None, None, None, None, graph, dropout_masks, nanflag, residual)
         check_nanflag(nanflag)
         return out_entity_1, out_relation_1, mask
 
```

After: 517.6 million, median of 6. 1.5% higher.
